# rasd3/3D-Dual-Fusion

Hardware: AMD Instinct MI355X
Metric: nuScenes sweeps/sec (0.075 m voxel, ~60k pts) (higher is better)
Workload: dtype f32 (fp32-grade throughout: every matrix-core GEMM -- C>=32 sparse convs, neck / head convs, FFN, query linears, image projection, value GEMM -- takes its fp32 operands as fp16 hi+lo pairs, 22 significand bits, 3 MFMA products, fp32 accumulate: <= 4e-6 of scale against float64, the grade of the exac

## Files before the change

### 3d-dual-fusion_amd/csrc/common.h

```cpp
#pragma once
#include <hip/hip_runtime.h>
#include <stdint.h>
#include <stdio.h>

#include "../../include/df3d_hip.h"

namespace df3d {

void set_error(const char *fmt, ...);

#define DF3D_CHECK_ARG(cond, ...)            \
  do {                                       \
    if (!(cond)) {                           \
      df3d::set_error(__VA_ARGS__);          \
      return DF3D_EINVAL;                    \
    }                                        \
  } while (0)

#define DF3D_HIP(call)                                                                   \
  do {                                                                                   \
    hipError_t e__ = (call);                                                             \
    if (e__ != hipSuccess) {                                                             \
      df3d::set_error("%s failed: %s (%s:%d)", #call, hipGetErrorString(e__), __FILE__, \
                      __LINE__);                                                         \
      return DF3D_EHIP;                                                                  \
    }                                                                                    \
  } while (0)

#define DF3D_LAUNCH_CHECK()                                                                  \
  do {                                                                                       \
    hipError_t e__ = hipGetLastError();                                                      \
    if (e__ != hipSuccess) {                                                                 \
      df3d::set_error("kernel launch failed: %s (%s:%d)", hipGetErrorString(e__), __FILE__, \
                      __LINE__);                                                             \
      return DF3D_EHIP;                                                                      \
    }                                                                                        \
  } while (0)

static inline size_t align_up(size_t v, size_t a) { return (v + a - 1) / a * a; }
#ifdef __HIPCC__
#define DF3D_SA_EXP 5
#define DF3D_SW_EXP 7
#define DF3D_SA_SCALE 32.0f
#define DF3D_SW_SCALE 128.0f
#define DF3D_SA_INV 0.03125f
#define DF3D_ACC_UNSCALE 0.000244140625f
#define DF3D_AA_UNSCALE 0.0009765625f
typedef __bf16 df3d_bf16x2 __attribute__((ext_vector_type(2)));
typedef _Float16 df3d_f16x2 __attribute__((ext_vector_type(2)));
typedef float df3d_f32x2 __attribute__((ext_vector_type(2)));
typedef _Float16 df3d_f16x8 __attribute__((ext_vector_type(8)));

static __device__ unsigned g_split_overflow_tu;

__device__ __forceinline__ unsigned rd_mix(unsigned x) {
  x ^= x >> 16, x *= 0x7feb352du, x ^= x >> 15, x *= 0x846ca68bu, x ^= x >> 16;
  return x;
}
__device__ __forceinline__ bool rd_keep(unsigned long long i, unsigned s0, unsigned s1, unsigned thr) {
  const unsigned h = rd_mix(rd_mix((unsigned)i ^ s0) + (unsigned)(i >> 32) * 0x9E3779B9u + s1);
  return (h >> 8) >= thr;
}

__device__ __forceinline__ unsigned bf16_pair(float x0, float x1) {
  df3d_f32x2 v = {x0, x1};
  return __builtin_bit_cast(unsigned, __builtin_convertvector(v, df3d_bf16x2));
}
__device__ __forceinline__ void split_pair_bf16_ref(float x0, float x1, unsigned &hi, unsigned &lo) {
  df3d_f32x2 v = {x0, x1};
  df3d_bf16x2 h = __builtin_convertvector(v, df3d_bf16x2);
  df3d_f32x2 r = v - __builtin_convertvector(h, df3d_f32x2);
  df3d_bf16x2 l = __builtin_convertvector(r, df3d_bf16x2);
  hi = __builtin_bit_cast(unsigned, h);
  lo = __builtin_bit_cast(unsigned, l);
}
template <bool CHECK>
__device__ __forceinline__ void split_pair_f16_ref(float x0, float x1, float s, unsigned &hi, unsigned &lo) {
  df3d_f32x2 v = {x0 * s, x1 * s};
  if (CHECK) {
    if (__builtin_expect(!(__builtin_fabsf(v[0]) <= 65504.f) || !(__builtin_fabsf(v[1]) <= 65504.f), 0))
      atomicOr(&g_split_overflow_tu, 1u);
  }
  df3d_f16x2 h = __builtin_convertvector(v, df3d_f16x2);
  df3d_f32x2 r = v - __builtin_convertvector(h, df3d_f32x2);
  df3d_f16x2 l = __builtin_convertvector(r, df3d_f16x2);
  hi = __builtin_bit_cast(unsigned, h);
  lo = __builtin_bit_cast(unsigned, l);
}
#define DF3D_SPLIT_PAIR_(x0, x1, S, CHECK, HI, LO)                          \
  do {                                                                      \
    unsigned sp_h__, sp_l__;                                                \
    df3d::split_pair_f16_ref<CHECK>(x0, x1, S, sp_h__, sp_l__);             \
    (HI) = sp_h__;                                                          \
    (LO) = sp_l__;                                                          \
  } while (0)
#define split_pair(x0, x1, HI, LO) DF3D_SPLIT_PAIR_(x0, x1, DF3D_SA_SCALE, true, HI, LO)
#define split_pair_nc(x0, x1, HI, LO) DF3D_SPLIT_PAIR_(x0, x1, DF3D_SA_SCALE, false, HI, LO)
#define split_pair_acc(x0, x1, HI, LO, AMAX)                                                  \
  do {                                                                                        \
    (AMAX) = fmaxf((AMAX), fmaxf(__builtin_fabsf(x0), __builtin_fabsf(x1)));                  \
    DF3D_SPLIT_PAIR_(x0, x1, DF3D_SA_SCALE, false, HI, LO);                                   \
  } while (0)
#define split_range_flag(AMAX)                                                                \
  do {                                                                                        \
    if (__builtin_expect(!((AMAX) * DF3D_SA_SCALE <= 65504.f), 0)) atomicOr(&df3d::g_split_overflow_tu, 1u); \
  } while (0)
#define split_range_flag_scaled(AMAX)                                                         \
  do {                                                                                        \
    if (__builtin_expect(!((AMAX) <= 65504.f), 0)) atomicOr(&df3d::g_split_overflow_tu, 1u);  \
  } while (0)
#define split_pair_w(x0, x1, HI, LO) DF3D_SPLIT_PAIR_(x0, x1, DF3D_SW_SCALE, true, HI, LO)
#define split_pair_bf16(x0, x1, HI, LO)                  \
  do {                                                   \
    unsigned sp_h__, sp_l__;                             \
    df3d::split_pair_bf16_ref(x0, x1, sp_h__, sp_l__);   \
    (HI) = sp_h__;                                       \
    (LO) = sp_l__;                                       \
  } while (0)
__device__ __forceinline__ void split_one(float x, unsigned &hi, unsigned &lo) {
  unsigned h, l;
  split_pair_f16_ref<true>(x, 0.f, DF3D_SA_SCALE, h, l);
  hi = h & 0xffffu;
  lo = l & 0xffffu;
}
__device__ __forceinline__ df3d_f32x2 split_part_to_f32(unsigned packed) {
  df3d_f32x2 v = __builtin_convertvector(__builtin_bit_cast(df3d_f16x2, packed), df3d_f32x2);
  return v * DF3D_SA_INV;
}
__device__ __forceinline__ df3d_f32x2 split_to_f32(unsigned hi, unsigned lo) {
  df3d_f32x2 h = __builtin_convertvector(__builtin_bit_cast(df3d_f16x2, hi), df3d_f32x2);
  df3d_f32x2 l = __builtin_convertvector(__builtin_bit_cast(df3d_f16x2, lo), df3d_f32x2);
  return (h + l) * DF3D_SA_INV;
}
#define DF3D_MFMA_F16(A, B, C) \
  __builtin_amdgcn_mfma_f32_16x16x32_f16(__builtin_bit_cast(df3d_f16x8, A), __builtin_bit_cast(df3d_f16x8, B), C, 0, 0, 0)
#endif

void split_overflow_register(const void *symbol, const char *tu);
#ifdef __HIPCC__
#define DF3D_SPLIT_OVERFLOW_TU(name)                                                                       \
  namespace {                                                                                              \
  struct SplitOverflowReg_##name {                                                                         \
    SplitOverflowReg_##name() { df3d::split_overflow_register((const void *)&df3d::g_split_overflow_tu, #name); } \
  } g_split_overflow_reg_##name;                                                                           \
  }
#endif

static inline int cdiv(long long a, long long b) { return (int)((a + b - 1) / b); }

struct Arena {
  char *base;
  size_t size, off;
  Arena(void *p, size_t n) : base((char *)p), size(n), off(0) {}
  template <typename T>
  T *take(size_t count) {
    size_t o = align_up(off, 256);
    size_t end = o + count * sizeof(T);
    if (end > size) return nullptr;
    off = end;
    return (T *)(base + o);
  }
};
static inline size_t arena_need(size_t cur, size_t bytes) { return align_up(cur, 256) + bytes; }

size_t scan_scratch_bytes(size_t n);
int exclusive_scan_u32(const uint32_t *in, uint32_t *out, size_t n, uint32_t *total,
                       void *scratch, size_t scratch_bytes, hipStream_t stream);
int exclusive_scan_popc64(const unsigned long long *words, uint32_t *out, size_t n,
                          uint32_t *total, void *scratch, size_t scratch_bytes,
                          hipStream_t stream);

struct GridHeader {
  int batch, shape[3];
  unsigned long long ncells;
  unsigned long long nwords;
  size_t off_bits, off_prefix, off_total, off_scratch, scratch_bytes;
};
struct GridView {
  const unsigned long long *bits;
  const uint32_t *prefix;
  int shape[3];
  long long vol;
};
GridHeader grid_layout(int batch, const int *shape);
static inline GridView grid_view(const void *blob, const GridHeader &h) {
  GridView v;
  v.bits = (const unsigned long long *)((const char *)blob + h.off_bits);
  v.prefix = (const uint32_t *)((const char *)blob + h.off_prefix);
  v.shape[0] = h.shape[0];
  v.shape[1] = h.shape[1];
  v.shape[2] = h.shape[2];
  v.vol = (long long)h.shape[0] * h.shape[1] * h.shape[2];
  return v;
}

__device__ __forceinline__ int grid_rank(const GridView &g, long long flat) {
  unsigned long long w = g.bits[flat >> 6];
  int b = (int)(flat & 63);
  if (!((w >> b) & 1ull)) return -1;
  return (int)(g.prefix[flat >> 6] + __popcll(w & ((1ull << b) - 1ull)));
}

size_t conv_operand_packed_bytes(int parts, int kvol, int cin, int cout);
int conv_operand_rows(int parts, const float *x, long long n, int c, void *rows, hipStream_t stream);
int conv_operand_run(int parts, const void *in, int n_in, int cin, const void *packed, int kvol, int cout, const int32_t *nbr,
                     int n_out, const float *bias, const float *scale, const float *shift, const void *residual, int relu,
                     float *out, void *out_rows, hipStream_t stream);

size_t topk_keys_workspace(int S, long long n, int K);
int topk_keys(const unsigned long long *keys, int S, long long n, int K, unsigned long long *out, int32_t *out_count,
              void *ws, size_t ws_bytes, hipStream_t stream);

}
```

### 3d-dual-fusion_amd/csrc/common.hip

```cpp
#include <stdarg.h>
#include <string.h>

#include "common.h"

namespace df3d {

static thread_local char g_err[512] = "";

void set_error(const char *fmt, ...) {
  va_list ap;
  va_start(ap, fmt);
  vsnprintf(g_err, sizeof(g_err), fmt, ap);
  va_end(ap);
}

static const void *g_ovf_sym[64];
static const char *g_ovf_tu[64];
static constexpr int OVF_MAXDEV = 16;
static unsigned *g_ovf_dev[OVF_MAXDEV][64];
static unsigned **g_ovf_table[OVF_MAXDEV];
static int g_ovf_table_n[OVF_MAXDEV];
static int g_ovf_n = 0;

static int ovf_resolve() {
  int dev = 0;
  if (hipGetDevice(&dev) != hipSuccess || dev < 0 || dev >= OVF_MAXDEV) return -1;
  for (int i = 0; i < g_ovf_n; ++i) {
    if (g_ovf_dev[dev][i]) continue;
    void *p = nullptr;
    if (hipGetSymbolAddress(&p, g_ovf_sym[i]) != hipSuccess || !p) {
      (void)hipGetLastError();
      continue;
    }
    g_ovf_dev[dev][i] = (unsigned *)p;
  }
  return dev;
}

__global__ void ovf_collect_kernel(unsigned *const *flags, int n, unsigned *out, int reset) {
  unsigned m = 0;
  for (int i = threadIdx.x; i < n; i += 64) {
    unsigned *f = flags[i];
    if (f && *f) {
      m |= 1u << (i & 31);
      if (reset) *f = 0u;
    }
  }
  for (int d = 32; d >= 1; d >>= 1) m |= __shfl_xor(m, d, 64);
  if (threadIdx.x == 0) *out = m;
}
void split_overflow_register(const void *symbol, const char *tu) {
  if (g_ovf_n < 64) g_ovf_sym[g_ovf_n] = symbol, g_ovf_tu[g_ovf_n] = tu, ++g_ovf_n;
}

constexpr int SCAN_THREADS = 256;
constexpr int SCAN_ITEMS = 4;
constexpr int SCAN_TILE = SCAN_THREADS * SCAN_ITEMS;

struct LoadU32 {
  const uint32_t *p;
  __device__ uint32_t operator()(size_t i) const { return p[i]; }
};
struct LoadPopc {
  const unsigned long long *p;
  __device__ uint32_t operator()(size_t i) const { return (uint32_t)__popcll(p[i]); }
};

__device__ __forceinline__ uint32_t wave_incl_scan(uint32_t v, int lane) {
#pragma unroll
  for (int d = 1; d < 64; d <<= 1) {
    uint32_t t = __shfl_up(v, d, 64);
    if (lane >= d) v += t;
  }
  return v;
}

__device__ __forceinline__ void block_excl_scan(uint32_t (&x)[SCAN_ITEMS], uint32_t &total,
                                                uint32_t *lds ) {
  int tid = threadIdx.x, lane = tid & 63, wave = tid >> 6;
  uint32_t s = 0;
#pragma unroll
  for (int i = 0; i < SCAN_ITEMS; ++i) s += x[i];
  uint32_t inc = wave_incl_scan(s, lane);
  if (lane == 63) lds[wave] = inc;
  __syncthreads();
  uint32_t woff = 0, tot = 0;
#pragma unroll
  for (int w = 0; w < SCAN_THREADS / 64; ++w) {
    uint32_t v = lds[w];
    if (w < wave) woff += v;
    tot += v;
  }
  uint32_t run = woff + inc - s;
#pragma unroll
  for (int i = 0; i < SCAN_ITEMS; ++i) {
    uint32_t v = x[i];
    x[i] = run;
    run += v;
  }
  total = tot;
  __syncthreads();
}

template <typename Loader>
__global__ __launch_bounds__(SCAN_THREADS) void scan_tiles_kernel(Loader in, uint32_t *out, size_t n,
                                                                  uint32_t *sums, uint32_t *total_if_single) {
  __shared__ uint32_t lds[SCAN_THREADS / 64 + 1];
  size_t base = (size_t)blockIdx.x * SCAN_TILE + (size_t)threadIdx.x * SCAN_ITEMS;
  uint32_t x[SCAN_ITEMS];
#pragma unroll
  for (int i = 0; i < SCAN_ITEMS; ++i) x[i] = (base + i < n) ? in(base + i) : 0u;
  uint32_t tot;
  block_excl_scan(x, tot, lds);
#pragma unroll
  for (int i = 0; i < SCAN_ITEMS; ++i)
    if (base + i < n) out[base + i] = x[i];
  if (threadIdx.x == 0) {
    sums[blockIdx.x] = tot;
    if (total_if_single) *total_if_single = tot;
  }
}

__global__ __launch_bounds__(SCAN_THREADS) void scan_offset_kernel(uint32_t *out, size_t n, const uint32_t *sums, size_t nb,
                                                                   uint32_t *total) {
  __shared__ uint32_t lds[SCAN_THREADS / 64];
  __shared__ uint32_t s_off;
  const int tid = threadIdx.x, lane = tid & 63, wave = tid >> 6;
  const bool last = blockIdx.x + 1 == nb;
  const size_t upto = last ? nb : blockIdx.x;
  uint32_t s = 0, mine = 0;
  for (size_t i = tid; i < upto; i += SCAN_THREADS) {
    const uint32_t v = sums[i];
    if (i < blockIdx.x) mine += v;
    s += v;
  }
#pragma unroll
  for (int d = 32; d >= 1; d >>= 1) {
    mine += __shfl_xor(mine, d, 64);
    s += __shfl_xor(s, d, 64);
  }
  __shared__ uint32_t lds2[SCAN_THREADS / 64];
  if (lane == 0) {
    lds[wave] = mine;
    lds2[wave] = s;
  }
  __syncthreads();
  if (tid == 0) {
    uint32_t a = 0, b = 0;
    for (int w = 0; w < SCAN_THREADS / 64; ++w) {
      a += lds[w];
      b += lds2[w];
    }
    s_off = a;
    if (last && total) *total = b;
  }
  __syncthreads();
  const uint32_t add = s_off;
  size_t base = (size_t)blockIdx.x * SCAN_TILE + (size_t)threadIdx.x * SCAN_ITEMS;
#pragma unroll
  for (int i = 0; i < SCAN_ITEMS; ++i)
    if (base + i < n) out[base + i] += add;
}

size_t scan_scratch_bytes(size_t n) { return align_up((n / SCAN_TILE + 2) * sizeof(uint32_t), 256); }

template <typename Loader>
static int scan_impl(Loader in, uint32_t *out, size_t n, uint32_t *total, void *scratch, size_t scratch_bytes,
                     hipStream_t stream) {
  if (n == 0) {
    if (total) DF3D_HIP(hipMemsetAsync(total, 0, sizeof(uint32_t), stream));
    return DF3D_OK;
  }
  if (scratch_bytes < scan_scratch_bytes(n)) {
    set_error("scan scratch too small");
    return DF3D_ENOMEM;
  }
  uint32_t *sums = (uint32_t *)scratch;
  size_t nb = (n + SCAN_TILE - 1) / SCAN_TILE;
  hipLaunchKernelGGL(scan_tiles_kernel<Loader>, dim3((unsigned)nb), dim3(SCAN_THREADS), 0, stream, in, out, n, sums,
                     nb == 1 ? total : (uint32_t *)nullptr);
  if (nb > 1)
    hipLaunchKernelGGL(scan_offset_kernel, dim3((unsigned)nb), dim3(SCAN_THREADS), 0, stream, out, n, sums, nb, total);
  DF3D_LAUNCH_CHECK();
  return DF3D_OK;
}

int exclusive_scan_u32(const uint32_t *in, uint32_t *out, size_t n, uint32_t *total, void *scratch,
                       size_t scratch_bytes, hipStream_t stream) {
  return scan_impl(LoadU32{in}, out, n, total, scratch, scratch_bytes, stream);
}
int exclusive_scan_popc64(const unsigned long long *words, uint32_t *out, size_t n, uint32_t *total,
                          void *scratch, size_t scratch_bytes, hipStream_t stream) {
  return scan_impl(LoadPopc{words}, out, n, total, scratch, scratch_bytes, stream);
}

}

extern "C" {

int df3d_version(void) { return 100; }

int df3d_split_overflow(int reset, char *where, int where_len) {
  unsigned any = 0;
  if (where && where_len > 0) where[0] = 0;
  if (hipDeviceSynchronize() != hipSuccess) {
    df3d::set_error("df3d_split_overflow: hipDeviceSynchronize failed");
    return DF3D_EHIP;
  }
  const int dev = df3d::ovf_resolve();
  if (dev < 0) {
    df3d::set_error("df3d_split_overflow: no current device");
    return DF3D_EHIP;
  }
  for (int i = 0; i < df3d::g_ovf_n; ++i) {
    unsigned *f = df3d::g_ovf_dev[dev][i];
    if (!f) continue;
    unsigned v = 0;
    DF3D_HIP(hipMemcpy(&v, f, sizeof(v), hipMemcpyDeviceToHost));
    if (v) {
      any |= v;
      if (where && where_len > 0) {
        size_t used = strlen(where);
        snprintf(where + used, (size_t)where_len - used, "%s%s", used ? "," : "", df3d::g_ovf_tu[i]);
      }
      if (reset) DF3D_HIP(hipMemset(f, 0, sizeof(v)));
    }
  }
  return any ? 1 : 0;
}

int df3d_split_overflow_collect(uint32_t *out, int reset, void *stream_) {
  hipStream_t stream = (hipStream_t)stream_;
  DF3D_CHECK_ARG(out, "split_overflow_collect: null output");
  const int dev = df3d::ovf_resolve();
  if (dev < 0) {
    df3d::set_error("df3d_split_overflow_collect: no current device");
    return DF3D_EHIP;
  }
  int resolved = 0;
  for (int i = 0; i < df3d::g_ovf_n; ++i) resolved += df3d::g_ovf_dev[dev][i] != nullptr;
  if (!df3d::g_ovf_table[dev] || df3d::g_ovf_table_n[dev] != resolved) {
    if (!df3d::g_ovf_table[dev]) DF3D_HIP(hipMalloc((void **)&df3d::g_ovf_table[dev], sizeof(unsigned *) * 64));
    DF3D_HIP(hipMemcpyAsync(df3d::g_ovf_table[dev], df3d::g_ovf_dev[dev], sizeof(unsigned *) * 64, hipMemcpyHostToDevice, stream));
    DF3D_HIP(hipStreamSynchronize(stream));
    df3d::g_ovf_table_n[dev] = resolved;
  }
  hipLaunchKernelGGL(df3d::ovf_collect_kernel, dim3(1), dim3(64), 0, stream, df3d::g_ovf_table[dev], df3d::g_ovf_n, out, reset);
  DF3D_LAUNCH_CHECK();
  return DF3D_OK;
}

int df3d_split_overflow_units(char *buf, int buflen) {
  if (!buf || buflen <= 0) return df3d::g_ovf_n;
  buf[0] = 0;
  for (int i = 0; i < df3d::g_ovf_n; ++i) {
    size_t used = strlen(buf);
    snprintf(buf + used, (size_t)buflen - used, "%s%s", used ? "," : "", df3d::g_ovf_tu[i]);
  }
  return df3d::g_ovf_n;
}
const char *df3d_last_error(void) { return df3d::g_err; }

int df3d_device_count(void) {
  int n = 0;
  if (hipGetDeviceCount(&n) != hipSuccess) return 0;
  return n;
}

int df3d_device_arch(char *buf, int buflen) {
  hipDeviceProp_t p;
  if (hipGetDeviceProperties(&p, 0) != hipSuccess) {
    df3d::set_error("hipGetDeviceProperties failed");
    return DF3D_EHIP;
  }
  snprintf(buf, buflen, "%s", p.gcnArchName);
  return DF3D_OK;
}
}
```

### 3d-dual-fusion_amd/csrc/executor.hip

```cpp
#include <stdio.h>
#include <stdlib.h>
#include <string.h>

#include <condition_variable>
#include <deque>
#include <mutex>
#include <string>
#include <thread>
#include <vector>

#include "common.h"

using namespace df3d;

namespace {

struct IndexSet {
  const int32_t *indices = nullptr;
  int n = 0;
  int shape[3] = {0, 0, 0};
  void *grid = nullptr;
  size_t grid_bytes = 0;
  int32_t *perm = nullptr;
  bool sorted = false;
};

struct LayerOut {
  float *features = nullptr;
  void *split = nullptr;
  void *rows16 = nullptr;
  int set = -1;
  int channels = 0;
  bool ran = false;
};

struct Bump {
  char *base;
  size_t cap, used = 0;
  bool overflow = false;
  Bump(void *p, size_t bytes) : base((char *)p), cap(bytes) {}
  void *take(size_t bytes) {
    size_t off = align_up(used, 256);
    used = off + bytes;
    if (used > cap) {
      overflow = true;
      return nullptr;
    }
    return base + off;
  }
};

int kvol_of(const int *k) { return k[0] * k[1] * k[2]; }

thread_local hipStream_t g_geo_stream = nullptr;
thread_local std::vector<hipEvent_t> g_event_sets[16];
thread_local unsigned g_run_counter = 0;
#define g_events g_event_sets[g_run_counter & 15]
thread_local hipEvent_t g_inputs_ready = nullptr;
hipEvent_t order_event(size_t i) {
  while (g_events.size() <= i) {
    hipEvent_t e = nullptr;
    if (hipEventCreateWithFlags(&e, hipEventDisableTiming) != hipSuccess) return nullptr;
    g_events.push_back(e);
  }
  return g_events[i];
}

}

extern "C" int df3d_backbone_inputs_ready(void *event) {
  g_inputs_ready = (hipEvent_t)event;
  return DF3D_OK;
}

namespace {

struct RunState {
  const df3d_layer *layers = nullptr;
  int nlayers = 0;
  const int32_t *indices = nullptr;
  int n = 0, in_channels = 0, batch = 0;
  int shape[3] = {0, 0, 0};
  Bump *gmem = nullptr;
  Bump *fmem = nullptr;
  Bump own_g{nullptr, 0}, own_f{nullptr, 0};
  std::vector<IndexSet> sets;
  std::vector<LayerOut> outs;
  std::vector<std::pair<int, const int32_t *>> rulebooks;
  std::vector<int> rulebook_set;
  std::vector<const int32_t *> layer_nbr;
  std::vector<const void *> rulebook_lists;
  std::vector<const void *> layer_lists;
  std::vector<int> layer_in_set;
  std::vector<char> need_f32;
  std::vector<char> want_split;
  int32_t *count_dev = nullptr;
  void *split0 = nullptr;
  void *rows16_0 = nullptr;
  hipEvent_t done = nullptr;
  hipEvent_t img_done = nullptr;
  int geometry_layers = 0;
  const float *input_features = nullptr;
  int range_next = 0;
};

int fail_arena(RunState &S, Bump *m, size_t *arena_used, size_t arena_bytes) {
  if (arena_used) *arena_used = m->used;
  set_error("backbone_run: arena of %zu bytes is too small (needed more than %zu)", arena_bytes, m->used);
  (void)S;
  return DF3D_ENOMEM;
}


int layer_parts(const df3d_layer &L) {
  if (!L.packed) return 0;
  if (L.reserved & 2) return 1;
  if (L.reserved & 8) return 3;
  return conv_operand_packed_bytes(2, kvol_of(L.ksize), L.cin, L.cout) != 0 ? 2 : 0;
}

int state_init(RunState &S, const df3d_layer *layers, int nlayers, const int32_t *indices, int n, int in_channels, int batch,
               const int *shape) {
  S.layers = layers, S.nlayers = nlayers, S.indices = indices, S.n = n, S.in_channels = in_channels, S.batch = batch;
  memcpy(S.shape, shape, sizeof(S.shape));
  S.outs.assign(nlayers, LayerOut());
  S.layer_nbr.assign(nlayers, nullptr);
  S.layer_lists.assign(nlayers, nullptr);
  S.layer_in_set.assign(nlayers, 0);
  IndexSet s0;
  s0.indices = indices;
  s0.n = n;
  memcpy(s0.shape, shape, sizeof(s0.shape));
  S.sets.push_back(s0);
  S.need_f32.assign(nlayers, 0);
  S.want_split.assign(nlayers, 0);
  bool flagged = false;
  for (int li = 0; li < nlayers; ++li) flagged = flagged || (layers[li].reserved & 4);
  static const bool write_all = getenv("DF3D_EXEC_F32_ALL") && atoi(getenv("DF3D_EXEC_F32_ALL"));
  if (write_all) flagged = false;
  for (int li = 0; li < nlayers; ++li) {
    const df3d_layer &L = layers[li];
    if (!flagged || (L.reserved & 4) || li == nlayers - 1) S.need_f32[li] = 1;
    if (L.residual >= 0 && L.residual < nlayers) S.need_f32[L.residual] = 1;
    const int parts = layer_parts(L);
    const bool split_consumer = parts >= 2 && !(L.reserved & 1) &&
                                conv_operand_packed_bytes(parts, kvol_of(L.ksize), L.cin, L.cout) != 0;
    if (L.input >= 0 && L.input < nlayers && !split_consumer) S.need_f32[L.input] = 1;
    if (L.input >= 0 && L.input < nlayers && split_consumer && !(L.reserved & 8)) S.want_split[L.input] = 1;
  }
  return DF3D_OK;
}

int geo_layer(RunState &S, int li, hipStream_t gstream, bool *new_table) {
  void *gs_ = (void *)gstream;
  Bump &mem = *S.gmem;
  const df3d_layer &L = S.layers[li];
  const int batch = S.batch;
  *new_table = false;
  DF3D_CHECK_ARG(L.input >= -1 && L.input < li && L.residual >= -1 && L.residual < li,
                 "backbone_run: layer %d reads a later layer", li);
  const int in_set = L.input < 0 ? 0 : S.outs[L.input].set;
  const int cin = L.input < 0 ? S.in_channels : S.outs[L.input].channels;
  DF3D_CHECK_ARG(cin == L.cin, "backbone_run: layer %d expects %d input channels, gets %d", li, L.cin, cin);
  const int K = kvol_of(L.ksize);
  DF3D_CHECK_ARG(K > 0 && K <= DF3D_MAX_KVOL, "backbone_run: layer %d kernel volume %d unsupported", li, K);
  if (!S.count_dev) {
    S.count_dev = (int32_t *)mem.take(256);
    if (!S.count_dev) return DF3D_ENOMEM;
  }
  const int32_t *nbr = nullptr;
  const void *lists = nullptr;
  int out_set = -1;
  if (L.rulebook >= 0)
    for (size_t r = 0; r < S.rulebooks.size(); ++r)
      if (S.rulebooks[r].first == L.rulebook) {
        nbr = S.rulebooks[r].second;
        lists = S.rulebook_lists[r];
        out_set = S.rulebook_set[r];
        DF3D_CHECK_ARG(L.kind != 0 || out_set == in_set,
                       "backbone_run: layer %d shares rulebook %d but reads another index set", li, L.rulebook);
      }
  if (!nbr) {
    auto ensure_grid = [&](int si) -> int {
      IndexSet &T = S.sets[si];
      if (T.grid) return DF3D_OK;
      T.grid_bytes = df3d_grid_bytes(batch, T.shape);
      T.grid = mem.take(T.grid_bytes);
      if (!T.sorted) T.perm = (int32_t *)mem.take((size_t)T.n * 4);
      if (!T.grid || (!T.sorted && !T.perm)) return DF3D_ENOMEM;
      return df3d_grid_build(T.indices, T.n, batch, T.shape, T.grid, T.grid_bytes, T.perm, gs_);
    };
    if (L.kind == 0) {
      int rc = ensure_grid(in_set);
      if (rc) return rc;
      const IndexSet &T = S.sets[in_set];
      int32_t *t = (int32_t *)mem.take((size_t)K * T.n * 4);
      if (!t) return DF3D_ENOMEM;
      rc = df3d_subm_neighbors(T.grid, T.perm, T.indices, T.n, batch, T.shape, L.ksize, L.dilation, t, gs_);
      if (rc) return rc;
      nbr = t;
      out_set = in_set;
    } else {
      const IndexSet T = S.sets[in_set];
      IndexSet O;
      for (int d = 0; d < 3; ++d)
        O.shape[d] = (T.shape[d] + 2 * L.padding[d] - L.dilation[d] * (L.ksize[d] - 1) - 1) / L.stride[d] + 1;
      long long fan = 1;
      for (int d = 0; d < 3; ++d) fan *= (L.ksize[d] + L.stride[d] - 1) / L.stride[d];
      long long vol = (long long)batch * O.shape[0] * O.shape[1] * O.shape[2];
      long long cap = (long long)T.n * (fan < K ? fan : K);
      if (cap > vol) cap = vol;
      if (cap < 1) cap = 1;
      O.grid_bytes = df3d_grid_bytes(batch, O.shape);
      O.grid = mem.take(O.grid_bytes);
      int32_t *oi = (int32_t *)mem.take((size_t)cap * 16);
      if (!O.grid || !oi) return DF3D_ENOMEM;
      int rc = df3d_conv_out_indices(T.indices, T.n, batch, T.shape, O.shape, L.ksize, L.stride, L.padding,
                                     L.dilation, O.grid, O.grid_bytes, oi, (int)cap, S.count_dev, gs_);
      if (rc) return rc;
      int32_t cnt = 0;
      DF3D_HIP(hipMemcpyAsync(&cnt, S.count_dev, sizeof(cnt), hipMemcpyDeviceToHost, gstream));
      DF3D_HIP(hipStreamSynchronize(gstream));
      if (cnt > cap) {
        set_error("backbone_run: layer %d produced %d outputs, capacity bound %lld", li, cnt, cap);
        return DF3D_EINVAL;
      }
      if (cnt <= 0) {
        set_error("backbone_run: layer %d has no active outputs", li);
        return DF3D_EINVAL;
      }
      O.indices = oi;
      O.n = cnt;
      O.sorted = true;
      S.sets.push_back(O);
      out_set = (int)S.sets.size() - 1;
      rc = ensure_grid(in_set);
      if (rc) return rc;
      const IndexSet &Tg = S.sets[in_set];
      int32_t *t = (int32_t *)mem.take((size_t)K * cnt * 4);
      if (!t) return DF3D_ENOMEM;
      rc = df3d_conv_neighbors(Tg.grid, Tg.perm, oi, cnt, batch, Tg.shape, L.ksize, L.stride, L.padding, L.dilation,
                               t, gs_);
      if (rc) return rc;
      nbr = t;
    }
    *new_table = true;
    static const bool lists_on = !(getenv("DF3D_ROW_LISTS") && getenv("DF3D_ROW_LISTS")[0] == '0');
    const bool fp32_small = !(L.reserved & 1) && layer_parts(L) == 0;
    const int n_rows = S.sets[out_set].n;
    if (lists_on && fp32_small && L.cin <= 16 && (L.cout == 16 || L.cout == 32) && n_rows >= 2048 &&
        S.sets[in_set].n < (1 << 26)) {
      const size_t lb = df3d_nbr_row_lists_bytes(K, n_rows);
      void *blob = lb ? mem.take(lb) : nullptr;
      if (lb && !blob) return DF3D_ENOMEM;
      if (blob) {
        int rc = df3d_nbr_row_lists(nbr, K, n_rows, S.sets[in_set].n, blob, lb, gs_);
        if (rc) return rc;
        lists = blob;
      }
    }
    S.rulebooks.push_back(std::make_pair(L.rulebook, nbr));
    S.rulebook_lists.push_back(lists);
    S.rulebook_set.push_back(out_set);
  }
  S.layer_nbr[li] = nbr;
  S.layer_lists[li] = lists;
  S.layer_in_set[li] = in_set;
  S.outs[li].set = out_set;
  S.outs[li].channels = L.cout;
  S.geometry_layers = li + 1;
  return DF3D_OK;
}

void view_geometry(const RunState &S, int li, df3d_layer_view &v) {
  const IndexSet &OS = S.sets[S.outs[li].set];
  v.nbr = S.layer_nbr[li];
  v.kvol = kvol_of(S.layers[li].ksize);
  v.indices = OS.indices;
  v.grid = OS.grid;
  v.grid_bytes = OS.grid_bytes;
  v.n = OS.n;
  v.channels = S.layers[li].cout;
  v.rows_sorted = OS.sorted ? 1 : 0;
  memcpy(v.shape, OS.shape, sizeof(v.shape));
}

int conv_layer(RunState &S, int li, const float *features, df3d_layer_view *views, hipStream_t stream) {
  void *stream_ = (void *)stream;
  Bump &mem = *S.fmem;
  const df3d_layer &L = S.layers[li];
  const int K = kvol_of(L.ksize);
  const int32_t *nbr = S.layer_nbr[li];
  const int in_set = S.layer_in_set[li], out_set = S.outs[li].set;
  const float *in_feat = L.input < 0 ? features : S.outs[L.input].features;
  const int n_out = S.sets[out_set].n;
  const int n_in = S.sets[in_set].n;
  LayerOut &o = S.outs[li];
  df3d_layer_view &v = views[li];
  view_geometry(S, li, v);
  if (L.reserved & 1) {
    v.features = nullptr;
    v.split = nullptr;
    return DF3D_OK;
  }
  DF3D_CHECK_ARG(L.input < 0 || S.outs[L.input].ran, "backbone_run: layer %d reads a geometry-only layer", li);
  o.ran = true;
  const int parts = layer_parts(L);
  if (parts)
    DF3D_CHECK_ARG(conv_operand_packed_bytes(parts, K, L.cin, L.cout) != 0,
                   "backbone_run: layer %d has no kernel on %d-part operands (K=%d cin=%d cout=%d)", li, parts, K, L.cin, L.cout);
  if (S.need_f32[li] || parts < 2) {
    o.features = (float *)mem.take((size_t)n_out * L.cout * 4);
    if (!o.features) return DF3D_ENOMEM;
  }
  const float *res = L.residual < 0 ? nullptr : S.outs[L.residual].features;
  if (L.residual >= 0)
    DF3D_CHECK_ARG(S.outs[L.residual].set == out_set && S.outs[L.residual].channels == L.cout,
                   "backbone_run: residual of layer %d lives on another index set", li);
  if (parts) {
    const size_t bpc = 2 * (size_t)parts;
    auto slot = [&](int layer) -> void *& {
      if (parts == 1) return layer < 0 ? S.rows16_0 : S.outs[layer].rows16;
      return layer < 0 ? S.split0 : S.outs[layer].split;
    };
    auto operand = [&](int layer, const float *rows, int n, int c, const void **out) {
      void *&r = slot(layer);
      if (!r) {
        r = mem.take((size_t)n * c * bpc);
        if (!r) return (int)DF3D_ENOMEM;
        int rc = conv_operand_rows(parts, rows, n, c, r, stream);
        if (rc) return rc;
      }
      *out = r;
      return (int)DF3D_OK;
    };
    const void *in_rows = nullptr, *res_rows = res;
    int rc = operand(L.input, in_feat, n_in, L.cin, &in_rows);
    if (rc) return rc;
    if (parts == 1 && L.residual >= 0) {
      rc = operand(L.residual, res, n_out, L.cout, &res_rows);
      if (rc) return rc;
    }
    void *&out_rows = slot(li);
    out_rows = mem.take((size_t)n_out * L.cout * bpc);
    if (!out_rows) return DF3D_ENOMEM;
    rc = conv_operand_run(parts, in_rows, n_in, L.cin, L.packed, K, L.cout, nbr, n_out, L.bias, L.scale, L.shift, res_rows,
                          L.relu, o.features, out_rows, stream);
    if (rc) return rc;
  } else {
    if (S.want_split[li] && S.layer_lists[li] && L.cout % 8 == 0) {
      o.split = mem.take((size_t)n_out * L.cout * 4);
      if (!o.split) return DF3D_ENOMEM;
    }
    int rc = df3d_sparse_conv_fused_lists(in_feat, n_in, L.cin, L.weight, K, L.cout, nbr, S.layer_lists[li], n_out, L.bias,
                                          L.scale, L.shift, res, L.relu, o.features, o.split, stream_);
    if (rc) return rc;
  }
  v.features = o.features;
  v.split = o.split ? o.split : o.rows16;
  v.reserved = o.rows16 && !o.split ? 2 : ((L.reserved & 8) && o.split ? 4 : 0);
  return DF3D_OK;
}

}

extern "C" int df3d_backbone_run(const df3d_layer *layers, int nlayers, const float *features, const int32_t *indices,
                                 int n, int in_channels, int batch, const int *shape, void *arena,
                                 size_t arena_bytes, df3d_layer_view *views, size_t *arena_used, void *stream_) {
  hipStream_t stream = (hipStream_t)stream_;
  hipEvent_t inputs_ready = g_inputs_ready;
  g_inputs_ready = nullptr;
  ++g_run_counter;
  DF3D_CHECK_ARG(layers && nlayers > 0 && features && indices && shape && arena && views,
                 "backbone_run: null argument");
  DF3D_CHECK_ARG(n > 0 && batch > 0, "backbone_run: empty input (n=%d, batch=%d)", n, batch);
  static const bool two_streams = !(getenv("DF3D_EXEC_STREAMS") && getenv("DF3D_EXEC_STREAMS")[0] == '0');
  hipStream_t gstream = stream;
  size_t next_event = 0;
  if (two_streams) {
    if (!g_geo_stream) DF3D_HIP(hipStreamCreateWithFlags(&g_geo_stream, hipStreamNonBlocking));
    gstream = g_geo_stream;
    if (inputs_ready) {
      DF3D_HIP(hipStreamWaitEvent(gstream, inputs_ready, 0));
    } else {
      hipEvent_t e = order_event(next_event++);
      DF3D_CHECK_ARG(e != nullptr, "backbone_run: cannot create an event");
      DF3D_HIP(hipEventRecord(e, stream));
      DF3D_HIP(hipStreamWaitEvent(gstream, e, 0));
    }
  }
  RunState S;
  S.own_g = Bump(arena, arena_bytes);
  S.gmem = S.fmem = &S.own_g;
  int rc = state_init(S, layers, nlayers, indices, n, in_channels, batch, shape);
  if (rc) return rc;
  for (int li = 0; li < nlayers; ++li) {
    bool new_table = false;
    rc = geo_layer(S, li, gstream, &new_table);
    if (rc == DF3D_ENOMEM) return fail_arena(S, S.gmem, arena_used, arena_bytes);
    if (rc) return rc;
    if (new_table && two_streams) {
      hipEvent_t e = order_event(next_event++);
      DF3D_CHECK_ARG(e != nullptr, "backbone_run: cannot create an event");
      DF3D_HIP(hipEventRecord(e, gstream));
      DF3D_HIP(hipStreamWaitEvent(stream, e, 0));
    }
    rc = conv_layer(S, li, features, views, stream);
    if (rc == DF3D_ENOMEM) return fail_arena(S, S.fmem, arena_used, arena_bytes);
    if (rc) return rc;
  }
  if (two_streams) {
    hipEvent_t e = order_event(next_event++);
    DF3D_CHECK_ARG(e != nullptr, "backbone_run: cannot create an event");
    DF3D_HIP(hipEventRecord(e, gstream));
    DF3D_HIP(hipStreamWaitEvent(stream, e, 0));
  }
  for (int li = 0; li < nlayers; ++li) {
    const IndexSet &OS = S.sets[S.outs[li].set];
    views[li].grid = OS.grid;
    views[li].grid_bytes = OS.grid_bytes;
  }
  if (arena_used) *arena_used = S.gmem->used;
  return DF3D_OK;
}

extern "C" int df3d_backbone_geometry(const df3d_layer *layers, int nlayers, const int32_t *indices, int n, int in_channels,
                                      int batch, const int *shape, void *arena, size_t arena_bytes, void *inputs_ready,
                                      df3d_layer_view *views, size_t *arena_used, void **handle) {
  DF3D_CHECK_ARG(layers && nlayers > 0 && indices && shape && arena && views && handle, "backbone_geometry: null argument");
  DF3D_CHECK_ARG(n > 0 && batch > 0, "backbone_geometry: empty input (n=%d, batch=%d)", n, batch);
  *handle = nullptr;
  if (!g_geo_stream) DF3D_HIP(hipStreamCreateWithFlags(&g_geo_stream, hipStreamNonBlocking));
  hipStream_t gstream = g_geo_stream;
  if (inputs_ready) DF3D_HIP(hipStreamWaitEvent(gstream, (hipEvent_t)inputs_ready, 0));
  RunState *S = new RunState();
  S->own_g = Bump(arena, arena_bytes);
  S->gmem = &S->own_g;
  int rc = state_init(*S, layers, nlayers, indices, n, in_channels, batch, shape);
  for (int li = 0; li < nlayers && !rc; ++li) {
    bool new_table = false;
    rc = geo_layer(*S, li, gstream, &new_table);
  }
  if (arena_used) *arena_used = S->gmem->used;
  if (rc == DF3D_ENOMEM) set_error("backbone_geometry: arena of %zu bytes is too small (needed more than %zu)", arena_bytes, S->gmem->used);
  if (!rc && hipEventCreateWithFlags(&S->done, hipEventDisableTiming) != hipSuccess) {
    set_error("backbone_geometry: cannot create an event");
    rc = DF3D_EHIP;
  }
  if (!rc && hipEventRecord(S->done, gstream) != hipSuccess) {
    set_error("backbone_geometry: hipEventRecord failed");
    rc = DF3D_EHIP;
  }
  if (rc) {
    if (S->done) (void)hipEventDestroy(S->done);
    delete S;
    return rc;
  }
  for (int li = 0; li < nlayers; ++li) {
    view_geometry(*S, li, views[li]);
    views[li].features = nullptr;
    views[li].split = nullptr;
    views[li].reserved = 0;
  }
  *handle = S;
  return DF3D_OK;
}

extern "C" int df3d_backbone_convs(void *handle, const float *features, void *arena, size_t arena_bytes,
                                   df3d_layer_view *views, size_t *arena_used, void *stream_) {
  DF3D_CHECK_ARG(handle && features && arena && views, "backbone_convs: null argument");
  RunState &S = *(RunState *)handle;
  DF3D_CHECK_ARG(S.geometry_layers == S.nlayers, "backbone_convs: the geometry phase of this handle did not finish");
  hipStream_t stream = (hipStream_t)stream_;
  DF3D_HIP(hipStreamWaitEvent(stream, S.done, 0));
  S.own_f = Bump(arena, arena_bytes);
  S.fmem = &S.own_f;
  S.split0 = S.rows16_0 = nullptr;
  for (auto &o : S.outs) o.features = nullptr, o.split = nullptr, o.rows16 = nullptr, o.ran = false;
  for (int li = 0; li < S.nlayers; ++li) {
    int rc = conv_layer(S, li, features, views, stream);
    if (rc == DF3D_ENOMEM) {
      if (arena_used) *arena_used = S.fmem->used;
      set_error("backbone_convs: arena of %zu bytes is too small (needed more than %zu)", arena_bytes, S.fmem->used);
      return DF3D_ENOMEM;
    }
    if (rc) return rc;
  }
  if (arena_used) *arena_used = S.fmem->used;
  return DF3D_OK;
}

extern "C" int df3d_backbone_convs_range(void *handle, const float *features, int first, int last, void *arena,
                                         size_t arena_bytes, df3d_layer_view *views, size_t *arena_used, void *stream_) {
  DF3D_CHECK_ARG(handle && features && arena && views, "backbone_convs_range: null argument");
  RunState &S = *(RunState *)handle;
  DF3D_CHECK_ARG(S.geometry_layers == S.nlayers, "backbone_convs_range: the geometry phase of this handle did not finish");
  DF3D_CHECK_ARG(first >= 0 && first < last && last <= S.nlayers, "backbone_convs_range: bad layer range [%d, %d) of %d", first,
                 last, S.nlayers);
  hipStream_t stream = (hipStream_t)stream_;
  if (first == 0) {
    DF3D_HIP(hipStreamWaitEvent(stream, S.done, 0));
    S.own_f = Bump(arena, arena_bytes);
    S.fmem = &S.own_f;
    S.split0 = S.rows16_0 = nullptr;
    for (auto &o : S.outs) o.features = nullptr, o.split = nullptr, o.rows16 = nullptr, o.ran = false;
    S.input_features = features;
  } else {
    DF3D_CHECK_ARG(S.range_next == first && S.fmem == &S.own_f && S.own_f.base == (char *)arena,
                   "backbone_convs_range: range [%d, %d) does not continue the previous one (next layer %d)", first, last,
                   S.range_next);
    LayerOut &p = S.outs[first - 1];
    DF3D_CHECK_ARG(p.ran, "backbone_convs_range: layer %d has not run", first - 1);
    p.features = (float *)features;
    p.split = nullptr;
    p.rows16 = nullptr;
  }
  for (int li = first; li < last; ++li) {
    int rc = conv_layer(S, li, S.input_features, views, stream);
    if (rc == DF3D_ENOMEM) {
      if (arena_used) *arena_used = S.fmem->used;
      set_error("backbone_convs_range: arena of %zu bytes is too small (needed more than %zu)", arena_bytes, S.fmem->used);
      return DF3D_ENOMEM;
    }
    if (rc) return rc;
  }
  S.range_next = last;
  if (arena_used) *arena_used = S.fmem->used;
  return DF3D_OK;
}

extern "C" int df3d_backbone_geometry_wait(void *handle, void *stream_) {
  DF3D_CHECK_ARG(handle, "backbone_geometry_wait: null handle");
  DF3D_HIP(hipStreamWaitEvent((hipStream_t)stream_, ((RunState *)handle)->done, 0));
  return DF3D_OK;
}

extern "C" int df3d_frame_head_image_wait(void *handle, void *stream_) {
  DF3D_CHECK_ARG(handle && ((RunState *)handle)->img_done, "frame_head_image_wait: no image projection in this handle");
  DF3D_HIP(hipStreamWaitEvent((hipStream_t)stream_, ((RunState *)handle)->img_done, 0));
  return DF3D_OK;
}

extern "C" int df3d_backbone_release(void *handle) {
  if (!handle) return DF3D_OK;
  RunState *S = (RunState *)handle;
  if (S->done) (void)hipEventDestroy(S->done);
  if (S->img_done) (void)hipEventDestroy(S->img_done);
  delete S;
  return DF3D_OK;
}


namespace {

struct HeadTicket {
  df3d_frame_head_desc d;
  std::vector<const float *> points;
  std::vector<int> num_points;
  Bump mem{nullptr, 0};
  size_t arena_bytes = 0;
  std::vector<df3d_layer_view> views;
  df3d_frame_head_out out;
  RunState *state = nullptr;
  int rc = DF3D_OK;
  std::string err;
  bool done = false;
  std::mutex mu;
  std::condition_variable cv;
};

struct HeadWorker {
  std::thread th;
  std::mutex mu;
  std::condition_variable cv;
  std::deque<HeadTicket *> q;
  bool stop = false;
  int device = 0;
};

thread_local hipStream_t g_img_stream = nullptr;

#define HEAD_TAKE(ptr, type, bytes)              \
  do {                                           \
    ptr = (type)t.mem.take(bytes);               \
    if (!ptr) return DF3D_ENOMEM;                \
  } while (0)

int frame_head_run(HeadTicket &t) {
  const df3d_frame_head_desc &d = t.d;
  if (!g_geo_stream) {
    static const bool high = !(getenv("DF3D_HEAD_PRIORITY") && getenv("DF3D_HEAD_PRIORITY")[0] == '0');
    int least = 0, greatest = 0;
    if (high && hipDeviceGetStreamPriorityRange(&least, &greatest) == hipSuccess && greatest != least) {
      DF3D_HIP(hipStreamCreateWithPriority(&g_geo_stream, hipStreamNonBlocking, greatest));
    } else {
      DF3D_HIP(hipStreamCreateWithFlags(&g_geo_stream, hipStreamNonBlocking));
    }
  }
  hipStream_t gs = g_geo_stream;
  void *gs_ = (void *)gs;
  const int B = d.batch, C = d.point_channels;
  memset(&t.out, 0, sizeof(t.out));
  static const bool dbg = getenv("DF3D_HEAD_DEBUG") != nullptr;
#define HEAD_PHASE(msg)                                                   \
  do {                                                                    \
    if (dbg) {                                                            \
      hipError_t e__ = hipStreamSynchronize(gs);                          \
      fprintf(stderr, "df3d frame head: %s -> %d\n", msg, (int)e__);     \
      fflush(stderr);                                                     \
    }                                                                     \
  } while (0)
  if (d.inputs_ready) DF3D_HIP(hipStreamWaitEvent(gs, (hipEvent_t)d.inputs_ready, 0));
  std::vector<float *> mean(B);
  std::vector<int32_t *> coors(B);
  std::vector<int> cap(B);
  int32_t *counts_dev;
  HEAD_TAKE(counts_dev, int32_t *, (size_t)(B > 64 ? B : 64) * 4);
  for (int b = 0; b < B; ++b) {
    const int P = t.num_points[b];
    cap[b] = (d.max_voxels < 0 || d.max_voxels > P) ? P : d.max_voxels;
    if (cap[b] < 1) cap[b] = 1;
    int32_t *num;
    void *ws;
    const size_t wsb = df3d_hard_voxelize_workspace_bytes(P, d.max_points, cap[b]);
    HEAD_TAKE(mean[b], float *, (size_t)cap[b] * C * 4);
    HEAD_TAKE(coors[b], int32_t *, (size_t)cap[b] * 16);
    HEAD_TAKE(num, int32_t *, (size_t)cap[b] * 4);
    HEAD_TAKE(ws, void *, wsb ? wsb : 1);
    int rc = df3d_hard_voxelize_batched(t.points[b], P, C, d.voxel_size, d.coors_range, d.max_points, cap[b], d.break_at_cap, b,
                                        nullptr, coors[b], num, mean[b], counts_dev + b, ws, wsb, gs_);
    if (rc) return rc;
  }
  HEAD_PHASE("voxelize queued");
  std::vector<int32_t> cnt(B, 0);
  DF3D_HIP(hipMemcpyAsync(cnt.data(), counts_dev, (size_t)B * 4, hipMemcpyDeviceToHost, gs));
  DF3D_HIP(hipStreamSynchronize(gs));
  long long total = 0;
  for (int b = 0; b < B; ++b) total += cnt[b];
  float *feats = mean[0];
  int32_t *ind = coors[0];
  if (B > 1) {
    HEAD_TAKE(feats, float *, (size_t)(total ? total : 1) * C * 4);
    HEAD_TAKE(ind, int32_t *, (size_t)(total ? total : 1) * 16);
    size_t at = 0;
    for (int b = 0; b < B; ++b) {
      if (cnt[b] > 0) {
        DF3D_HIP(hipMemcpyAsync(feats + at * C, mean[b], (size_t)cnt[b] * C * 4, hipMemcpyDeviceToDevice, gs));
        DF3D_HIP(hipMemcpyAsync(ind + at * 4, coors[b], (size_t)cnt[b] * 16, hipMemcpyDeviceToDevice, gs));
      }
      at += cnt[b];
    }
  }
  t.out.features = feats;
  t.out.coors = ind;
  t.out.n = (int)total;
  RunState *S = new RunState();
  t.state = S;
  if (hipEventCreateWithFlags(&S->done, hipEventDisableTiming) != hipSuccess) {
    set_error("frame_head: cannot create an event");
    return DF3D_EHIP;
  }
  if (d.img_ptrs && d.img_count > 0) {
    if (!g_img_stream) DF3D_HIP(hipStreamCreateWithFlags(&g_img_stream, hipStreamNonBlocking));
    HEAD_TAKE(t.out.img_split, void *, (size_t)d.img_count * d.img_pixels * 512);
    HEAD_TAKE(t.out.img_gate, float *, (size_t)d.img_count * d.img_pixels * 4);
    if (hipEventCreateWithFlags(&S->img_done, hipEventDisableTiming) != hipSuccess) {
      set_error("frame_head: cannot create an event");
      return DF3D_EHIP;
    }
    if (d.inputs_ready) DF3D_HIP(hipStreamWaitEvent(g_img_stream, (hipEvent_t)d.inputs_ready, 0));
    int rc = df3d_imgproj_split(d.img_ptrs, d.img_count, d.img_cin, d.img_pixels, d.img_packed, t.out.img_split, t.out.img_gate,
                                (void *)g_img_stream);
    if (rc) return rc;
    DF3D_HIP(hipEventRecord(S->img_done, g_img_stream));
    t.out.img_done = S->img_done;
  }
  if (total > 0 && d.nlayers > 0) {
    S->gmem = &t.mem;
    int rc = state_init(*S, d.layers, d.nlayers, ind, (int)total, C, B, d.shape);
    HEAD_PHASE("voxel counts read");
    if (dbg) fprintf(stderr, "df3d frame head: n = %lld, arena used %zu of %zu\n", total, t.mem.used, t.arena_bytes);
    for (int li = 0; li < d.nlayers && !rc; ++li) {
      bool new_table = false;
      rc = geo_layer(*S, li, gs, &new_table);
      if (dbg) {
        char b[64];
        snprintf(b, sizeof(b), "geometry layer %d rc %d", li, rc);
        HEAD_PHASE(b);
      }
    }
    if (rc) return rc;
    t.views.assign(d.nlayers, df3d_layer_view());
    for (int li = 0; li < d.nlayers; ++li) {
      memset(&t.views[li], 0, sizeof(df3d_layer_view));
      view_geometry(*S, li, t.views[li]);
    }
    if (d.ncam > 0) {
      DF3D_CHECK_ARG(d.nproj >= 0 && d.nproj <= DF3D_HEAD_MAX_PROJ && d.slots_proj < d.nproj, "frame_head: bad projection list");
      for (int p = 0; p < d.nproj; ++p) {
        const int li = d.proj[p].layer;
        DF3D_CHECK_ARG(li >= 0 && li < d.nlayers, "frame_head: projection %d reads layer %d", p, li);
        const IndexSet &T = S->sets[S->outs[li].set];
        HEAD_TAKE(t.out.grid_xy[p], int32_t *, (size_t)d.ncam * T.n * 8);
        HEAD_TAKE(t.out.mask[p], uint8_t *, (size_t)d.ncam * T.n);
        HEAD_TAKE(t.out.point_inv[p], float *, (size_t)T.n * 12);
        t.out.proj_n[p] = T.n;
        rc = df3d_project_voxels(T.indices, T.n, B, d.ncam, d.proj[p].scale_xyz, d.pc_min, d.lidar2cam, d.intrinsic, d.raw_hw,
                                 d.depth_thres, d.image_scale, d.feat_scale, t.out.grid_xy[p], t.out.mask[p],
                                 t.out.point_inv[p], nullptr, d.aug_inv, gs_);
        if (rc) return rc;
        if (d.proj[p].want_winner && d.feat_h > 0 && d.feat_w > 0) {
          HEAD_TAKE(t.out.winner[p], int32_t *, (size_t)B * d.ncam * d.feat_h * d.feat_w * 4);
          rc = df3d_scatter_winner(T.indices, t.out.grid_xy[p], t.out.mask[p], T.n, B, d.ncam, d.feat_h, d.feat_w,
                                   t.out.winner[p], gs_);
          if (rc) return rc;
        }
      }
      if (d.slots_proj >= 0) {
        const int p = d.slots_proj;
        const IndexSet &T = S->sets[S->outs[d.proj[p].layer].set];
        HEAD_TAKE(t.out.pos, int32_t *, (size_t)d.ncam * T.n * 4);
        HEAD_TAKE(t.out.counts, int32_t *, (size_t)B * d.ncam * 4);
        rc = df3d_query_slots(t.out.mask[p], T.indices, T.n, B, d.ncam, t.out.pos, t.out.counts, gs_);
        if (rc) return rc;
        int32_t *ptot = nullptr;
        if (d.want_pixrow && d.feat_h > 0 && d.feat_w > 0) {
          const size_t wsb = df3d_query_pixel_rows_workspace_bytes(B, d.ncam, d.feat_h, d.feat_w);
          void *ws;
          HEAD_TAKE(t.out.pixrow, int32_t *, (size_t)B * d.ncam * d.feat_h * d.feat_w * 4);
          HEAD_TAKE(ptot, int32_t *, 256);
          HEAD_TAKE(ws, void *, wsb);
          rc = df3d_query_pixel_rows(T.indices, t.out.grid_xy[p], t.out.mask[p], T.n, B, d.ncam, d.feat_h, d.feat_w, t.out.pixrow,
                                     ptot, ws, wsb, gs_);
          if (rc) return rc;
        }
        std::vector<int32_t> qc((size_t)B * d.ncam, 0);
        DF3D_HIP(hipMemcpyAsync(qc.data(), t.out.counts, qc.size() * 4, hipMemcpyDeviceToHost, gs));
        int32_t tot = 0;
        if (ptot) DF3D_HIP(hipMemcpyAsync(&tot, ptot, 4, hipMemcpyDeviceToHost, gs));
        DF3D_HIP(hipStreamSynchronize(gs));
        t.out.pixrow_total = tot;
        int mx = 0;
        for (int v : qc) mx = v > mx ? v : mx;
        t.out.max_ne = mx;
      }
    }
  }
  HEAD_PHASE("projection / slots");
  DF3D_HIP(hipEventRecord(S->done, gs));
  return DF3D_OK;
}

void head_worker_main(HeadWorker *w) {
  (void)hipSetDevice(w->device);
  for (;;) {
    HeadTicket *t = nullptr;
    {
      std::unique_lock<std::mutex> lk(w->mu);
      w->cv.wait(lk, [&] { return w->stop || !w->q.empty(); });
      if (w->q.empty()) return;
      t = w->q.front();
      w->q.pop_front();
    }
    int rc = frame_head_run(*t);
    {
      std::lock_guard<std::mutex> lk(t->mu);
      t->rc = rc;
      if (rc) t->err = df3d_last_error();
      t->done = true;
      t->cv.notify_all();
    }
  }
}

}

extern "C" void *df3d_head_worker_create(int device) {
  HeadWorker *w = new HeadWorker();
  w->device = device;
  w->th = std::thread(head_worker_main, w);
  return w;
}

extern "C" int df3d_head_worker_destroy(void *worker) {
  if (!worker) return DF3D_OK;
  HeadWorker *w = (HeadWorker *)worker;
  {
    std::lock_guard<std::mutex> lk(w->mu);
    w->stop = true;
  }
  w->cv.notify_all();
  if (w->th.joinable()) w->th.join();
  for (HeadTicket *t : w->q) delete t;
  delete w;
  return DF3D_OK;
}

extern "C" int df3d_frame_head_submit(void *worker, const df3d_frame_head_desc *desc, void *arena, size_t arena_bytes,
                                      void **ticket) {
  DF3D_CHECK_ARG(worker && desc && arena && ticket, "frame_head_submit: null argument");
  DF3D_CHECK_ARG(desc->batch > 0 && desc->points && desc->num_points && desc->point_channels > 0,
                 "frame_head_submit: no point clouds");
  DF3D_CHECK_ARG(desc->nlayers == 0 || desc->layers, "frame_head_submit: layer table missing");
  HeadTicket *t = new HeadTicket();
  t->d = *desc;
  t->points.assign(desc->points, desc->points + desc->batch);
  t->num_points.assign(desc->num_points, desc->num_points + desc->batch);
  t->d.points = nullptr, t->d.num_points = nullptr;
  t->mem = Bump(arena, arena_bytes);
  t->arena_bytes = arena_bytes;
  HeadWorker *w = (HeadWorker *)worker;
  {
    std::lock_guard<std::mutex> lk(w->mu);
    w->q.push_back(t);
  }
  w->cv.notify_one();
  *ticket = t;
  return DF3D_OK;
}

extern "C" int df3d_frame_head_wait(void *ticket, df3d_layer_view *views, df3d_frame_head_out *out, size_t *arena_used,
                                    void **handle) {
  DF3D_CHECK_ARG(ticket && out && handle, "frame_head_wait: null argument");
  HeadTicket *t = (HeadTicket *)ticket;
  {
    std::unique_lock<std::mutex> lk(t->mu);
    t->cv.wait(lk, [&] { return t->done; });
  }
  *handle = nullptr;
  if (arena_used) *arena_used = t->mem.used;
  int rc = t->rc;
  if (rc) {
    if (rc == DF3D_ENOMEM) set_error("frame_head: arena of %zu bytes is too small (needed more than %zu)", t->arena_bytes, t->mem.used);
    else set_error("%s", t->err.c_str());
    if (t->state) {
      if (t->state->done) (void)hipEventDestroy(t->state->done);
      if (t->state->img_done) (void)hipEventDestroy(t->state->img_done);
      delete t->state;
    }
    delete t;
    return rc;
  }
  *out = t->out;
  if (views && !t->views.empty()) memcpy(views, t->views.data(), t->views.size() * sizeof(df3d_layer_view));
  RunState *S = t->state;
  S->gmem = nullptr;
  *handle = S;
  delete t;
  return DF3D_OK;
}
```

### 3d-dual-fusion_amd/csrc/fusion.hip

```cpp
#include "common.h"

typedef float f32x4 __attribute__((ext_vector_type(4)));
typedef unsigned int u32x4 __attribute__((ext_vector_type(4)));

namespace df3d {

DF3D_SPLIT_OVERFLOW_TU(fusion)

struct ProjArgs {
  const int32_t *ind;
  int n, batch, ncam;
  float sx, sy, sz, minx, miny, minz;
  const float *l2c;
  const float *intr;
  const int32_t *raw_hw;
  const float *thres;
  float image_scale;
  const float *feat_scale;
  int32_t *grid;
  uint8_t *mask;
  float *pinv;
  float *depth;
  const float *aug;
};

__device__ __forceinline__ float dot4(float a0, float a1, float a2, float a3, const float *m) {
#pragma clang fp contract(off)
  float acc = a0 * m[0];
  acc = fmaf(a1, m[1], acc);
  acc = fmaf(a2, m[2], acc);
  acc = fmaf(a3, m[3], acc);
  return acc;
}

__global__ __launch_bounds__(256) void project_voxels_kernel(ProjArgs a) {
#pragma clang fp contract(off)
  long long t = (long long)blockIdx.x * blockDim.x + threadIdx.x;
  if (t >= (long long)a.n * a.ncam) return;
  int cam = (int)(t / a.n);
  int i = (int)(t - (long long)cam * a.n);
  const int32_t *p = a.ind + (size_t)i * 4;
  int b = p[0];
  float px = (float)p[3] * a.sx;
  px = px + a.minx;
  float py = (float)p[2] * a.sy;
  py = py + a.miny;
  float pz = (float)p[1] * a.sz;
  pz = pz + a.minz;
  if (a.aug) {
    const float *g = a.aug + (size_t)b * 30;
    px = px + g[0];
    py = py + g[1];
    pz = pz + g[2];
#pragma unroll
    for (int f = 0; f < 3; ++f) {
      const float *m = g + 3 + 9 * f;
      const float qx = fmaf(pz, m[6], fmaf(py, m[3], px * m[0]));
      const float qy = fmaf(pz, m[7], fmaf(py, m[4], px * m[1]));
      const float qz = fmaf(pz, m[8], fmaf(py, m[5], px * m[2]));
      px = qx, py = qy, pz = qz;
    }
  }
  if (cam == 0) {
    a.pinv[(size_t)i * 3 + 0] = px;
    a.pinv[(size_t)i * 3 + 1] = py;
    a.pinv[(size_t)i * 3 + 2] = pz;
  }
  const float *M = a.l2c + ((size_t)b * a.ncam + cam) * 16;
  float cx = dot4(px, py, pz, 1.f, M + 0);
  float cy = dot4(px, py, pz, 1.f, M + 4);
  float cz = dot4(px, py, pz, 1.f, M + 8);
  const float *K = a.intr + ((size_t)b * a.ncam + cam) * 9;
  float uh = fmaf(cz, K[2], fmaf(cy, K[1], (cx * K[0])));
  float vh = fmaf(cz, K[5], fmaf(cy, K[4], (cx * K[3])));
  float wh = fmaf(cz, K[8], fmaf(cy, K[7], (cx * K[6])));
  float u = uh / wh, v = vh / wh;
  bool ok = isfinite(u) && isfinite(v) && fabsf(u) < 1e9f && fabsf(v) < 1e9f;
  long long gx = 0, gy = 0;
  if (ok) {
    gx = (long long)u;
    gy = (long long)v;
    gx = (long long)(a.image_scale * (float)gx);
    gy = (long long)(a.image_scale * (float)gy);
    const int32_t *hw = a.raw_hw + ((size_t)b * a.ncam + cam) * 2;
    ok = gx > 0 && gx < hw[1] && gy > 0 && gy < hw[0] && cz > a.thres[cam];
  }
  int fx = 0, fy = 0;
  if (ok) {
    const float *fs = a.feat_scale + ((size_t)b * a.ncam + cam) * 2;
    fx = (int)((float)gx * fs[0]);
    fy = (int)((float)gy * fs[1]);
  }
  a.grid[((size_t)cam * a.n + i) * 2 + 0] = fx;
  a.grid[((size_t)cam * a.n + i) * 2 + 1] = fy;
  a.mask[(size_t)cam * a.n + i] = ok ? 1 : 0;
  if (a.depth) a.depth[(size_t)cam * a.n + i] = ok ? cz : 0.f;
}

struct ScatArgs {
  const float *feat;
  const float *pinv;
  const int32_t *ind;
  const int32_t *grid;
  const uint8_t *mask;
  int n, C, ncam, H, W;
  int32_t *winner;
  float *canvas;
};

__global__ __launch_bounds__(256) void scatter_winner_kernel(ScatArgs a) {
  long long t = (long long)blockIdx.x * blockDim.x + threadIdx.x;
  if (t >= (long long)a.n * a.ncam) return;
  int cam = (int)(t / a.n), i = (int)(t - (long long)cam * a.n);
  if (!a.mask[(size_t)cam * a.n + i]) return;
  int gx = a.grid[((size_t)cam * a.n + i) * 2], gy = a.grid[((size_t)cam * a.n + i) * 2 + 1];
  if (gx < 0 || gx >= a.W || gy < 0 || gy >= a.H) return;
  int img = a.ind[(size_t)i * 4] * a.ncam + cam;
  atomicMax(&a.winner[((size_t)img * a.H + gy) * a.W + gx], i);
}

__global__ __launch_bounds__(256) void scatter_write_kernel(ScatArgs a) {
  long long t = (long long)blockIdx.x * blockDim.x + threadIdx.x;
  if (t >= (long long)a.n * a.ncam) return;
  int cam = (int)(t / a.n), i = (int)(t - (long long)cam * a.n);
  if (!a.mask[(size_t)cam * a.n + i]) return;
  int gx = a.grid[((size_t)cam * a.n + i) * 2], gy = a.grid[((size_t)cam * a.n + i) * 2 + 1];
  if (gx < 0 || gx >= a.W || gy < 0 || gy >= a.H) return;
  int img = a.ind[(size_t)i * 4] * a.ncam + cam;
  size_t pix = (size_t)gy * a.W + gx;
  if (a.winner[(size_t)img * a.H * a.W + pix] != i) return;
  size_t hw = (size_t)a.H * a.W;
  float *dst = a.canvas + (size_t)img * (a.C + 3) * hw + pix;
  for (int c = 0; c < a.C; ++c) dst[(size_t)c * hw] = a.feat[(size_t)i * a.C + c];
  for (int c = 0; c < 3; ++c) dst[(size_t)(a.C + c) * hw] = a.pinv[(size_t)i * 3 + c];
}

struct AsmArgs {
  const float *feat;
  const float *pinv;
  const int32_t *ind;
  const int32_t *grid;
  const uint8_t *mask;
  const int32_t *pos;
  const float *img;
  int n, C, Ci, ncam, H, W, max_ne;
  float *v_feat;
  float *v_i_feat;
  float *qgrid;
  float *qpts;
};

__global__ __launch_bounds__(256) void assemble_queries_kernel(AsmArgs a) {
  long long w = ((long long)blockIdx.x * blockDim.x + threadIdx.x) >> 6;
  int lane = threadIdx.x & 63;
  if (w >= (long long)a.n * a.ncam) return;
  int cam = (int)(w / a.n), i = (int)(w - (long long)cam * a.n);
  if (!a.mask[(size_t)cam * a.n + i]) return;
  int slot = a.pos[(size_t)cam * a.n + i];
  if (slot >= a.max_ne) return;
  int img = a.ind[(size_t)i * 4] * a.ncam + cam;
  size_t q = (size_t)img * a.max_ne + slot;
  int gx = a.grid[((size_t)cam * a.n + i) * 2], gy = a.grid[((size_t)cam * a.n + i) * 2 + 1];
  for (int c = lane; c < a.C; c += 64) a.v_feat[q * a.C + c] = a.feat[(size_t)i * a.C + c];
  size_t hw = (size_t)a.H * a.W;
  const float *src = a.img + (size_t)img * a.Ci * hw + (size_t)gy * a.W + gx;
  for (int c = lane; c < a.Ci; c += 64) a.v_i_feat[q * a.Ci + c] = src[(size_t)c * hw];
  if (lane == 0) {
    a.qgrid[q * 2 + 0] = (float)gx / (float)a.W;
    a.qgrid[q * 2 + 1] = (float)gy / (float)a.H;
  }
  if (lane < 3) a.qpts[q * 3 + lane] = a.pinv[(size_t)i * 3 + lane];
}

__global__ __launch_bounds__(256) void writeback_kernel(const float *__restrict__ feat,
                                                        const float *__restrict__ enh,
                                                        const int32_t *__restrict__ ind,
                                                        const uint8_t *__restrict__ mask,
                                                        const int32_t *__restrict__ pos, int n, int C, int ncam,
                                                        int max_ne, float *__restrict__ out) {
  long long t = (long long)blockIdx.x * blockDim.x + threadIdx.x;
  if (t >= (long long)n * C) return;
  int i = (int)(t / C), c = (int)(t - (long long)i * C);
  float v = feat[t];
  int b = ind[(size_t)i * 4];
  for (int cam = 0; cam < ncam; ++cam) {
    if (mask[(size_t)cam * n + i]) {
      int slot = pos[(size_t)cam * n + i];
      if (slot < max_ne) v += enh[((size_t)(b * ncam + cam) * max_ne + slot) * C + c];
    }
  }
  out[t] = v;
}

__global__ __launch_bounds__(256) void writeback8_kernel(const float *__restrict__ feat, const float *__restrict__ enh,
                                                         const int32_t *__restrict__ ind, const uint8_t *__restrict__ mask,
                                                         const int32_t *__restrict__ pos, int n, int C, int ncam, int max_ne,
                                                         float *__restrict__ out, u32x4 *__restrict__ out_split) {
  const int C8 = C >> 3;
  long long t = (long long)blockIdx.x * blockDim.x + threadIdx.x;
  if (t >= (long long)n * C8) return;
  const int i = (int)(t / C8), c8 = (int)(t - (long long)i * C8);
  const float *f = feat + (size_t)i * C + c8 * 8;
  f32x4 v0 = *(const f32x4 *)f, v1 = *(const f32x4 *)(f + 4);
  const int b = ind[(size_t)i * 4];
  for (int cam = 0; cam < ncam; ++cam) {
    if (mask[(size_t)cam * n + i]) {
      const int slot = pos[(size_t)cam * n + i];
      if (slot < max_ne) {
        const float *e = enh + ((size_t)(b * ncam + cam) * max_ne + slot) * C + c8 * 8;
        v0 += *(const f32x4 *)e;
        v1 += *(const f32x4 *)(e + 4);
      }
    }
  }
  float *o = out + (size_t)i * C + c8 * 8;
  *(f32x4 *)o = v0;
  *(f32x4 *)(o + 4) = v1;
  if (out_split) {
    u32x4 h, l;
    split_pair(v0[0], v0[1], h[0], l[0]);
    split_pair(v0[2], v0[3], h[1], l[1]);
    split_pair(v1[0], v1[1], h[2], l[2]);
    split_pair(v1[2], v1[3], h[3], l[3]);
    out_split[((size_t)i * C8 + c8) * 2] = h;
    out_split[((size_t)i * C8 + c8) * 2 + 1] = l;
  }
}

}

using namespace df3d;

extern "C" int df3d_project_voxels(const int32_t *indices, int n, int batch, int ncam, const float *scale_xyz,
                                   const float *pc_min, const float *lidar2cam, const float *intrinsic,
                                   const int32_t *raw_hw, const float *depth_thres, float image_scale,
                                   const float *feat_scale, int32_t *grid_xy, uint8_t *mask, float *point_inv,
                                   float *depth, const float *aug_inv, void *stream_) {
  hipStream_t stream = (hipStream_t)stream_;
  DF3D_CHECK_ARG(indices && lidar2cam && intrinsic && raw_hw && depth_thres && feat_scale && grid_xy && mask &&
                     point_inv && scale_xyz && pc_min,
                 "project_voxels: null argument");
  if (n == 0) return DF3D_OK;
  ProjArgs a = {indices, n, batch, ncam, scale_xyz[0], scale_xyz[1], scale_xyz[2], pc_min[0], pc_min[1], pc_min[2],
                lidar2cam, intrinsic, raw_hw, depth_thres, image_scale, feat_scale, grid_xy, mask, point_inv, depth, aug_inv};
  hipLaunchKernelGGL(project_voxels_kernel, dim3(cdiv((long long)n * ncam, 256)), dim3(256), 0, stream, a);
  DF3D_LAUNCH_CHECK();
  return DF3D_OK;
}

extern "C" int df3d_scatter_to_image(const float *features, const float *point_inv, const int32_t *indices,
                                     const int32_t *grid_xy, const uint8_t *mask, int n, int channels, int batch,
                                     int ncam, int H, int W, int32_t *winner, float *canvas, void *stream_) {
  hipStream_t stream = (hipStream_t)stream_;
  DF3D_CHECK_ARG(winner && canvas, "scatter_to_image: null output");
  size_t nimg = (size_t)batch * ncam;
  DF3D_HIP(hipMemsetAsync(winner, 0xff, nimg * H * W * sizeof(int32_t), stream));
  DF3D_HIP(hipMemsetAsync(canvas, 0, nimg * (channels + 3) * (size_t)H * W * sizeof(float), stream));
  if (n == 0) return DF3D_OK;
  DF3D_CHECK_ARG(features && point_inv && indices && grid_xy && mask, "scatter_to_image: null input");
  ScatArgs a = {features, point_inv, indices, grid_xy, mask, n, channels, ncam, H, W, winner, canvas};
  dim3 g(cdiv((long long)n * ncam, 256));
  hipLaunchKernelGGL(scatter_winner_kernel, g, dim3(256), 0, stream, a);
  hipLaunchKernelGGL(scatter_write_kernel, g, dim3(256), 0, stream, a);
  DF3D_LAUNCH_CHECK();
  return DF3D_OK;
}

extern "C" int df3d_scatter_winner(const int32_t *indices, const int32_t *grid_xy, const uint8_t *mask, int n, int batch,
                                   int ncam, int H, int W, int32_t *winner, void *stream_) {
  hipStream_t stream = (hipStream_t)stream_;
  DF3D_CHECK_ARG(winner && batch > 0 && ncam > 0 && H > 0 && W > 0, "scatter_winner: bad arguments");
  DF3D_HIP(hipMemsetAsync(winner, 0xff, (size_t)batch * ncam * H * W * sizeof(int32_t), stream));
  if (n == 0) return DF3D_OK;
  DF3D_CHECK_ARG(indices && grid_xy && mask, "scatter_winner: null input");
  ScatArgs a = {nullptr, nullptr, indices, grid_xy, mask, n, 0, ncam, H, W, winner, nullptr};
  hipLaunchKernelGGL(scatter_winner_kernel, dim3(cdiv((long long)n * ncam, 256)), dim3(256), 0, stream, a);
  DF3D_LAUNCH_CHECK();
  return DF3D_OK;
}

extern "C" int df3d_assemble_queries(const float *features, const float *point_inv, const int32_t *indices,
                                     const int32_t *grid_xy, const uint8_t *mask, const int32_t *pos,
                                     const float *img_feats, int n, int channels, int img_channels, int batch,
                                     int ncam, int H, int W, int max_ne, float *v_feat, float *v_i_feat, float *qgrid,
                                     float *qpts, void *stream_) {
  hipStream_t stream = (hipStream_t)stream_;
  DF3D_CHECK_ARG(v_feat && v_i_feat && qgrid && qpts, "assemble_queries: null output");
  size_t nq = (size_t)batch * ncam * max_ne;
  DF3D_HIP(hipMemsetAsync(v_feat, 0, nq * channels * sizeof(float), stream));
  DF3D_HIP(hipMemsetAsync(v_i_feat, 0, nq * img_channels * sizeof(float), stream));
  DF3D_HIP(hipMemsetAsync(qgrid, 0, nq * 2 * sizeof(float), stream));
  DF3D_HIP(hipMemsetAsync(qpts, 0, nq * 3 * sizeof(float), stream));
  if (n == 0 || max_ne == 0) return DF3D_OK;
  DF3D_CHECK_ARG(features && point_inv && indices && grid_xy && mask && pos && img_feats,
                 "assemble_queries: null input");
  AsmArgs a = {features, point_inv, indices, grid_xy, mask, pos, img_feats, n, channels, img_channels, ncam, H, W,
               max_ne, v_feat, v_i_feat, qgrid, qpts};
  hipLaunchKernelGGL(assemble_queries_kernel, dim3(cdiv((long long)n * ncam * 64, 256)), dim3(256), 0, stream, a);
  DF3D_LAUNCH_CHECK();
  return DF3D_OK;
}

extern "C" int df3d_fusion_writeback(const float *features, const float *enh, const int32_t *indices,
                                     const uint8_t *mask, const int32_t *pos, int n, int channels, int ncam,
                                     int max_ne, float *out, void *stream_) {
  hipStream_t stream = (hipStream_t)stream_;
  if (n == 0) return DF3D_OK;
  DF3D_CHECK_ARG(features && enh && indices && mask && pos && out, "fusion_writeback: null argument");
  if (channels % 8 == 0 && (((uintptr_t)features | (uintptr_t)enh | (uintptr_t)out) & 15) == 0) {
    hipLaunchKernelGGL(writeback8_kernel, dim3(cdiv((long long)n * (channels / 8), 256)), dim3(256), 0, stream, features, enh,
                       indices, mask, pos, n, channels, ncam, max_ne, out, (u32x4 *)nullptr);
    DF3D_LAUNCH_CHECK();
    return DF3D_OK;
  }
  hipLaunchKernelGGL(writeback_kernel, dim3(cdiv((long long)n * channels, 256)), dim3(256), 0, stream, features, enh,
                     indices, mask, pos, n, channels, ncam, max_ne, out);
  DF3D_LAUNCH_CHECK();
  return DF3D_OK;
}

namespace df3d {

__global__ __launch_bounds__(256) void gate_scatter_kernel(const float *__restrict__ s9, const int32_t *__restrict__ ind,
                                                           const int32_t *__restrict__ grid,
                                                           const uint8_t *__restrict__ mask,
                                                           const int32_t *__restrict__ winner, int n, int ncam, int H,
                                                           int W, float *__restrict__ S) {
  long long t = (long long)blockIdx.x * blockDim.x + threadIdx.x;
  if (t >= (long long)n * ncam) return;
  int cam = (int)(t / n), i = (int)(t - (long long)cam * n);
  if (!mask[(size_t)cam * n + i]) return;
  int gx = grid[((size_t)cam * n + i) * 2], gy = grid[((size_t)cam * n + i) * 2 + 1];
  if (gx < 0 || gx >= W || gy < 0 || gy >= H) return;
  int img = ind[(size_t)i * 4] * ncam + cam;
  size_t pix = (size_t)gy * W + gx;
  if (winner[(size_t)img * H * W + pix] != i) return;
  size_t hw = (size_t)H * W;
  float *dst = S + (size_t)img * 9 * hw + pix;
#pragma unroll
  for (int k = 0; k < 9; ++k) dst[(size_t)k * hw] += s9[(size_t)i * 9 + k];
}

__global__ __launch_bounds__(256) void gate_scatter_rows_kernel(const float *__restrict__ feat, int C,
                                                                const float *__restrict__ pinv, const float *__restrict__ T,
                                                                const int32_t *__restrict__ winner, long long npix, int hw,
                                                                int clear, float *__restrict__ S) {
  extern __shared__ float Tl[];
  const int CE = C + 3;
  for (int e = threadIdx.x; e < 9 * CE; e += 256) {
    const int k = e / CE, c = e - k * CE;
    Tl[c * 9 + k] = T[e];
  }
  __syncthreads();
  const long long t = (long long)blockIdx.x * blockDim.x + threadIdx.x;
  if (t >= npix) return;
  const long long img = t / hw;
  const int pix = (int)(t - img * hw);
  float *dst = S + (size_t)img * 9 * hw + pix;
  const int i = winner[t];
  if (i < 0) {
    if (clear) {
#pragma unroll
      for (int k = 0; k < 9; ++k) dst[(size_t)k * hw] = 0.f;
    }
    return;
  }
  float acc[9];
#pragma unroll
  for (int k = 0; k < 9; ++k) acc[k] = 0.f;
  const float *f = feat + (size_t)i * C;
  for (int c0 = 0; c0 < C; c0 += 32) {
    float4 v[8];
#pragma unroll
    for (int u = 0; u < 8; ++u) v[u] = c0 + 4 * u < C ? *(const float4 *)(f + c0 + 4 * u) : make_float4(0.f, 0.f, 0.f, 0.f);
#pragma unroll
    for (int u = 0; u < 8; ++u) {
      const int c = c0 + 4 * u;
      if (c < C) {
        const float x[4] = {v[u].x, v[u].y, v[u].z, v[u].w};
#pragma unroll
        for (int j = 0; j < 4; ++j)
#pragma unroll
          for (int k = 0; k < 9; ++k) acc[k] = fmaf(x[j], Tl[(c + j) * 9 + k], acc[k]);
      }
    }
  }
#pragma unroll
  for (int j = 0; j < 3; ++j) {
    const float x = pinv[(size_t)i * 3 + j];
#pragma unroll
    for (int k = 0; k < 9; ++k) acc[k] = fmaf(x, Tl[(C + j) * 9 + k], acc[k]);
  }
#pragma unroll
  for (int k = 0; k < 9; ++k) dst[(size_t)k * hw] = clear ? acc[k] : dst[(size_t)k * hw] + acc[k];
}

template <bool BIAS>
__global__ __launch_bounds__(256) void gate_finish_kernel(const float *__restrict__ gate, const float *__restrict__ gate_bias,
                                                          const float *__restrict__ S,
                                                          const float *__restrict__ kg ,
                                                          int nimg, int H, int W, float *__restrict__ att) {
  long long t = (long long)blockIdx.x * blockDim.x + threadIdx.x;
  size_t hw = (size_t)H * W;
  if (t >= (long long)nimg * hw) return;
  int img = (int)(t / hw);
  int p = (int)(t - (long long)img * hw);
  int y = p / W, x = p - y * W;
  float acc = kg[18];
  const float gb = BIAS ? gate_bias[0] : 0.f;
#pragma unroll
  for (int ty = 0; ty < 3; ++ty)
#pragma unroll
    for (int tx = 0; tx < 3; ++tx) {
      int yy = y + ty - 1, xx = x + tx - 1;
      if (yy < 0 || yy >= H || xx < 0 || xx >= W) continue;
      int k = ty * 3 + tx;
      size_t q = (size_t)yy * W + xx;
      const float gq = BIAS ? gate[(size_t)img * hw + q] + gb : gate[(size_t)img * hw + q];
      acc += kg[k] + kg[9 + k] * gq + S[((size_t)img * 9 + k) * hw + q];
    }
  att[t] = 1.f / (1.f + __expf(-acc));
}

__global__ __launch_bounds__(256) void mark_query_pixels_kernel(const int32_t *__restrict__ ind, const int32_t *__restrict__ grid,
                                                                const uint8_t *__restrict__ mask, int n, int ncam, int H, int W,
                                                                uint32_t *__restrict__ flag) {
  long long t = (long long)blockIdx.x * blockDim.x + threadIdx.x;
  if (t >= (long long)n * ncam) return;
  const int cam = (int)(t / n), i = (int)(t - (long long)cam * n);
  if (!mask[t]) return;
  const int img = ind[(size_t)i * 4] * ncam + cam;
  const int gx = grid[t * 2], gy = grid[t * 2 + 1];
  flag[(size_t)img * H * W + (size_t)gy * W + gx] = 1u;
}

__global__ __launch_bounds__(256) void pixrow_kernel(const uint32_t *__restrict__ flag, const uint32_t *__restrict__ rank, size_t n,
                                                     int32_t *__restrict__ pixrow) {
  size_t i = (size_t)blockIdx.x * blockDim.x + threadIdx.x;
  if (i < n) pixrow[i] = flag[i] ? (int32_t)rank[i] : -1;
}

struct AsmArgs2 {
  const float *feat, *pinv;
  const int32_t *ind, *grid;
  const uint8_t *mask;
  const int32_t *pos;
  const float *img;
  const float *const *img_ptrs;
  const float *att;
  int n, C, Ci, ncam, H, W, max_ne;
  float *v_feat, *v_i_feat, *qgrid, *qpts, *qpos;
  const int32_t *pixrow;
  const float *compact;
};

__global__ __launch_bounds__(256) void assemble_queries2_kernel(AsmArgs2 a) {
  long long w = ((long long)blockIdx.x * blockDim.x + threadIdx.x) >> 6;
  int lane = threadIdx.x & 63;
  if (w >= (long long)a.n * a.ncam) return;
  int cam = (int)(w / a.n), i = (int)(w - (long long)cam * a.n);
  if (!a.mask[(size_t)cam * a.n + i]) return;
  int slot = a.pos[(size_t)cam * a.n + i];
  if (slot >= a.max_ne) return;
  int img = a.ind[(size_t)i * 4] * a.ncam + cam;
  size_t q = (size_t)img * a.max_ne + slot;
  int gx = a.grid[((size_t)cam * a.n + i) * 2], gy = a.grid[((size_t)cam * a.n + i) * 2 + 1];
  for (int c = lane; c < a.C; c += 64) a.v_feat[q * a.C + c] = a.feat[(size_t)i * a.C + c];
  size_t hw = (size_t)a.H * a.W;
  size_t pix = (size_t)gy * a.W + gx;
  float g = a.att ? a.att[(size_t)img * hw + pix] : 1.f;
  if (a.compact) {
    const float *src = a.compact + (size_t)a.pixrow[(size_t)img * hw + pix] * a.Ci;
    for (int c = lane; c < a.Ci; c += 64) a.v_i_feat[q * a.Ci + c] = src[c] * g;
  } else {
    const float *src = (a.img ? a.img + (size_t)img * a.Ci * hw : a.img_ptrs[img]) + pix;
    for (int c = lane; c < a.Ci; c += 64) a.v_i_feat[q * a.Ci + c] = src[(size_t)c * hw] * g;
  }
  if (lane == 0) {
    a.qgrid[q * 2 + 0] = (float)gx / (float)a.W;
    a.qgrid[q * 2 + 1] = (float)gy / (float)a.H;
  }
  if (lane < 3) a.qpts[q * 3 + lane] = a.pinv[(size_t)i * 3 + lane];
  if (a.qpos) {
    float d = a.pinv[(size_t)i * 3] / 60.f * 6.283185307179586f;
    for (int c = lane; c < a.C; c += 64) {
      float dim_t = powf(10000.f, (float)(2 * (c / 2)) / (float)a.C);
      float v = d / dim_t;
      a.qpos[q * a.C + c] = (c & 1) ? cosf(v) : sinf(v);
    }
  }
}

constexpr int ASM3_CH = 64;
__global__ __launch_bounds__(256) void assemble_queries3_kernel(AsmArgs2 a, const int32_t *__restrict__ counts) {
  __shared__ float tile[64][ASM3_CH + 1];
  __shared__ int rowL[64], pixL[64];
  __shared__ float gL[64];
  const int img = blockIdx.y, cam = img % a.ncam, b = img / a.ncam;
  const int cnt = counts[img] < a.max_ne ? counts[img] : a.max_ne;
  const int s0 = blockIdx.x * 64;
  if (s0 >= cnt) return;
  const int tid = threadIdx.x, lane = tid & 63, wave = tid >> 6;
  const size_t hw = (size_t)a.H * a.W;
  if (tid < 64) {
    int row = -1, pix = 0;
    float g = 0.f;
    const int s = s0 + tid;
    if (s < cnt) {
      int lo = 0, hi = a.n;
      while (lo < hi) {
        const int mid = (lo + hi) >> 1;
        if (a.ind[(size_t)mid * 4] < b) lo = mid + 1;
        else hi = mid;
      }
      int r0 = lo;
      hi = a.n;
      while (lo < hi) {
        const int mid = (lo + hi) >> 1;
        if (a.ind[(size_t)mid * 4] < b + 1) lo = mid + 1;
        else hi = mid;
      }
      int r1 = lo;
      const int32_t *pc = a.pos + (size_t)cam * a.n;
      const uint8_t *mc = a.mask + (size_t)cam * a.n;
      lo = r0, hi = r1;
      while (lo < hi) {
        const int mid = (lo + hi) >> 1;
        if (pc[mid] <= s) lo = mid + 1;
        else hi = mid;
      }
      row = lo - 1;
      if (!mc[row]) row = -1;
      if (row >= 0) {
        const int gx = a.grid[((size_t)cam * a.n + row) * 2], gy = a.grid[((size_t)cam * a.n + row) * 2 + 1];
        pix = gy * a.W + gx;
        g = a.att ? a.att[(size_t)img * hw + pix] : 1.f;
      }
      if (row >= 0 && blockIdx.z == 0) {
        const int gx = a.grid[((size_t)cam * a.n + row) * 2], gy = a.grid[((size_t)cam * a.n + row) * 2 + 1];
        const size_t q = (size_t)img * a.max_ne + s;
        a.qgrid[q * 2 + 0] = (float)gx / (float)a.W;
        a.qgrid[q * 2 + 1] = (float)gy / (float)a.H;
        a.qpts[q * 3 + 0] = a.pinv[(size_t)row * 3 + 0];
        a.qpts[q * 3 + 1] = a.pinv[(size_t)row * 3 + 1];
        a.qpts[q * 3 + 2] = a.pinv[(size_t)row * 3 + 2];
      }
    }
    rowL[tid] = row;
    pixL[tid] = pix;
    gL[tid] = g;
  }
  __syncthreads();
  const float *base = a.img ? a.img + (size_t)img * a.Ci * hw : a.img_ptrs[img];
  for (int c0 = blockIdx.z * ASM3_CH; c0 < a.Ci; c0 += gridDim.z * ASM3_CH) {
    const int myrow = rowL[lane];
    const float g = gL[lane];
    const float *src = base + pixL[lane];
#pragma unroll 4
    for (int c = wave; c < ASM3_CH; c += 4)
      tile[lane][c] = (myrow >= 0 && c0 + c < a.Ci) ? src[(size_t)(c0 + c) * hw] * g : 0.f;
    __syncthreads();
    for (int r = wave; r < 64; r += 4) {
      if (rowL[r] < 0 || c0 + lane >= a.Ci) continue;
      a.v_i_feat[((size_t)img * a.max_ne + s0 + r) * a.Ci + c0 + lane] = tile[r][lane];
    }
    __syncthreads();
  }
  if (blockIdx.z != 0) return;
  for (int r = wave; r < 64; r += 4) {
    const int row = rowL[r];
    if (row < 0) continue;
    const size_t q = (size_t)img * a.max_ne + s0 + r;
    for (int c = lane; c < a.C; c += 64) a.v_feat[q * a.C + c] = a.feat[(size_t)row * a.C + c];
    if (a.qpos) {
      const float d = a.pinv[(size_t)row * 3] / 60.f * 6.283185307179586f;
      for (int c = lane; c < a.C; c += 64) {
        const float dim_t = powf(10000.f, (float)(2 * (c / 2)) / (float)a.C);
        const float v = d / dim_t;
        a.qpos[q * a.C + c] = (c & 1) ? cosf(v) : sinf(v);
      }
    }
  }
}

__global__ __launch_bounds__(256) void qpos_pad_kernel(float *__restrict__ qpos, size_t n) {
  size_t i = (size_t)blockIdx.x * blockDim.x + threadIdx.x;
  if (i < n) qpos[i] = (i & 1) ? 1.f : 0.f;
}

__global__ __launch_bounds__(1024) void query_slots_kernel(const uint8_t *__restrict__ mask,
                                                           const int32_t *__restrict__ ind, int n, int ncam,
                                                           int32_t *__restrict__ pos, int32_t *__restrict__ counts) {
  const int cam = blockIdx.x, b = blockIdx.y;
  const int tid = threadIdx.x, lane = tid & 63, wave = tid >> 6;
  __shared__ int range[2];
  __shared__ int wsum[16];
  __shared__ int carry;
  if (tid < 2) {
    int key = b + tid, lo = 0, hi = n;
    while (lo < hi) {
      int mid = (lo + hi) >> 1;
      if (ind[(size_t)mid * 4] < key) lo = mid + 1;
      else hi = mid;
    }
    range[tid] = lo;
  }
  if (tid == 0) carry = 0;
  __syncthreads();
  const int r0 = range[0], r1 = range[1];
  const uint8_t *m = mask + (size_t)cam * n;
  for (int base = r0; base < r1; base += 1024) {
    int r = base + tid;
    bool v = r < r1 && m[r] != 0;
    unsigned long long bal = __ballot(v);
    int within = __popcll(bal & ((1ull << lane) - 1ull));
    if (lane == 0) wsum[wave] = __popcll(bal);
    __syncthreads();
    int off = carry;
    for (int w = 0; w < wave; ++w) off += wsum[w];
    if (r < r1) pos[(size_t)cam * n + r] = off + within;
    __syncthreads();
    if (tid == 0) {
      int t = 0;
      for (int w = 0; w < 16; ++w) t += wsum[w];
      carry += t;
    }
    __syncthreads();
  }
  if (tid == 0) counts[b * ncam + cam] = carry;
}

__global__ __launch_bounds__(256) void query_inverse_kernel(const int32_t *__restrict__ ind, const uint8_t *__restrict__ mask,
                                                            const int32_t *__restrict__ pos, const int32_t *__restrict__ grid,
                                                            const int32_t *__restrict__ pixrow, int n, int ncam, int max_ne,
                                                            int H, int W, int4 *__restrict__ inv) {
  long long t = (long long)blockIdx.x * blockDim.x + threadIdx.x;
  if (t >= (long long)n * ncam) return;
  const int cam = (int)(t / n), i = (int)(t - (long long)cam * n);
  if (!mask[t]) return;
  const int slot = pos[t];
  if (slot >= max_ne) return;
  const int img = ind[(size_t)i * 4] * ncam + cam;
  const int gx = grid[(size_t)t * 2], gy = grid[(size_t)t * 2 + 1];
  const int pr = pixrow ? pixrow[(size_t)img * H * W + (size_t)gy * W + gx] : -1;
  inv[(size_t)img * max_ne + slot] = make_int4(i, gx, gy, pr);
}

__global__ __launch_bounds__(256) void assemble_queries4_kernel(AsmArgs2 a, const int32_t *__restrict__ counts,
                                                                const int4 *__restrict__ inv, int nimg) {
  const long long w = ((long long)blockIdx.x * blockDim.x + threadIdx.x) >> 6;
  const int lane = threadIdx.x & 63;
  if (w >= (long long)nimg * a.max_ne) return;
  const int img = (int)(w / a.max_ne), slot = (int)(w - (long long)img * a.max_ne);
  const size_t q = (size_t)w;
  if (slot >= counts[img]) {
    for (int c = lane; c < a.C; c += 64) {
      a.v_feat[q * a.C + c] = 0.f;
      if (a.qpos) a.qpos[q * a.C + c] = (c & 1) ? 1.f : 0.f;
    }
    for (int c = lane; c < a.Ci; c += 64) a.v_i_feat[q * a.Ci + c] = 0.f;
    if (lane < 2) a.qgrid[q * 2 + lane] = 0.f;
    if (lane < 3) a.qpts[q * 3 + lane] = 0.f;
    return;
  }
  const int4 e = inv[q];
  const int i = e.x, gx = e.y, gy = e.z;
  const size_t hw = (size_t)a.H * a.W, pix = (size_t)gy * a.W + gx;
  float vf[4], vi[8];
#pragma unroll
  for (int j = 0; j < 4; ++j) vf[j] = (lane + 64 * j < a.C) ? a.feat[(size_t)i * a.C + lane + 64 * j] : 0.f;
  if (a.compact) {
    const float *src = a.compact + (size_t)e.w * a.Ci;
#pragma unroll
    for (int j = 0; j < 8; ++j) vi[j] = (lane + 64 * j < a.Ci) ? src[lane + 64 * j] : 0.f;
  } else {
    const float *src = (a.img ? a.img + (size_t)img * a.Ci * hw : a.img_ptrs[img]) + pix;
#pragma unroll
    for (int j = 0; j < 8; ++j) vi[j] = (lane + 64 * j < a.Ci) ? src[(size_t)(lane + 64 * j) * hw] : 0.f;
  }
  const float g = a.att ? a.att[(size_t)img * hw + pix] : 1.f;
  const float p0 = a.pinv[(size_t)i * 3], pl = lane < 3 ? a.pinv[(size_t)i * 3 + lane] : 0.f;
#pragma unroll
  for (int j = 0; j < 4; ++j)
    if (lane + 64 * j < a.C) a.v_feat[q * a.C + lane + 64 * j] = vf[j];
#pragma unroll
  for (int j = 0; j < 8; ++j)
    if (lane + 64 * j < a.Ci) a.v_i_feat[q * a.Ci + lane + 64 * j] = vi[j] * g;
  if (lane == 0) {
    a.qgrid[q * 2 + 0] = (float)gx / (float)a.W;
    a.qgrid[q * 2 + 1] = (float)gy / (float)a.H;
  }
  if (lane < 3) a.qpts[q * 3 + lane] = pl;
  if (a.qpos) {
    const float d = p0 / 60.f * 6.283185307179586f;
    for (int c = lane; c < a.C; c += 64) {
      float dim_t = powf(10000.f, (float)(2 * (c / 2)) / (float)a.C);
      float v = d / dim_t;
      a.qpos[q * a.C + c] = (c & 1) ? cosf(v) : sinf(v);
    }
  }
}

__global__ __launch_bounds__(256) void pad_queries_kernel(const int32_t *__restrict__ counts, int nimg, int max_ne, int C,
                                                          int Ci, float *__restrict__ v_feat,
                                                          float *__restrict__ v_i_feat, float *__restrict__ qgrid,
                                                          float *__restrict__ qpts, float *__restrict__ qpos) {
  long long w = ((long long)blockIdx.x * blockDim.x + threadIdx.x) >> 6;
  int lane = threadIdx.x & 63;
  if (w >= (long long)nimg * max_ne) return;
  int img = (int)(w / max_ne), slot = (int)(w - (long long)img * max_ne);
  if (slot < counts[img]) return;
  size_t q = (size_t)w;
  for (int c = lane; c < C; c += 64) {
    v_feat[q * C + c] = 0.f;
    if (qpos) qpos[q * C + c] = (c & 1) ? 1.f : 0.f;
  }
  for (int c = lane; c < Ci; c += 64) v_i_feat[q * Ci + c] = 0.f;
  if (lane < 2) qgrid[q * 2 + lane] = 0.f;
  if (lane < 3) qpts[q * 3 + lane] = 0.f;
}

}

extern "C" int df3d_gate_scatter(const float *s9, const int32_t *indices, const int32_t *grid_xy, const uint8_t *mask,
                                 int n, int batch, int ncam, int H, int W, int32_t *winner, float *S, int clear,
                                 void *stream_) {
  hipStream_t stream = (hipStream_t)stream_;
  DF3D_CHECK_ARG(winner && S, "gate_scatter: null output");
  size_t nimg = (size_t)batch * ncam;
  if (clear) DF3D_HIP(hipMemsetAsync(S, 0, nimg * 9 * (size_t)H * W * sizeof(float), stream));
  DF3D_HIP(hipMemsetAsync(winner, 0xff, nimg * H * W * sizeof(int32_t), stream));
  if (n == 0) return DF3D_OK;
  DF3D_CHECK_ARG(s9 && indices && grid_xy && mask, "gate_scatter: null input");
  ScatArgs a = {nullptr, nullptr, indices, grid_xy, mask, n, 0, ncam, H, W, winner, nullptr};
  dim3 g(cdiv((long long)n * ncam, 256));
  hipLaunchKernelGGL(scatter_winner_kernel, g, dim3(256), 0, stream, a);
  hipLaunchKernelGGL(gate_scatter_kernel, g, dim3(256), 0, stream, s9, indices, grid_xy, mask, winner, n, ncam, H, W, S);
  DF3D_LAUNCH_CHECK();
  return DF3D_OK;
}

extern "C" int df3d_gate_scatter_rows(const float *features, int channels, const float *point_inv, const float *T,
                                      const int32_t *indices, const int32_t *grid_xy, const uint8_t *mask, int n, int batch,
                                      int ncam, int H, int W, int32_t *winner, float *S, int clear, void *stream_) {
  hipStream_t stream = (hipStream_t)stream_;
  DF3D_CHECK_ARG(winner && S, "gate_scatter_rows: null output");
  DF3D_CHECK_ARG(channels > 0 && channels % 4 == 0 && channels <= 1024, "gate_scatter_rows: %d channels", channels);
  size_t nimg = (size_t)batch * ncam;
  DF3D_HIP(hipMemsetAsync(winner, 0xff, nimg * H * W * sizeof(int32_t), stream));
  if (n == 0) {
    if (clear) DF3D_HIP(hipMemsetAsync(S, 0, nimg * 9 * (size_t)H * W * sizeof(float), stream));
    return DF3D_OK;
  }
  DF3D_CHECK_ARG(features && point_inv && T && indices && grid_xy && mask, "gate_scatter_rows: null input");
  DF3D_CHECK_ARG((long long)H * W < 0x7fffffffLL, "gate_scatter_rows: map size");
  ScatArgs a = {nullptr, nullptr, indices, grid_xy, mask, n, 0, ncam, H, W, winner, nullptr};
  hipLaunchKernelGGL(scatter_winner_kernel, dim3(cdiv((long long)n * ncam, 256)), dim3(256), 0, stream, a);
  const long long npix = (long long)nimg * H * W;
  hipLaunchKernelGGL(gate_scatter_rows_kernel, dim3(cdiv(npix, 256)), dim3(256), (size_t)(channels + 3) * 9 * sizeof(float),
                     stream, features, channels, point_inv, T, winner, npix, H * W, clear, S);
  DF3D_LAUNCH_CHECK();
  return DF3D_OK;
}

extern "C" int df3d_gate_rows(const float *features, int channels, const float *point_inv, const float *T, const int32_t *winner,
                              int nimg, int H, int W, float *S, int clear, void *stream_) {
  hipStream_t stream = (hipStream_t)stream_;
  DF3D_CHECK_ARG(features && point_inv && T && winner && S, "gate_rows: null argument");
  DF3D_CHECK_ARG(channels > 0 && channels % 4 == 0 && channels <= 1024, "gate_rows: %d channels", channels);
  DF3D_CHECK_ARG((long long)H * W < 0x7fffffffLL, "gate_rows: map size");
  const long long npix = (long long)nimg * H * W;
  if (npix == 0) return DF3D_OK;
  hipLaunchKernelGGL(gate_scatter_rows_kernel, dim3(cdiv(npix, 256)), dim3(256), (size_t)(channels + 3) * 9 * sizeof(float),
                     stream, features, channels, point_inv, T, winner, npix, H * W, clear, S);
  DF3D_LAUNCH_CHECK();
  return DF3D_OK;
}

extern "C" int df3d_gate_finish_bias(const float *gate, const float *gate_bias, const float *S, const float *kg, int nimg, int H,
                                     int W, float *att, void *stream_) {
  hipStream_t stream = (hipStream_t)stream_;
  DF3D_CHECK_ARG(gate && gate_bias && S && kg && att, "gate_finish_bias: null argument");
  long long tot = (long long)nimg * H * W;
  if (tot == 0) return DF3D_OK;
  hipLaunchKernelGGL(gate_finish_kernel<true>, dim3(cdiv(tot, 256)), dim3(256), 0, stream, gate, gate_bias, S, kg, nimg, H, W, att);
  DF3D_LAUNCH_CHECK();
  return DF3D_OK;
}

extern "C" int df3d_fusion_writeback_split(const float *features, const float *enh, const int32_t *indices, const uint8_t *mask,
                                           const int32_t *pos, int n, int channels, int ncam, int max_ne, float *out,
                                           void *out_split, void *stream_) {
  hipStream_t stream = (hipStream_t)stream_;
  DF3D_CHECK_ARG(out && channels > 0 && channels % 8 == 0, "fusion_writeback_split: channels must be a multiple of 8");
  if (n == 0) return DF3D_OK;
  DF3D_CHECK_ARG(features && enh && indices && mask && pos, "fusion_writeback_split: null input");
  hipLaunchKernelGGL(writeback8_kernel, dim3(cdiv((long long)n * (channels / 8), 256)), dim3(256), 0, stream, features, enh,
                     indices, mask, pos, n, channels, ncam, max_ne, out, (u32x4 *)out_split);
  DF3D_LAUNCH_CHECK();
  return DF3D_OK;
}

extern "C" int df3d_gate_finish(const float *gate, const float *S, const float *kg, int nimg, int H, int W, float *att,
                                void *stream_) {
  hipStream_t stream = (hipStream_t)stream_;
  DF3D_CHECK_ARG(gate && S && kg && att, "gate_finish: null argument");
  long long tot = (long long)nimg * H * W;
  if (tot == 0) return DF3D_OK;
  hipLaunchKernelGGL(gate_finish_kernel<false>, dim3(cdiv(tot, 256)), dim3(256), 0, stream, gate, (const float *)nullptr, S, kg,
                     nimg, H, W, att);
  DF3D_LAUNCH_CHECK();
  return DF3D_OK;
}

static int assemble_queries2_impl(const float *features, const float *point_inv, const int32_t *indices,
                                  const int32_t *grid_xy, const uint8_t *mask, const int32_t *pos,
                                  const float *img_feats, const float *const *img_ptrs, const float *att, int n,
                                  int channels, int img_channels, int batch, int ncam, int H, int W, int max_ne,
                                  float *v_feat, float *v_i_feat, float *qgrid, float *qpts, float *qpos,
                                  const int32_t *counts, const int32_t *pixrow, const float *compact, int32_t *inv,
                                  void *stream_) {
  hipStream_t stream = (hipStream_t)stream_;
  DF3D_CHECK_ARG(v_feat && v_i_feat && qgrid && qpts, "assemble_queries2: null output");
  size_t nq = (size_t)batch * ncam * max_ne;
  if (qpos) DF3D_CHECK_ARG(channels % 2 == 0, "assemble_queries2: odd channel count");
  if (inv && counts && nq && n && channels <= 256 && img_channels <= 512) {
    DF3D_CHECK_ARG(features && point_inv && indices && grid_xy && mask && pos && (img_feats || img_ptrs || (compact && pixrow)),
                   "assemble_queries2: null input");
    AsmArgs2 a = {features, point_inv, indices, grid_xy, mask, pos, img_feats, img_ptrs, att, n, channels, img_channels, ncam, H, W,
                  max_ne, v_feat, v_i_feat, qgrid, qpts, qpos, pixrow, compact};
    hipLaunchKernelGGL(query_inverse_kernel, dim3(cdiv((long long)n * ncam, 256)), dim3(256), 0, stream, indices, mask, pos,
                       grid_xy, compact ? pixrow : nullptr, n, ncam, max_ne, H, W, (int4 *)inv);
    hipLaunchKernelGGL(assemble_queries4_kernel, dim3(cdiv((long long)nq * 64, 256)), dim3(256), 0, stream, a, counts,
                       (const int4 *)inv, batch * ncam);
    DF3D_LAUNCH_CHECK();
    return DF3D_OK;
  }
  if (counts && nq) {
    hipLaunchKernelGGL(pad_queries_kernel, dim3(cdiv((long long)nq * 64, 256)), dim3(256), 0, stream, counts,
                       batch * ncam, max_ne, channels, img_channels, v_feat, v_i_feat, qgrid, qpts, qpos);
  } else {
    DF3D_HIP(hipMemsetAsync(v_feat, 0, nq * channels * sizeof(float), stream));
    DF3D_HIP(hipMemsetAsync(v_i_feat, 0, nq * img_channels * sizeof(float), stream));
    DF3D_HIP(hipMemsetAsync(qgrid, 0, nq * 2 * sizeof(float), stream));
    DF3D_HIP(hipMemsetAsync(qpts, 0, nq * 3 * sizeof(float), stream));
    if (qpos && nq) {
      size_t tot = nq * channels;
      hipLaunchKernelGGL(qpos_pad_kernel, dim3(cdiv((long long)tot, 256)), dim3(256), 0, stream, qpos, tot);
    }
  }
  if (n == 0 || max_ne == 0) return DF3D_OK;
  DF3D_CHECK_ARG(features && point_inv && indices && grid_xy && mask && pos && (img_feats || img_ptrs || compact),
                 "assemble_queries2: null input");
  AsmArgs2 a = {features, point_inv, indices, grid_xy, mask, pos, img_feats, img_ptrs, att, n, channels, img_channels, ncam, H, W,
                max_ne, v_feat, v_i_feat, qgrid, qpts, qpos, pixrow, compact};
  if (compact) {
    hipLaunchKernelGGL(assemble_queries2_kernel, dim3(cdiv((long long)n * ncam * 64, 256)), dim3(256), 0, stream, a);
    DF3D_LAUNCH_CHECK();
    return DF3D_OK;
  }
  static const int forced = getenv("DF3D_ASSEMBLE") ? atoi(getenv("DF3D_ASSEMBLE")) : 0;
  const bool by_slot = forced == 1 || (forced != 2 && batch * ncam >= 12);
  if (counts && by_slot)
    hipLaunchKernelGGL(assemble_queries3_kernel, dim3(cdiv(max_ne, 64), batch * ncam, cdiv(img_channels, ASM3_CH)), dim3(256), 0, stream, a, counts);
  else
    hipLaunchKernelGGL(assemble_queries2_kernel, dim3(cdiv((long long)n * ncam * 64, 256)), dim3(256), 0, stream, a);
  DF3D_LAUNCH_CHECK();
  return DF3D_OK;
}

extern "C" int df3d_assemble_queries2(const float *features, const float *point_inv, const int32_t *indices,
                                      const int32_t *grid_xy, const uint8_t *mask, const int32_t *pos,
                                      const float *img_feats, const float *const *img_ptrs, const float *att, int n,
                                      int channels, int img_channels, int batch, int ncam, int H, int W, int max_ne,
                                      float *v_feat, float *v_i_feat, float *qgrid, float *qpts, float *qpos,
                                      const int32_t *counts, void *stream_) {
  return assemble_queries2_impl(features, point_inv, indices, grid_xy, mask, pos, img_feats, img_ptrs, att, n, channels,
                                img_channels, batch, ncam, H, W, max_ne, v_feat, v_i_feat, qgrid, qpts, qpos, counts, nullptr,
                                nullptr, nullptr, stream_);
}

extern "C" int df3d_assemble_queries2_slots(const float *features, const float *point_inv, const int32_t *indices,
                                            const int32_t *grid_xy, const uint8_t *mask, const int32_t *pos,
                                            const float *img_feats, const float *const *img_ptrs, const float *att, int n,
                                            int channels, int img_channels, int batch, int ncam, int H, int W, int max_ne,
                                            float *v_feat, float *v_i_feat, float *qgrid, float *qpts, float *qpos,
                                            const int32_t *counts, int32_t *slot_rows, const int32_t *pixrow,
                                            const float *compact, void *stream_) {
  DF3D_CHECK_ARG(counts && slot_rows, "assemble_queries2_slots: the list lengths and the table scratch are required");
  DF3D_CHECK_ARG((pixrow != nullptr) == (compact != nullptr), "assemble_queries2_slots: pixrow and compact come together");
  return assemble_queries2_impl(features, point_inv, indices, grid_xy, mask, pos, img_feats, img_ptrs, att, n, channels,
                                img_channels, batch, ncam, H, W, max_ne, v_feat, v_i_feat, qgrid, qpts, qpos, counts, pixrow,
                                compact, slot_rows, stream_);
}

extern "C" int df3d_assemble_queries2_compact(const float *features, const float *point_inv, const int32_t *indices,
                                              const int32_t *grid_xy, const uint8_t *mask, const int32_t *pos,
                                              const int32_t *pixrow, const float *compact, const float *att, int n, int channels,
                                              int img_channels, int batch, int ncam, int H, int W, int max_ne, float *v_feat,
                                              float *v_i_feat, float *qgrid, float *qpts, float *qpos, const int32_t *counts,
                                              void *stream_) {
  DF3D_CHECK_ARG(pixrow && compact, "assemble_queries2_compact: null pixel rows");
  return assemble_queries2_impl(features, point_inv, indices, grid_xy, mask, pos, nullptr, nullptr, att, n, channels,
                                img_channels, batch, ncam, H, W, max_ne, v_feat, v_i_feat, qgrid, qpts, qpos, counts, pixrow,
                                compact, nullptr, stream_);
}

static size_t df3d_query_pixel_rows_workspace_bytes_impl(long long npix) {
  return align_up((size_t)npix * 4, 256) * 2 + scan_scratch_bytes((size_t)npix) + 256;
}

extern "C" size_t df3d_query_pixel_rows_workspace_bytes(int batch, int ncam, int H, int W) {
  return df3d_query_pixel_rows_workspace_bytes_impl((long long)batch * ncam * H * W);
}

extern "C" int df3d_query_pixel_rows(const int32_t *indices, const int32_t *grid_xy, const uint8_t *mask, int n, int batch,
                                     int ncam, int H, int W, int32_t *pixrow, int32_t *total, void *workspace,
                                     size_t workspace_bytes, void *stream_) {
  hipStream_t stream = (hipStream_t)stream_;
  DF3D_CHECK_ARG(pixrow && total && workspace && batch > 0 && ncam > 0 && H > 0 && W > 0, "query_pixel_rows: bad arguments");
  const long long npix = (long long)batch * ncam * H * W;
  DF3D_CHECK_ARG(workspace_bytes >= df3d_query_pixel_rows_workspace_bytes_impl(npix), "query_pixel_rows: workspace too small");
  char *ws = (char *)workspace;
  uint32_t *flag = (uint32_t *)ws;
  uint32_t *rank = (uint32_t *)(ws + align_up((size_t)npix * 4, 256));
  void *scratch = ws + 2 * align_up((size_t)npix * 4, 256);
  DF3D_HIP(hipMemsetAsync(flag, 0, (size_t)npix * 4, stream));
  if (n > 0) {
    DF3D_CHECK_ARG(indices && grid_xy && mask, "query_pixel_rows: null input");
    hipLaunchKernelGGL(mark_query_pixels_kernel, dim3(cdiv((long long)n * ncam, 256)), dim3(256), 0, stream, indices, grid_xy, mask,
                       n, ncam, H, W, flag);
  }
  int rc = exclusive_scan_u32(flag, rank, (size_t)npix, (uint32_t *)total, scratch, scan_scratch_bytes((size_t)npix), stream);
  if (rc) return rc;
  hipLaunchKernelGGL(pixrow_kernel, dim3(cdiv(npix, 256)), dim3(256), 0, stream, flag, rank, (size_t)npix, pixrow);
  DF3D_LAUNCH_CHECK();
  return DF3D_OK;
}

extern "C" int df3d_query_slots(const uint8_t *mask, const int32_t *indices, int n, int batch, int ncam, int32_t *pos,
                                int32_t *counts, void *stream_) {
  hipStream_t stream = (hipStream_t)stream_;
  DF3D_CHECK_ARG(counts && batch > 0 && ncam > 0, "query_slots: bad arguments");
  if (n == 0) {
    DF3D_HIP(hipMemsetAsync(counts, 0, (size_t)batch * ncam * sizeof(int32_t), stream));
    return DF3D_OK;
  }
  DF3D_CHECK_ARG(mask && indices && pos, "query_slots: null argument");
  hipLaunchKernelGGL(query_slots_kernel, dim3(ncam, batch), dim3(1024), 0, stream, mask, indices, n, ncam, pos, counts);
  DF3D_LAUNCH_CHECK();
  return DF3D_OK;
}

namespace df3d {
__global__ __launch_bounds__(256) void chanfirst_dot_kernel(const float *__restrict__ x, const float *__restrict__ g, int C,
                                                            long long S, float *__restrict__ out) {
  typedef float f4 __attribute__((ext_vector_type(4)));
  const int row = blockIdx.x, n = row / C;
  const float *xr = x + (size_t)row * S, *gr = g + (size_t)n * S;
  float acc = 0.f;
  const bool vec = (S % 4 == 0) && (((size_t)xr | (size_t)gr) % 16 == 0);
  if (vec) {
    for (long long i = threadIdx.x; i < S / 4; i += 256) {
      const f4 a = ((const f4 *)xr)[i], b = ((const f4 *)gr)[i];
      acc += (a[0] * b[0] + a[1] * b[1]) + (a[2] * b[2] + a[3] * b[3]);
    }
  } else {
    for (long long i = threadIdx.x; i < S; i += 256) acc += xr[i] * gr[i];
  }
  __shared__ float red[256];
  red[threadIdx.x] = acc;
  __syncthreads();
  for (int w = 128; w > 0; w >>= 1) {
    if ((int)threadIdx.x < w) red[threadIdx.x] += red[threadIdx.x + w];
    __syncthreads();
  }
  if (threadIdx.x == 0) out[row] = red[0];
}
}

extern "C" int df3d_chanfirst_dot(const float *x, const float *g, int nmaps, int channels, long long S, float *out, void *stream_) {
  hipStream_t stream = (hipStream_t)stream_;
  DF3D_CHECK_ARG(nmaps >= 0 && channels > 0 && S >= 0, "chanfirst_dot: bad sizes");
  if (nmaps == 0) return DF3D_OK;
  DF3D_CHECK_ARG(x && g && out, "chanfirst_dot: null argument");
  hipLaunchKernelGGL(df3d::chanfirst_dot_kernel, dim3(nmaps * channels), dim3(256), 0, stream, x, g, channels, S, out);
  DF3D_LAUNCH_CHECK();
  return DF3D_OK;
}
```

### 3d-dual-fusion_amd/csrc/rulebook.hip

```cpp
#include "common.h"

namespace df3d {

GridHeader grid_layout(int batch, const int *shape) {
  GridHeader h;
  h.batch = batch;
  h.shape[0] = shape[0];
  h.shape[1] = shape[1];
  h.shape[2] = shape[2];
  h.ncells = (unsigned long long)batch * shape[0] * shape[1] * shape[2];
  h.nwords = (h.ncells + 63) / 64;
  size_t off = align_up(sizeof(GridHeader), 256);
  h.off_bits = off;
  off = align_up(off + h.nwords * 8, 256);
  h.off_prefix = off;
  off = align_up(off + h.nwords * 4, 256);
  h.off_total = off;
  off = align_up(off + 64, 256);
  h.off_scratch = off;
  h.scratch_bytes = scan_scratch_bytes(h.nwords);
  return h;
}

struct Shape3 {
  int v[3];
};

__global__ __launch_bounds__(256) void grid_setbits_kernel(const int32_t *__restrict__ ind, int n, Shape3 shp,
                                                           long long vol, unsigned long long *__restrict__ bits) {
  int i = blockIdx.x * blockDim.x + threadIdx.x;
  if (i >= n) return;
  const int32_t *p = ind + (size_t)i * 4;
  long long flat = (long long)p[0] * vol + ((long long)p[1] * shp.v[1] + p[2]) * shp.v[2] + p[3];
  atomicOr(&bits[flat >> 6], 1ull << (flat & 63));
}

__global__ __launch_bounds__(256) void grid_perm_kernel(const int32_t *__restrict__ ind, int n, GridView g,
                                                        int32_t *__restrict__ perm) {
  int i = blockIdx.x * blockDim.x + threadIdx.x;
  if (i >= n) return;
  const int32_t *p = ind + (size_t)i * 4;
  long long flat = (long long)p[0] * g.vol + ((long long)p[1] * g.shape[1] + p[2]) * g.shape[2] + p[3];
  perm[grid_rank(g, flat)] = i;
}

struct ConvGeom {
  int ks[3], st[3], pad[3], dil[3];
  int in_shape[3], out_shape[3];
  int K;
};

__global__ __launch_bounds__(256) void neighbors_kernel(GridView g, const int32_t *__restrict__ perm,
                                                        const int32_t *__restrict__ out_ind, int n, ConvGeom cg,
                                                        int32_t *__restrict__ nbr) {
  long long t = (long long)blockIdx.x * blockDim.x + threadIdx.x;
  if (t >= (long long)n * cg.K) return;
  int k = (int)(t / n);
  int o = (int)(t - (long long)k * n);
  const int32_t *p = out_ind + (size_t)o * 4;
  int kx = k % cg.ks[2];
  int kt = k / cg.ks[2];
  int ky = kt % cg.ks[1];
  int kz = kt / cg.ks[1];
  int z = p[1] * cg.st[0] - cg.pad[0] + kz * cg.dil[0];
  int y = p[2] * cg.st[1] - cg.pad[1] + ky * cg.dil[1];
  int x = p[3] * cg.st[2] - cg.pad[2] + kx * cg.dil[2];
  int r = -1;
  if (z >= 0 && z < g.shape[0] && y >= 0 && y < g.shape[1] && x >= 0 && x < g.shape[2]) {
    long long flat = (long long)p[0] * g.vol + ((long long)z * g.shape[1] + y) * g.shape[2] + x;
    r = grid_rank(g, flat);
    if (r >= 0 && perm) r = perm[r];
  }
  nbr[t] = r;
}

__global__ __launch_bounds__(256) void conv_mark_kernel(const int32_t *__restrict__ ind, int n, ConvGeom cg,
                                                        long long out_vol, unsigned long long *__restrict__ bits) {
  const int KZY = cg.ks[0] * cg.ks[1];
  long long t = (long long)blockIdx.x * blockDim.x + threadIdx.x;
  if (t >= (long long)n * KZY) return;
  int i = (int)(t / KZY);
  int kzy = (int)(t - (long long)i * KZY);
  const int32_t *p = ind + (size_t)i * 4;
  int kk[2] = {kzy / cg.ks[1], kzy % cg.ks[1]};
  int o[2];
#pragma unroll
  for (int d = 0; d < 2; ++d) {
    int num = p[1 + d] + cg.pad[d] - kk[d] * cg.dil[d];
    if (num < 0 || (num % cg.st[d]) != 0) return;
    o[d] = num / cg.st[d];
    if (o[d] >= cg.out_shape[d]) return;
  }
  const long long row = (long long)p[0] * out_vol + ((long long)o[0] * cg.out_shape[1] + o[1]) * cg.out_shape[2];
  long long cur = -1;
  unsigned long long mask = 0ull;
  for (int kx = 0; kx < cg.ks[2]; ++kx) {
    int num = p[3] + cg.pad[2] - kx * cg.dil[2];
    if (num < 0 || (num % cg.st[2]) != 0) continue;
    int ox = num / cg.st[2];
    if (ox >= cg.out_shape[2]) continue;
    long long flat = row + ox;
    if ((flat >> 6) != cur) {
      if (mask) atomicOr(&bits[cur], mask);
      cur = flat >> 6;
      mask = 0ull;
    }
    mask |= 1ull << (flat & 63);
  }
  if (mask) atomicOr(&bits[cur], mask);
}

__global__ __launch_bounds__(256) void conv_mark_transpose_kernel(const int32_t *__restrict__ ind, int n, ConvGeom cg,
                                                                  long long out_vol,
                                                                  unsigned long long *__restrict__ bits) {
  const int KZY = cg.ks[0] * cg.ks[1];
  long long t = (long long)blockIdx.x * blockDim.x + threadIdx.x;
  if (t >= (long long)n * KZY) return;
  int i = (int)(t / KZY);
  int kzy = (int)(t - (long long)i * KZY);
  const int32_t *p = ind + (size_t)i * 4;
  int kk[2] = {kzy / cg.ks[1], kzy % cg.ks[1]};
  int o[2];
#pragma unroll
  for (int d = 0; d < 2; ++d) {
    o[d] = p[1 + d] * cg.st[d] - cg.pad[d] + kk[d] * cg.dil[d];
    if (o[d] < 0 || o[d] >= cg.out_shape[d]) return;
  }
  const long long row = (long long)p[0] * out_vol + ((long long)o[0] * cg.out_shape[1] + o[1]) * cg.out_shape[2];
  long long cur = -1;
  unsigned long long mask = 0ull;
  for (int kx = 0; kx < cg.ks[2]; ++kx) {
    int ox = p[3] * cg.st[2] - cg.pad[2] + kx * cg.dil[2];
    if (ox < 0 || ox >= cg.out_shape[2]) continue;
    long long flat = row + ox;
    if ((flat >> 6) != cur) {
      if (mask) atomicOr(&bits[cur], mask);
      cur = flat >> 6;
      mask = 0ull;
    }
    mask |= 1ull << (flat & 63);
  }
  if (mask) atomicOr(&bits[cur], mask);
}

__global__ __launch_bounds__(256) void neighbors_transpose_kernel(GridView g, const int32_t *__restrict__ perm,
                                                                  const int32_t *__restrict__ out_ind, int n, ConvGeom cg,
                                                                  int32_t *__restrict__ nbr) {
  long long t = (long long)blockIdx.x * blockDim.x + threadIdx.x;
  if (t >= (long long)n * cg.K) return;
  int k = (int)(t / n);
  int o = (int)(t - (long long)k * n);
  const int32_t *p = out_ind + (size_t)o * 4;
  int c[3];
  c[2] = k % cg.ks[2];
  int kt = k / cg.ks[2];
  c[1] = kt % cg.ks[1];
  c[0] = kt / cg.ks[1];
  int in[3];
  bool ok = true;
#pragma unroll
  for (int d = 0; d < 3; ++d) {
    int num = p[1 + d] + cg.pad[d] - c[d] * cg.dil[d];
    if (num < 0 || (num % cg.st[d]) != 0) ok = false;
    in[d] = num / cg.st[d];
    if (in[d] >= g.shape[d]) ok = false;
  }
  int r = -1;
  if (ok) {
    long long flat = (long long)p[0] * g.vol + ((long long)in[0] * g.shape[1] + in[1]) * g.shape[2] + in[2];
    r = grid_rank(g, flat);
    if (r >= 0 && perm) r = perm[r];
  }
  nbr[t] = r;
}

__global__ __launch_bounds__(256) void grid_enumerate_kernel(GridView g, unsigned long long nwords,
                                                             int32_t *__restrict__ out_ind, int cap) {
  unsigned long long w = (unsigned long long)blockIdx.x * blockDim.x + threadIdx.x;
  if (w >= nwords) return;
  unsigned long long bits = g.bits[w];
  if (!bits) return;
  uint32_t r = g.prefix[w];
  const long long flat0 = (long long)(w << 6);
  const long long yx = (long long)g.shape[1] * g.shape[2];
  int bb = (int)(flat0 / g.vol);
  long long rem = flat0 - (long long)bb * g.vol;
  int z = (int)(rem / yx);
  rem -= (long long)z * yx;
  int y = (int)(rem / g.shape[2]);
  int x = (int)(rem - (long long)y * g.shape[2]);
  int prev = 0;
  while (bits) {
    int b = __ffsll((long long)bits) - 1;
    bits &= bits - 1;
    x += b - prev;
    prev = b;
    while (x >= g.shape[2]) {
      x -= g.shape[2];
      if (++y == g.shape[1]) {
        y = 0;
        if (++z == g.shape[0]) {
          z = 0;
          ++bb;
        }
      }
    }
    if ((int)r < cap) *(int4 *)(out_ind + (size_t)r * 4) = make_int4(bb, z, y, x);
    ++r;
  }
}

__global__ __launch_bounds__(256) void nbr_flag_kernel(const int32_t *__restrict__ nbr, size_t n,
                                                       uint32_t *__restrict__ flag) {
  size_t i = (size_t)blockIdx.x * blockDim.x + threadIdx.x;
  if (i < n) flag[i] = nbr[i] >= 0 ? 1u : 0u;
}

__global__ __launch_bounds__(256) void nbr_compact_kernel(const int32_t *__restrict__ nbr,
                                                          const uint32_t *__restrict__ excl, int K, int n_out,
                                                          int n_in, const uint32_t *__restrict__ total, int32_t *__restrict__ pairs,
                                                          int32_t *__restrict__ num) {
  size_t t = (size_t)blockIdx.x * blockDim.x + threadIdx.x;
  size_t n = (size_t)K * n_out;
  if (t >= n) return;
  int k = (int)(t / n_out);
  int o = (int)(t - (size_t)k * n_out);
  uint32_t seg0 = excl[(size_t)k * n_out];
  int v = nbr[t];
  if (v >= 0) {
    uint32_t j = excl[t] - seg0;
    if ((int)j < n_in) {
      pairs[((size_t)k * 2 + 0) * n_in + j] = v;
      pairs[((size_t)k * 2 + 1) * n_in + j] = o;
    }
  }
  if (o == 0) {
    uint32_t seg1 = (k + 1 < K) ? excl[(size_t)(k + 1) * n_out] : *total;
    num[k] = (int32_t)(seg1 - seg0);
  }
}

struct NumArr {
  int v[DF3D_MAX_KVOL];
};
__global__ __launch_bounds__(256) void pairs_to_nbr_kernel(const int32_t *__restrict__ pairs, NumArr num, int K,
                                                           int n_in, int n_out, int32_t *__restrict__ nbr) {
  size_t t = (size_t)blockIdx.x * blockDim.x + threadIdx.x;
  if (t >= (size_t)K * n_in) return;
  int k = (int)(t / n_in);
  int j = (int)(t - (size_t)k * n_in);
  if (j >= num.v[k]) return;
  int i = pairs[((size_t)k * 2 + 0) * n_in + j];
  int o = pairs[((size_t)k * 2 + 1) * n_in + j];
  if (o >= 0 && o < n_out) nbr[(size_t)k * n_out + o] = i;
}

static int fill_geom(ConvGeom &cg, const int *ks, const int *st, const int *pad, const int *dil, const int *in_shape,
                     const int *out_shape) {
  cg.K = 1;
  for (int d = 0; d < 3; ++d) {
    cg.ks[d] = ks[d];
    cg.st[d] = st ? st[d] : 1;
    cg.pad[d] = pad ? pad[d] : ks[d] / 2;
    cg.dil[d] = dil ? dil[d] : 1;
    cg.in_shape[d] = in_shape ? in_shape[d] : 0;
    cg.out_shape[d] = out_shape ? out_shape[d] : 0;
    cg.K *= ks[d];
  }
  return cg.K;
}

}

using namespace df3d;

extern "C" size_t df3d_grid_bytes(int batch, const int *shape) {
  if (batch <= 0 || !shape || shape[0] <= 0 || shape[1] <= 0 || shape[2] <= 0) return 0;
  GridHeader h = grid_layout(batch, shape);
  return h.off_scratch + h.scratch_bytes + 256;
}

static int grid_finish(void *grid, const GridHeader &h, hipStream_t stream) {
  unsigned long long *bits = (unsigned long long *)((char *)grid + h.off_bits);
  uint32_t *prefix = (uint32_t *)((char *)grid + h.off_prefix);
  uint32_t *total = (uint32_t *)((char *)grid + h.off_total);
  return exclusive_scan_popc64(bits, prefix, (size_t)h.nwords, total, (char *)grid + h.off_scratch, h.scratch_bytes,
                               stream);
}

extern "C" int df3d_grid_build(const int32_t *indices, int n, int batch, const int *shape, void *grid,
                               size_t grid_bytes, int32_t *perm, void *stream_) {
  hipStream_t stream = (hipStream_t)stream_;
  DF3D_CHECK_ARG(batch > 0 && shape && n >= 0, "grid_build: bad arguments");
  GridHeader h = grid_layout(batch, shape);
  if (grid_bytes < h.off_scratch + h.scratch_bytes) {
    set_error("grid_build: grid blob too small (%zu < %zu)", grid_bytes, h.off_scratch + h.scratch_bytes);
    return DF3D_ENOMEM;
  }
  unsigned long long *bits = (unsigned long long *)((char *)grid + h.off_bits);
  DF3D_HIP(hipMemsetAsync(bits, 0, (size_t)h.nwords * 8, stream));
  Shape3 s3 = {{shape[0], shape[1], shape[2]}};
  long long vol = (long long)shape[0] * shape[1] * shape[2];
  if (n > 0)
    hipLaunchKernelGGL(grid_setbits_kernel, dim3(cdiv(n, 256)), dim3(256), 0, stream, indices, n, s3, vol, bits);
  int rc = grid_finish(grid, h, stream);
  if (rc) return rc;
  if (perm && n > 0) {
    GridView g = grid_view(grid, h);
    hipLaunchKernelGGL(grid_perm_kernel, dim3(cdiv(n, 256)), dim3(256), 0, stream, indices, n, g, perm);
  }
  DF3D_LAUNCH_CHECK();
  return DF3D_OK;
}

extern "C" int df3d_subm_neighbors(const void *grid, const int32_t *perm, const int32_t *indices, int n, int batch,
                                   const int *shape, const int *ksize, const int *dilation, int32_t *nbr,
                                   void *stream_) {
  hipStream_t stream = (hipStream_t)stream_;
  DF3D_CHECK_ARG(grid && indices && nbr && shape && ksize, "subm_neighbors: null argument");
  ConvGeom cg;
  int K = fill_geom(cg, ksize, nullptr, nullptr, dilation, shape, shape);
  DF3D_CHECK_ARG(K <= DF3D_MAX_KVOL, "subm_neighbors: kernel volume %d > %d", K, DF3D_MAX_KVOL);
  for (int d = 0; d < 3; ++d) {
    DF3D_CHECK_ARG(ksize[d] % 2 == 1, "subm_neighbors: even kernel size");
    cg.pad[d] = (ksize[d] / 2) * cg.dil[d];
    DF3D_CHECK_ARG(cg.dil[d] == 1, "subm_neighbors: dilation != 1 is not supported");
  }
  if (n == 0) return DF3D_OK;
  GridHeader h = grid_layout(batch, shape);
  GridView g = grid_view(grid, h);
  long long total = (long long)n * K;
  hipLaunchKernelGGL(neighbors_kernel, dim3(cdiv(total, 256)), dim3(256), 0, stream, g, perm, indices, n, cg, nbr);
  DF3D_LAUNCH_CHECK();
  return DF3D_OK;
}

extern "C" int df3d_conv_out_indices(const int32_t *indices, int n, int batch, const int *in_shape,
                                     const int *out_shape, const int *ksize, const int *stride, const int *padding,
                                     const int *dilation, void *out_grid, size_t out_grid_bytes,
                                     int32_t *out_indices, int out_cap, int32_t *num_out, void *stream_) {
  hipStream_t stream = (hipStream_t)stream_;
  DF3D_CHECK_ARG(indices && out_grid && out_indices && num_out, "conv_out_indices: null argument");
  ConvGeom cg;
  int K = fill_geom(cg, ksize, stride, padding, dilation, in_shape, out_shape);
  DF3D_CHECK_ARG(K <= DF3D_MAX_KVOL, "conv_out_indices: kernel volume %d > %d", K, DF3D_MAX_KVOL);
  for (int d = 0; d < 3; ++d) DF3D_CHECK_ARG(cg.dil[d] == 1 && cg.st[d] >= 1, "conv_out_indices: dilation != 1");
  GridHeader h = grid_layout(batch, out_shape);
  if (out_grid_bytes < h.off_scratch + h.scratch_bytes) {
    set_error("conv_out_indices: grid blob too small");
    return DF3D_ENOMEM;
  }
  unsigned long long *bits = (unsigned long long *)((char *)out_grid + h.off_bits);
  DF3D_HIP(hipMemsetAsync(bits, 0, (size_t)h.nwords * 8, stream));
  long long out_vol = (long long)out_shape[0] * out_shape[1] * out_shape[2];
  if (n > 0) {
    long long total = (long long)n * cg.ks[0] * cg.ks[1];
    hipLaunchKernelGGL(conv_mark_kernel, dim3(cdiv(total, 256)), dim3(256), 0, stream, indices, n, cg, out_vol, bits);
  }
  int rc = grid_finish(out_grid, h, stream);
  if (rc) return rc;
  GridView g = grid_view(out_grid, h);
  hipLaunchKernelGGL(grid_enumerate_kernel, dim3(cdiv((long long)h.nwords, 256)), dim3(256), 0, stream, g, h.nwords,
                     out_indices, out_cap);
  DF3D_HIP(hipMemcpyAsync(num_out, (char *)out_grid + h.off_total, sizeof(int32_t), hipMemcpyDeviceToDevice, stream));
  DF3D_LAUNCH_CHECK();
  return DF3D_OK;
}

extern "C" int df3d_conv_transpose_out_indices(const int32_t *indices, int n, int batch, const int *in_shape,
                                               const int *out_shape, const int *ksize, const int *stride,
                                               const int *padding, const int *dilation, void *out_grid,
                                               size_t out_grid_bytes, int32_t *out_indices, int out_cap,
                                               int32_t *num_out, void *stream_) {
  hipStream_t stream = (hipStream_t)stream_;
  DF3D_CHECK_ARG(indices && out_grid && out_indices && num_out, "conv_transpose_out_indices: null argument");
  ConvGeom cg;
  int K = fill_geom(cg, ksize, stride, padding, dilation, in_shape, out_shape);
  DF3D_CHECK_ARG(K <= DF3D_MAX_KVOL, "conv_transpose_out_indices: kernel volume %d > %d", K, DF3D_MAX_KVOL);
  for (int d = 0; d < 3; ++d) DF3D_CHECK_ARG(cg.dil[d] >= 1 && cg.st[d] >= 1, "conv_transpose_out_indices: bad stride / dilation");
  GridHeader h = grid_layout(batch, out_shape);
  if (out_grid_bytes < h.off_scratch + h.scratch_bytes) {
    set_error("conv_transpose_out_indices: grid blob too small");
    return DF3D_ENOMEM;
  }
  unsigned long long *bits = (unsigned long long *)((char *)out_grid + h.off_bits);
  DF3D_HIP(hipMemsetAsync(bits, 0, (size_t)h.nwords * 8, stream));
  long long out_vol = (long long)out_shape[0] * out_shape[1] * out_shape[2];
  if (n > 0) {
    long long total = (long long)n * cg.ks[0] * cg.ks[1];
    hipLaunchKernelGGL(conv_mark_transpose_kernel, dim3(cdiv(total, 256)), dim3(256), 0, stream, indices, n, cg, out_vol,
                       bits);
  }
  int rc = grid_finish(out_grid, h, stream);
  if (rc) return rc;
  GridView g = grid_view(out_grid, h);
  hipLaunchKernelGGL(grid_enumerate_kernel, dim3(cdiv((long long)h.nwords, 256)), dim3(256), 0, stream, g, h.nwords,
                     out_indices, out_cap);
  DF3D_HIP(hipMemcpyAsync(num_out, (char *)out_grid + h.off_total, sizeof(int32_t), hipMemcpyDeviceToDevice, stream));
  DF3D_LAUNCH_CHECK();
  return DF3D_OK;
}

extern "C" int df3d_conv_transpose_neighbors(const void *in_grid, const int32_t *in_perm, const int32_t *out_indices,
                                             int n_out, int batch, const int *in_shape, const int *ksize,
                                             const int *stride, const int *padding, const int *dilation, int32_t *nbr,
                                             void *stream_) {
  hipStream_t stream = (hipStream_t)stream_;
  DF3D_CHECK_ARG(in_grid && out_indices && nbr, "conv_transpose_neighbors: null argument");
  ConvGeom cg;
  int K = fill_geom(cg, ksize, stride, padding, dilation, in_shape, nullptr);
  DF3D_CHECK_ARG(K <= DF3D_MAX_KVOL, "conv_transpose_neighbors: kernel volume %d > %d", K, DF3D_MAX_KVOL);
  if (n_out == 0) return DF3D_OK;
  GridHeader h = grid_layout(batch, in_shape);
  GridView g = grid_view(in_grid, h);
  long long total = (long long)n_out * K;
  hipLaunchKernelGGL(neighbors_transpose_kernel, dim3(cdiv(total, 256)), dim3(256), 0, stream, g, in_perm, out_indices,
                     n_out, cg, nbr);
  DF3D_LAUNCH_CHECK();
  return DF3D_OK;
}

extern "C" int df3d_conv_neighbors(const void *in_grid, const int32_t *in_perm, const int32_t *out_indices,
                                   int n_out, int batch, const int *in_shape, const int *ksize, const int *stride,
                                   const int *padding, const int *dilation, int32_t *nbr, void *stream_) {
  hipStream_t stream = (hipStream_t)stream_;
  DF3D_CHECK_ARG(in_grid && out_indices && nbr, "conv_neighbors: null argument");
  ConvGeom cg;
  int K = fill_geom(cg, ksize, stride, padding, dilation, in_shape, nullptr);
  DF3D_CHECK_ARG(K <= DF3D_MAX_KVOL, "conv_neighbors: kernel volume %d > %d", K, DF3D_MAX_KVOL);
  if (n_out == 0) return DF3D_OK;
  GridHeader h = grid_layout(batch, in_shape);
  GridView g = grid_view(in_grid, h);
  long long total = (long long)n_out * K;
  hipLaunchKernelGGL(neighbors_kernel, dim3(cdiv(total, 256)), dim3(256), 0, stream, g, in_perm, out_indices, n_out,
                     cg, nbr);
  DF3D_LAUNCH_CHECK();
  return DF3D_OK;
}

extern "C" size_t df3d_nbr_to_pairs_workspace_bytes(int kvol, int n_out) {
  size_t n = (size_t)kvol * (size_t)n_out;
  size_t b = 0;
  b = arena_need(b, n * 4);
  b = arena_need(b, 64);
  b = arena_need(b, scan_scratch_bytes(n));
  return b + 256;
}

extern "C" int df3d_nbr_to_pairs(const int32_t *nbr, int kvol, int n_out, int n_in, int32_t *indice_pairs,
                                 int32_t *indice_num, void *workspace, size_t workspace_bytes, void *stream_) {
  hipStream_t stream = (hipStream_t)stream_;
  DF3D_CHECK_ARG(nbr && indice_pairs && indice_num && kvol > 0 && kvol <= DF3D_MAX_KVOL, "nbr_to_pairs: bad args");
  DF3D_HIP(hipMemsetAsync(indice_pairs, 0xff, (size_t)kvol * 2 * (size_t)n_in * 4, stream));
  DF3D_HIP(hipMemsetAsync(indice_num, 0, (size_t)kvol * 4, stream));
  size_t n = (size_t)kvol * n_out;
  if (n == 0) return DF3D_OK;
  Arena ar(workspace, workspace_bytes);
  uint32_t *excl = ar.take<uint32_t>(n);
  uint32_t *total = ar.take<uint32_t>(16);
  size_t ssz = scan_scratch_bytes(n);
  void *sscr = ar.take<char>(ssz);
  if (!sscr) {
    set_error("nbr_to_pairs: workspace too small");
    return DF3D_ENOMEM;
  }
  hipLaunchKernelGGL(nbr_flag_kernel, dim3(cdiv((long long)n, 256)), dim3(256), 0, stream, nbr, n, excl);
  int rc = exclusive_scan_u32(excl, excl, n, total, sscr, ssz, stream);
  if (rc) return rc;
  hipLaunchKernelGGL(nbr_compact_kernel, dim3(cdiv((long long)n, 256)), dim3(256), 0, stream, nbr, excl, kvol, n_out,
                     n_in, total, indice_pairs, indice_num);
  DF3D_LAUNCH_CHECK();
  return DF3D_OK;
}

extern "C" int df3d_pairs_to_nbr(const int32_t *indice_pairs, const int32_t *indice_num_host, int kvol, int n_in,
                                 int n_out, int32_t *nbr, void *stream_) {
  hipStream_t stream = (hipStream_t)stream_;
  DF3D_CHECK_ARG(indice_pairs && indice_num_host && nbr && kvol > 0 && kvol <= DF3D_MAX_KVOL, "pairs_to_nbr: bad args");
  DF3D_HIP(hipMemsetAsync(nbr, 0xff, (size_t)kvol * (size_t)n_out * 4, stream));
  if (n_in == 0 || n_out == 0) return DF3D_OK;
  NumArr na;
  for (int k = 0; k < DF3D_MAX_KVOL; ++k) na.v[k] = k < kvol ? indice_num_host[k] : 0;
  size_t n = (size_t)kvol * n_in;
  hipLaunchKernelGGL(pairs_to_nbr_kernel, dim3(cdiv((long long)n, 256)), dim3(256), 0, stream, indice_pairs, na, kvol,
                     n_in, n_out, nbr);
  DF3D_LAUNCH_CHECK();
  return DF3D_OK;
}
```

### 3d-dual-fusion_amd/csrc/voxelize.hip

```cpp
#include "common.h"

namespace df3d {

struct VoxParams {
  float min[3], vs[3];
  int grid[3];
  int P, C, T, maxV, cap_mask;
  int batch_index;
};

__device__ __forceinline__ uint32_t hash_u32(uint32_t k) {
  k ^= k >> 16;
  k *= 0x85ebca6bu;
  k ^= k >> 13;
  k *= 0xc2b2ae35u;
  k ^= k >> 16;
  return k;
}

__global__ __launch_bounds__(256) void vox_insert_kernel(const float *__restrict__ pts, VoxParams p,
                                                         int *__restrict__ keys, int *__restrict__ first,
                                                         int *__restrict__ slot_of_point) {
  int i = blockIdx.x * blockDim.x + threadIdx.x;
  if (i >= p.P) return;
  const float *q = pts + (size_t)i * p.C;
  int c[3];
  bool ok = true;
#pragma unroll
  for (int j = 0; j < 3; ++j) {
    float f = floorf((q[j] - p.min[j]) / p.vs[j]);
    if (!(f >= 0.0f && f < (float)p.grid[j])) ok = false;
    c[j] = (int)f;
  }
  if (!ok) {
    slot_of_point[i] = -1;
    return;
  }
  int key = (c[2] * p.grid[1] + c[1]) * p.grid[0] + c[0];
  uint32_t s = hash_u32((uint32_t)key) & (uint32_t)p.cap_mask;
  while (true) {
    int prev = atomicCAS(&keys[s], -1, key);
    if (prev == -1 || prev == key) break;
    s = (s + 1) & (uint32_t)p.cap_mask;
  }
  atomicMin(&first[s], i);
  slot_of_point[i] = (int)s;
}

__global__ __launch_bounds__(256) void vox_flag_kernel(int P, const int *__restrict__ first,
                                                       const int *__restrict__ slot_of_point,
                                                       uint32_t *__restrict__ flag) {
  int i = blockIdx.x * blockDim.x + threadIdx.x;
  if (i >= P) return;
  int s = slot_of_point[i];
  flag[i] = (s >= 0 && first[s] == i) ? 1u : 0u;
}

__global__ __launch_bounds__(256) void vox_number_kernel(VoxParams p, const int *__restrict__ keys,
                                                         const int *__restrict__ first,
                                                         const int *__restrict__ slot_of_point,
                                                         const uint32_t *__restrict__ rank, int *__restrict__ vid,
                                                         int32_t *__restrict__ coors, int *__restrict__ misc,
                                                         int32_t *__restrict__ voxel_num) {
  int i = blockIdx.x * blockDim.x + threadIdx.x;
  if (i == 0) {
    int tot = misc[0];
    int n = tot < p.maxV ? tot : p.maxV;
    misc[2] = n;
    *voxel_num = n;
  }
  if (i >= p.P) return;
  int s = slot_of_point[i];
  if (s < 0 || first[s] != i) return;
  int r = (int)rank[i];
  vid[s] = r;
  if (r == p.maxV) misc[1] = i;
  if (r < p.maxV) {
    int key = keys[s];
    int x = key % p.grid[0];
    int t = key / p.grid[0];
    int y = t % p.grid[1];
    int z = t / p.grid[1];
    if (p.batch_index >= 0) {
      *(int4 *)(coors + (size_t)r * 4) = make_int4(p.batch_index, z, y, x);
    } else {
      coors[r * 3 + 0] = z;
      coors[r * 3 + 1] = y;
      coors[r * 3 + 2] = x;
    }
  }
}

__global__ __launch_bounds__(256) void vox_assign_kernel(VoxParams p, int break_at_cap,
                                                         const int *__restrict__ slot_of_point,
                                                         const int *__restrict__ vid, const int *__restrict__ misc,
                                                         int *__restrict__ count, int *__restrict__ ptlist) {
  int i = blockIdx.x * blockDim.x + threadIdx.x;
  if (i >= p.P) return;
  int s = slot_of_point[i];
  if (s < 0) return;
  int v = vid[s];
  if (v >= p.maxV) return;
  if (break_at_cap && i >= misc[1]) return;
  atomicAdd(&count[v], 1);
  int *lst = ptlist + (size_t)v * p.T;
  int x = i;
  for (int t = 0; t < p.T; ++t) {
    int old = atomicMin(&lst[t], x);
    if (old == 0x7f7f7f7f) break;
    x = old > x ? old : x;
  }
}

__global__ __launch_bounds__(256) void vox_gather_kernel(const float *__restrict__ pts, VoxParams p,
                                                         const int *__restrict__ misc, const int *__restrict__ count,
                                                         const int *__restrict__ ptlist, float *__restrict__ voxels,
                                                         int32_t *__restrict__ num, float *__restrict__ mean) {
  int v = blockIdx.x * blockDim.x + threadIdx.x;
  if (v >= misc[2]) return;
  int n = count[v];
  if (n > p.T) n = p.T;
  num[v] = n;
  const int *lst = ptlist + (size_t)v * p.T;
  for (int c = 0; c < p.C; ++c) {
    float acc = 0.f;
    for (int t = 0; t < p.T; ++t) {
      float x = 0.f;
      if (t < n) x = pts[(size_t)lst[t] * p.C + c];
      if (voxels) voxels[((size_t)v * p.T + t) * p.C + c] = x;
      acc += x;
    }
    if (mean) mean[(size_t)v * p.C + c] = acc / (float)n;
  }
}

static int table_capacity(int P) {
  int cap = 1024;
  while (cap < 2 * P) cap <<= 1;
  return cap;
}

__global__ __launch_bounds__(256) void vox_init_kernel(int *__restrict__ keys, size_t n_keys, int *__restrict__ first,
                                                       size_t n_first, int *__restrict__ count, size_t n_count,
                                                       int *__restrict__ ptlist, size_t n_pt, int *__restrict__ misc) {
  const size_t total = n_keys + n_first + n_count + n_pt + 16;
  const size_t i0 = ((size_t)blockIdx.x * 256 + threadIdx.x) * 4;
  for (int e = 0; e < 4; ++e) {
    size_t j = i0 + e;
    if (j >= total) return;
    if (j < n_keys) {
      keys[j] = -1;
      continue;
    }
    j -= n_keys;
    if (j < n_first) {
      first[j] = 0x7f7f7f7f;
      continue;
    }
    j -= n_first;
    if (j < n_count) {
      count[j] = 0;
      continue;
    }
    j -= n_count;
    if (j < n_pt) {
      ptlist[j] = 0x7f7f7f7f;
      continue;
    }
    misc[j - n_pt] = 0x7f7f7f7f;
  }
}

}

using namespace df3d;

extern "C" size_t df3d_hard_voxelize_workspace_bytes(int num_points, int max_points, int max_voxels) {
  if (num_points < 0) return 0;
  if (max_voxels < 0 || max_voxels > num_points) max_voxels = num_points;
  size_t cap = (size_t)table_capacity(num_points);
  size_t b = 0;
  b = arena_need(b, cap * 4);
  b = arena_need(b, cap * 4);
  b = arena_need(b, cap * 4);
  b = arena_need(b, (size_t)num_points * 4);
  b = arena_need(b, (size_t)num_points * 4);
  b = arena_need(b, (size_t)max_voxels * 4);
  b = arena_need(b, (size_t)max_voxels * (size_t)(max_points > 0 ? max_points : 1) * 4);
  b = arena_need(b, 64);
  b = arena_need(b, scan_scratch_bytes((size_t)num_points));
  return b + 256;
}

static int hard_voxelize_impl(const float *points, int num_points, int num_features, const float *voxel_size,
                              const float *coors_range, int max_points, int max_voxels, int break_at_cap,
                              float *voxels, int32_t *coors, int batch_index, int32_t *num_points_per_voxel,
                              float *mean, int32_t *voxel_num, void *workspace, size_t workspace_bytes,
                              void *stream_);

extern "C" int df3d_hard_voxelize(const float *points, int num_points, int num_features,
                                  const float *voxel_size, const float *coors_range, int max_points,
                                  int max_voxels, int break_at_cap, float *voxels, int32_t *coors,
                                  int32_t *num_points_per_voxel, float *mean, int32_t *voxel_num,
                                  void *workspace, size_t workspace_bytes, void *stream_) {
  return hard_voxelize_impl(points, num_points, num_features, voxel_size, coors_range, max_points, max_voxels,
                            break_at_cap, voxels, coors, -1, num_points_per_voxel, mean, voxel_num, workspace,
                            workspace_bytes, stream_);
}

extern "C" int df3d_hard_voxelize_batched(const float *points, int num_points, int num_features,
                                          const float *voxel_size, const float *coors_range, int max_points,
                                          int max_voxels, int break_at_cap, int batch_index, float *voxels,
                                          int32_t *coors4, int32_t *num_points_per_voxel, float *mean,
                                          int32_t *voxel_num, void *workspace, size_t workspace_bytes, void *stream_) {
  DF3D_CHECK_ARG(batch_index >= 0, "hard_voxelize_batched: negative batch index");
  return hard_voxelize_impl(points, num_points, num_features, voxel_size, coors_range, max_points, max_voxels,
                            break_at_cap, voxels, coors4, batch_index, num_points_per_voxel, mean, voxel_num, workspace,
                            workspace_bytes, stream_);
}

static int hard_voxelize_impl(const float *points, int num_points, int num_features, const float *voxel_size,
                              const float *coors_range, int max_points, int max_voxels, int break_at_cap,
                              float *voxels, int32_t *coors, int batch_index, int32_t *num_points_per_voxel,
                              float *mean, int32_t *voxel_num, void *workspace, size_t workspace_bytes,
                              void *stream_) {
  hipStream_t stream = (hipStream_t)stream_;
  DF3D_CHECK_ARG(num_points >= 0 && num_features >= 3, "hard_voxelize: need points [P,C>=3]");
  DF3D_CHECK_ARG(max_points > 0, "hard_voxelize: max_points must be > 0 (got %d)", max_points);
  DF3D_CHECK_ARG(coors && num_points_per_voxel && voxel_num, "hard_voxelize: null output");
  if (max_voxels < 0 || max_voxels > num_points) max_voxels = num_points;
  VoxParams p;
  long long vol = 1;
  for (int i = 0; i < 3; ++i) {
    p.min[i] = coors_range[i];
    p.vs[i] = voxel_size[i];
    p.grid[i] = (int)roundf((coors_range[3 + i] - coors_range[i]) / voxel_size[i]);
    DF3D_CHECK_ARG(p.grid[i] > 0, "hard_voxelize: empty grid on axis %d", i);
    vol *= p.grid[i];
  }
  DF3D_CHECK_ARG(vol < 2147483647LL, "hard_voxelize: grid volume %lld overflows int32 keys", vol);
  p.P = num_points;
  p.C = num_features;
  p.T = max_points;
  p.maxV = max_voxels;
  p.batch_index = batch_index;
  if (num_points == 0) {
    DF3D_HIP(hipMemsetAsync(voxel_num, 0, sizeof(int32_t), stream));
    return DF3D_OK;
  }
  int cap = table_capacity(num_points);
  p.cap_mask = cap - 1;
  if (workspace_bytes < df3d_hard_voxelize_workspace_bytes(num_points, max_points, max_voxels)) {
    set_error("hard_voxelize: workspace too small");
    return DF3D_ENOMEM;
  }
  Arena ar(workspace, workspace_bytes);
  int *keys = ar.take<int>(cap);
  int *first = ar.take<int>(cap);
  int *vid = ar.take<int>(cap);
  int *slot = ar.take<int>(num_points);
  uint32_t *rank = ar.take<uint32_t>(num_points);
  int *count = ar.take<int>(max_voxels);
  int *ptlist = ar.take<int>((size_t)max_voxels * max_points);
  int *misc = ar.take<int>(16);
  size_t ssz = scan_scratch_bytes((size_t)num_points);
  void *sscr = ar.take<char>(ssz);
  if (!sscr) {
    set_error("hard_voxelize: workspace too small");
    return DF3D_ENOMEM;
  }
  {
    const size_t n_keys = (size_t)cap, n_first = (size_t)cap, n_count = (size_t)max_voxels,
                 n_pt = (size_t)max_voxels * max_points, total = n_keys + n_first + n_count + n_pt + 16;
    hipLaunchKernelGGL(vox_init_kernel, dim3(cdiv((long long)((total + 3) / 4), 256)), dim3(256), 0, stream, keys, n_keys,
                       first, n_first, count, n_count, ptlist, n_pt, misc);
  }
  int nb = cdiv(num_points, 256);
  hipLaunchKernelGGL(vox_insert_kernel, dim3(nb), dim3(256), 0, stream, points, p, keys, first, slot);
  hipLaunchKernelGGL(vox_flag_kernel, dim3(nb), dim3(256), 0, stream, num_points, first, slot, rank);
  int rc = exclusive_scan_u32(rank, rank, (size_t)num_points, (uint32_t *)misc, sscr, ssz, stream);
  if (rc) return rc;
  hipLaunchKernelGGL(vox_number_kernel, dim3(nb), dim3(256), 0, stream, p, keys, first, slot, rank, vid, coors, misc,
                     voxel_num);
  hipLaunchKernelGGL(vox_assign_kernel, dim3(nb), dim3(256), 0, stream, p, break_at_cap, slot, vid, misc, count,
                     ptlist);
  hipLaunchKernelGGL(vox_gather_kernel, dim3(cdiv(max_voxels, 256)), dim3(256), 0, stream, points, p, misc, count,
                     ptlist, voxels, num_points_per_voxel, mean);
  DF3D_LAUNCH_CHECK();
  return DF3D_OK;
}
```

Measured before the change: 362.2.

## Cut launch count: batched grid zeroing, single-block scans, fused voxel flag scan

Adds a multi-range fill kernel that clears every grid bitmap the backbone will need in one launch ahead of time, so per-layer grid builds skip their own memsets. Scans of up to 32K elements now run as one 1024-thread block instead of tile plus offset kernels, with 16 items per thread and vectorised loads and stores. The voxelizer's flag kernel is folded into the scan loader. Neighbour kernels take a centre index and launch over only the first two kernel dimensions. The aim is fewer small launches and memsets on a latency-bound pipeline, at the cost of a single-block scan with limited parallelism and more complex code.

```diff
diff --git a/3d-dual-fusion_amd/csrc/common.h b/3d-dual-fusion_amd/csrc/common.h
--- a/3d-dual-fusion_amd/csrc/common.h
+++ b/3d-dual-fusion_amd/csrc/common.h
@@ -163,12 +163,21 @@
 };
 static inline size_t arena_need(size_t cur, size_t bytes) { return align_up(cur, 256) + bytes; }
 
+struct FillRange {
+  void *p;
+  size_t words;
+  uint32_t value;
+};
+int fill_ranges(const FillRange *ranges, int count, hipStream_t stream);
+
 size_t scan_scratch_bytes(size_t n);
 int exclusive_scan_u32(const uint32_t *in, uint32_t *out, size_t n, uint32_t *total,
                        void *scratch, size_t scratch_bytes, hipStream_t stream);
 int exclusive_scan_popc64(const unsigned long long *words, uint32_t *out, size_t n,
                           uint32_t *total, void *scratch, size_t scratch_bytes,
                           hipStream_t stream);
+int exclusive_scan_first_flag(const int *first, const int *slot_of_point, uint32_t *out, size_t n,
+                              uint32_t *total, void *scratch, size_t scratch_bytes, hipStream_t stream);
 
 struct GridHeader {
   int batch, shape[3];
@@ -201,6 +210,21 @@
   return (int)(g.prefix[flat >> 6] + __popcll(w & ((1ull << b) - 1ull)));
 }
 
+int zero_directories(int batch, const int (*shapes)[3], void *const *grids, int count, hipStream_t stream);
+int grid_build_on(const int32_t *indices, int n, int batch, const int *shape, void *grid, size_t grid_bytes, int32_t *perm,
+                  bool zero_bits, hipStream_t stream);
+int conv_out_indices_on(const int32_t *indices, int n, int batch, const int *in_shape, const int *out_shape,
+                        const int *ksize, const int *stride, const int *padding, const int *dilation, void *out_grid,
+                        size_t out_grid_bytes, int32_t *out_indices, int out_cap, int32_t *num_out, bool zero_bits,
+                        hipStream_t stream);
+const int32_t *grid_total_word(const void *grid, int batch, const int *shape);
+
+int scatter_winner_on(const int32_t *indices, const int32_t *grid_xy, const uint8_t *mask, int n, int batch, int ncam, int H,
+                      int W, int32_t *winner, bool fill, hipStream_t stream);
+int query_pixel_rows_on(const int32_t *indices, const int32_t *grid_xy, const uint8_t *mask, int n, int batch, int ncam, int H,
+                        int W, int32_t *pixrow, int32_t *total, void *workspace, size_t workspace_bytes, bool zero_flags,
+                        hipStream_t stream);
+
 size_t conv_operand_packed_bytes(int parts, int kvol, int cin, int cout);
 int conv_operand_rows(int parts, const float *x, long long n, int c, void *rows, hipStream_t stream);
 int conv_operand_run(int parts, const void *in, int n_in, int cin, const void *packed, int kvol, int cout, const int32_t *nbr,
diff --git a/3d-dual-fusion_amd/csrc/common.hip b/3d-dual-fusion_amd/csrc/common.hip
--- a/3d-dual-fusion_amd/csrc/common.hip
+++ b/3d-dual-fusion_amd/csrc/common.hip
@@ -53,18 +53,123 @@
   if (g_ovf_n < 64) g_ovf_sym[g_ovf_n] = symbol, g_ovf_tu[g_ovf_n] = tu, ++g_ovf_n;
 }
 
+constexpr int FILL_MAX_RANGES = 8;
+struct FillArgs {
+  uint32_t *p[FILL_MAX_RANGES];
+  unsigned long long words[FILL_MAX_RANGES];
+  unsigned long long end[FILL_MAX_RANGES];
+  uint32_t value[FILL_MAX_RANGES];
+  int count;
+};
+__global__ __launch_bounds__(256) void fill_ranges_kernel(FillArgs a) {
+  const unsigned long long t = (unsigned long long)blockIdx.x * blockDim.x + threadIdx.x;
+  unsigned long long begin = 0;
+  for (int i = 0; i < a.count; ++i) {
+    if (t < a.end[i]) {
+      const unsigned long long w = (t - begin) * 4;
+      const uint32_t v = a.value[i];
+      uint32_t *q = a.p[i] + w;
+      if (w + 4 <= a.words[i] && ((uintptr_t)a.p[i] & 15) == 0) {
+        *(uint4 *)q = make_uint4(v, v, v, v);
+      } else {
+        for (int e = 0; e < 4 && w + e < a.words[i]; ++e) q[e] = v;
+      }
+      return;
+    }
+    begin = a.end[i];
+  }
+}
+
+int fill_ranges(const FillRange *ranges, int count, hipStream_t stream) {
+  for (int at = 0; at < count; at += FILL_MAX_RANGES) {
+    FillArgs a;
+    unsigned long long end = 0;
+    a.count = 0;
+    for (int i = at; i < count && a.count < FILL_MAX_RANGES; ++i) {
+      if (!ranges[i].words) continue;
+      a.p[a.count] = (uint32_t *)ranges[i].p;
+      a.words[a.count] = ranges[i].words;
+      a.value[a.count] = ranges[i].value;
+      end += (ranges[i].words + 3) / 4;
+      a.end[a.count++] = end;
+    }
+    if (end) hipLaunchKernelGGL(fill_ranges_kernel, dim3(cdiv((long long)end, 256)), dim3(256), 0, stream, a);
+  }
+  DF3D_LAUNCH_CHECK();
+  return DF3D_OK;
+}
+
+constexpr int SCAN_TILE = 1024;
+constexpr int SCAN_SINGLE_MAX_TILES = 32;
+constexpr int SCAN_ITEMS = 16;
 constexpr int SCAN_THREADS = 256;
-constexpr int SCAN_ITEMS = 4;
-constexpr int SCAN_TILE = SCAN_THREADS * SCAN_ITEMS;
+constexpr int SCAN_WIDE_TILE = SCAN_THREADS * SCAN_ITEMS;
+constexpr int SCAN_SINGLE_THREADS = 1024;
+constexpr int SCAN_SINGLE_ROUND = SCAN_SINGLE_THREADS * SCAN_ITEMS;
+constexpr int SCAN_SINGLE_ROUNDS = SCAN_SINGLE_MAX_TILES * SCAN_TILE / SCAN_SINGLE_ROUND;
+static_assert(SCAN_SINGLE_ROUNDS * SCAN_SINGLE_ROUND == SCAN_SINGLE_MAX_TILES * SCAN_TILE, "whole rounds");
 
 struct LoadU32 {
   const uint32_t *p;
-  __device__ uint32_t operator()(size_t i) const { return p[i]; }
+  __device__ void load4(size_t i, size_t n, uint32_t *v) const {
+    if (i + 4 <= n && ((uintptr_t)p & 15) == 0) {
+      const uint4 q = *(const uint4 *)(p + i);
+      v[0] = q.x, v[1] = q.y, v[2] = q.z, v[3] = q.w;
+    } else {
+#pragma unroll
+      for (int e = 0; e < 4; ++e) v[e] = (i + e < n) ? p[i + e] : 0u;
+    }
+  }
 };
 struct LoadPopc {
   const unsigned long long *p;
-  __device__ uint32_t operator()(size_t i) const { return (uint32_t)__popcll(p[i]); }
+  __device__ void load4(size_t i, size_t n, uint32_t *v) const {
+    if (i + 4 <= n && ((uintptr_t)p & 15) == 0) {
+      const uint4 a = *(const uint4 *)(p + i), b = *(const uint4 *)(p + i + 2);
+      v[0] = __popc(a.x) + __popc(a.y), v[1] = __popc(a.z) + __popc(a.w);
+      v[2] = __popc(b.x) + __popc(b.y), v[3] = __popc(b.z) + __popc(b.w);
+    } else {
+#pragma unroll
+      for (int e = 0; e < 4; ++e) v[e] = (i + e < n) ? (uint32_t)__popcll(p[i + e]) : 0u;
+    }
+  }
 };
+struct LoadFirst {
+  const int *first, *slot;
+  __device__ void load4(size_t i, size_t n, uint32_t *v) const {
+    int s[4];
+    if (i + 4 <= n && ((uintptr_t)slot & 15) == 0) {
+      const int4 q = *(const int4 *)(slot + i);
+      s[0] = q.x, s[1] = q.y, s[2] = q.z, s[3] = q.w;
+    } else {
+#pragma unroll
+      for (int e = 0; e < 4; ++e) s[e] = (i + e < n) ? slot[i + e] : -1;
+    }
+#pragma unroll
+    for (int e = 0; e < 4; ++e) v[e] = (s[e] >= 0 && first[s[e]] == (int)(i + e)) ? 1u : 0u;
+  }
+};
+
+template <typename Loader>
+__device__ __forceinline__ void scan_load(const Loader &in, size_t base, size_t n, uint32_t (&x)[SCAN_ITEMS]) {
+#pragma unroll
+  for (int q = 0; q < SCAN_ITEMS; q += 4) {
+    if (base + q < n) in.load4(base + q, n, &x[q]);
+    else x[q] = x[q + 1] = x[q + 2] = x[q + 3] = 0u;
+  }
+}
+__device__ __forceinline__ void scan_store(uint32_t *out, size_t base, size_t n, const uint32_t (&x)[SCAN_ITEMS], uint32_t add) {
+#pragma unroll
+  for (int q = 0; q < SCAN_ITEMS; q += 4) {
+    if (base + q + 4 <= n && ((uintptr_t)out & 15) == 0) {
+      *(uint4 *)(out + base + q) = make_uint4(x[q] + add, x[q + 1] + add, x[q + 2] + add, x[q + 3] + add);
+    } else {
+#pragma unroll
+      for (int e = 0; e < 4; ++e)
+        if (base + q + e < n) out[base + q + e] = x[q + e] + add;
+    }
+  }
+}
 
 __device__ __forceinline__ uint32_t wave_incl_scan(uint32_t v, int lane) {
 #pragma unroll
@@ -75,8 +180,8 @@
   return v;
 }
 
-__device__ __forceinline__ void block_excl_scan(uint32_t (&x)[SCAN_ITEMS], uint32_t &total,
-                                                uint32_t *lds ) {
+template <int THREADS>
+__device__ __forceinline__ void block_excl_scan(uint32_t (&x)[SCAN_ITEMS], uint32_t &total, uint32_t *lds ) {
   int tid = threadIdx.x, lane = tid & 63, wave = tid >> 6;
   uint32_t s = 0;
 #pragma unroll
@@ -86,7 +191,7 @@
   __syncthreads();
   uint32_t woff = 0, tot = 0;
 #pragma unroll
-  for (int w = 0; w < SCAN_THREADS / 64; ++w) {
+  for (int w = 0; w < THREADS / 64; ++w) {
     uint32_t v = lds[w];
     if (w < wave) woff += v;
     tot += v;
@@ -103,22 +208,36 @@
 }
 
 template <typename Loader>
-__global__ __launch_bounds__(SCAN_THREADS) void scan_tiles_kernel(Loader in, uint32_t *out, size_t n,
-                                                                  uint32_t *sums, uint32_t *total_if_single) {
-  __shared__ uint32_t lds[SCAN_THREADS / 64 + 1];
-  size_t base = (size_t)blockIdx.x * SCAN_TILE + (size_t)threadIdx.x * SCAN_ITEMS;
+__global__ __launch_bounds__(SCAN_SINGLE_THREADS) void scan_single_kernel(Loader in, uint32_t *out, size_t n, uint32_t *total) {
+  __shared__ uint32_t lds[SCAN_SINGLE_THREADS / 64];
+  uint32_t x[SCAN_SINGLE_ROUNDS][SCAN_ITEMS];
+  const size_t base = (size_t)threadIdx.x * SCAN_ITEMS;
+#pragma unroll
+  for (int r = 0; r < SCAN_SINGLE_ROUNDS; ++r)
+    if ((size_t)r * SCAN_SINGLE_ROUND < n) scan_load(in, base + (size_t)r * SCAN_SINGLE_ROUND, n, x[r]);
+  uint32_t carry = 0;
+#pragma unroll
+  for (int r = 0; r < SCAN_SINGLE_ROUNDS; ++r) {
+    if ((size_t)r * SCAN_SINGLE_ROUND < n) {
+      uint32_t tot;
+      block_excl_scan<SCAN_SINGLE_THREADS>(x[r], tot, lds);
+      scan_store(out, base + (size_t)r * SCAN_SINGLE_ROUND, n, x[r], carry);
+      carry += tot;
+    }
+  }
+  if (threadIdx.x == 0 && total) *total = carry;
+}
+
+template <typename Loader>
+__global__ __launch_bounds__(SCAN_THREADS) void scan_tiles_kernel(Loader in, uint32_t *out, size_t n, uint32_t *sums) {
+  __shared__ uint32_t lds[SCAN_THREADS / 64];
+  size_t base = (size_t)blockIdx.x * SCAN_WIDE_TILE + (size_t)threadIdx.x * SCAN_ITEMS;
   uint32_t x[SCAN_ITEMS];
-#pragma unroll
-  for (int i = 0; i < SCAN_ITEMS; ++i) x[i] = (base + i < n) ? in(base + i) : 0u;
+  scan_load(in, base, n, x);
   uint32_t tot;
-  block_excl_scan(x, tot, lds);
-#pragma unroll
-  for (int i = 0; i < SCAN_ITEMS; ++i)
-    if (base + i < n) out[base + i] = x[i];
-  if (threadIdx.x == 0) {
-    sums[blockIdx.x] = tot;
-    if (total_if_single) *total_if_single = tot;
-  }
+  block_excl_scan<SCAN_THREADS>(x, tot, lds);
+  scan_store(out, base, n, x, 0u);
+  if (threadIdx.x == 0) sums[blockIdx.x] = tot;
 }
 
 __global__ __launch_bounds__(SCAN_THREADS) void scan_offset_kernel(uint32_t *out, size_t n, const uint32_t *sums, size_t nb,
@@ -156,10 +275,20 @@
   }
   __syncthreads();
   const uint32_t add = s_off;
-  size_t base = (size_t)blockIdx.x * SCAN_TILE + (size_t)threadIdx.x * SCAN_ITEMS;
-#pragma unroll
-  for (int i = 0; i < SCAN_ITEMS; ++i)
-    if (base + i < n) out[base + i] += add;
+  if (add == 0u) return;
+  size_t base = (size_t)blockIdx.x * SCAN_WIDE_TILE + (size_t)threadIdx.x * SCAN_ITEMS;
+#pragma unroll
+  for (int q = 0; q < SCAN_ITEMS; q += 4) {
+    if (base + q + 4 <= n && ((uintptr_t)out & 15) == 0) {
+      uint4 v = *(uint4 *)(out + base + q);
+      v.x += add, v.y += add, v.z += add, v.w += add;
+      *(uint4 *)(out + base + q) = v;
+    } else {
+#pragma unroll
+      for (int e = 0; e < 4; ++e)
+        if (base + q + e < n) out[base + q + e] += add;
+    }
+  }
 }
 
 size_t scan_scratch_bytes(size_t n) { return align_up((n / SCAN_TILE + 2) * sizeof(uint32_t), 256); }
@@ -175,12 +304,14 @@
     set_error("scan scratch too small");
     return DF3D_ENOMEM;
   }
-  uint32_t *sums = (uint32_t *)scratch;
-  size_t nb = (n + SCAN_TILE - 1) / SCAN_TILE;
-  hipLaunchKernelGGL(scan_tiles_kernel<Loader>, dim3((unsigned)nb), dim3(SCAN_THREADS), 0, stream, in, out, n, sums,
-                     nb == 1 ? total : (uint32_t *)nullptr);
-  if (nb > 1)
+  if (n <= (size_t)SCAN_SINGLE_MAX_TILES * SCAN_TILE) {
+    hipLaunchKernelGGL(scan_single_kernel<Loader>, dim3(1), dim3(SCAN_SINGLE_THREADS), 0, stream, in, out, n, total);
+  } else {
+    uint32_t *sums = (uint32_t *)scratch;
+    size_t nb = (n + SCAN_WIDE_TILE - 1) / SCAN_WIDE_TILE;
+    hipLaunchKernelGGL(scan_tiles_kernel<Loader>, dim3((unsigned)nb), dim3(SCAN_THREADS), 0, stream, in, out, n, sums);
     hipLaunchKernelGGL(scan_offset_kernel, dim3((unsigned)nb), dim3(SCAN_THREADS), 0, stream, out, n, sums, nb, total);
+  }
   DF3D_LAUNCH_CHECK();
   return DF3D_OK;
 }
@@ -192,6 +323,10 @@
 int exclusive_scan_popc64(const unsigned long long *words, uint32_t *out, size_t n, uint32_t *total,
                           void *scratch, size_t scratch_bytes, hipStream_t stream) {
   return scan_impl(LoadPopc{words}, out, n, total, scratch, scratch_bytes, stream);
+}
+int exclusive_scan_first_flag(const int *first, const int *slot_of_point, uint32_t *out, size_t n, uint32_t *total,
+                              void *scratch, size_t scratch_bytes, hipStream_t stream) {
+  return scan_impl(LoadFirst{first, slot_of_point}, out, n, total, scratch, scratch_bytes, stream);
 }
 
 }
diff --git a/3d-dual-fusion_amd/csrc/executor.hip b/3d-dual-fusion_amd/csrc/executor.hip
--- a/3d-dual-fusion_amd/csrc/executor.hip
+++ b/3d-dual-fusion_amd/csrc/executor.hip
@@ -7,6 +7,7 @@
 #include <mutex>
 #include <string>
 #include <thread>
+#include <array>
 #include <vector>
 
 #include "common.h"
@@ -94,7 +95,8 @@
   std::vector<int> layer_in_set;
   std::vector<char> need_f32;
   std::vector<char> want_split;
-  int32_t *count_dev = nullptr;
+  std::vector<void *> set_grid;
+  bool prepared = false;
   void *split0 = nullptr;
   void *rows16_0 = nullptr;
   hipEvent_t done = nullptr;
@@ -151,6 +153,57 @@
   return DF3D_OK;
 }
 
+void strided_out_shape(const df3d_layer &L, const int *in, int *out) {
+  for (int d = 0; d < 3; ++d) out[d] = (in[d] + 2 * L.padding[d] - L.dilation[d] * (L.ksize[d] - 1) - 1) / L.stride[d] + 1;
+}
+
+thread_local int32_t *g_count_host = nullptr;
+
+int geo_prepare(RunState &S, hipStream_t gstream) {
+  if (!g_count_host) DF3D_HIP(hipHostMalloc((void **)&g_count_host, 64, hipHostMallocDefault));
+  std::vector<std::array<int, 3>> shapes(1);
+  std::vector<char> need(1, 0);
+  memcpy(shapes[0].data(), S.shape, sizeof(S.shape));
+  std::vector<int> out_set(S.nlayers, 0);
+  std::vector<std::pair<int, int>> books;
+  for (int li = 0; li < S.nlayers; ++li) {
+    const df3d_layer &L = S.layers[li];
+    if (L.input >= li) break;
+    const int in_set = L.input < 0 ? 0 : out_set[L.input];
+    int os = -1;
+    if (L.rulebook >= 0)
+      for (auto &b : books)
+        if (b.first == L.rulebook) os = b.second;
+    if (os < 0) {
+      need[in_set] = 1;
+      if (L.kind == 0) {
+        os = in_set;
+      } else {
+        std::array<int, 3> o;
+        strided_out_shape(L, shapes[in_set].data(), o.data());
+        shapes.push_back(o);
+        need.push_back(1);
+        os = (int)shapes.size() - 1;
+      }
+      books.push_back(std::make_pair(L.rulebook, os));
+    }
+    out_set[li] = os;
+  }
+  S.set_grid.assign(shapes.size(), nullptr);
+  std::vector<void *> grids;
+  std::vector<std::array<int, 3>> gshapes;
+  for (size_t i = 0; i < shapes.size(); ++i) {
+    if (!need[i] || shapes[i][0] <= 0 || shapes[i][1] <= 0 || shapes[i][2] <= 0) continue;
+    void *g = S.gmem->take(df3d_grid_bytes(S.batch, shapes[i].data()));
+    if (!g) return DF3D_ENOMEM;
+    S.set_grid[i] = g;
+    grids.push_back(g);
+    gshapes.push_back(shapes[i]);
+  }
+  S.prepared = true;
+  return zero_directories(S.batch, (const int(*)[3])gshapes.data(), grids.data(), (int)grids.size(), gstream);
+}
+
 int geo_layer(RunState &S, int li, hipStream_t gstream, bool *new_table) {
   void *gs_ = (void *)gstream;
   Bump &mem = *S.gmem;
@@ -164,9 +217,9 @@
   DF3D_CHECK_ARG(cin == L.cin, "backbone_run: layer %d expects %d input channels, gets %d", li, L.cin, cin);
   const int K = kvol_of(L.ksize);
   DF3D_CHECK_ARG(K > 0 && K <= DF3D_MAX_KVOL, "backbone_run: layer %d kernel volume %d unsupported", li, K);
-  if (!S.count_dev) {
-    S.count_dev = (int32_t *)mem.take(256);
-    if (!S.count_dev) return DF3D_ENOMEM;
+  if (!S.prepared) {
+    int rc = geo_prepare(S, gstream);
+    if (rc) return rc;
   }
   const int32_t *nbr = nullptr;
   const void *lists = nullptr;
@@ -185,10 +238,11 @@
       IndexSet &T = S.sets[si];
       if (T.grid) return DF3D_OK;
       T.grid_bytes = df3d_grid_bytes(batch, T.shape);
-      T.grid = mem.take(T.grid_bytes);
+      const bool cleared = (size_t)si < S.set_grid.size() && S.set_grid[si];
+      T.grid = cleared ? S.set_grid[si] : mem.take(T.grid_bytes);
       if (!T.sorted) T.perm = (int32_t *)mem.take((size_t)T.n * 4);
       if (!T.grid || (!T.sorted && !T.perm)) return DF3D_ENOMEM;
-      return df3d_grid_build(T.indices, T.n, batch, T.shape, T.grid, T.grid_bytes, T.perm, gs_);
+      return grid_build_on(T.indices, T.n, batch, T.shape, T.grid, T.grid_bytes, T.perm, !cleared, gstream);
     };
     if (L.kind == 0) {
       int rc = ensure_grid(in_set);
@@ -203,8 +257,7 @@
     } else {
       const IndexSet T = S.sets[in_set];
       IndexSet O;
-      for (int d = 0; d < 3; ++d)
-        O.shape[d] = (T.shape[d] + 2 * L.padding[d] - L.dilation[d] * (L.ksize[d] - 1) - 1) / L.stride[d] + 1;
+      strided_out_shape(L, T.shape, O.shape);
       long long fan = 1;
       for (int d = 0; d < 3; ++d) fan *= (L.ksize[d] + L.stride[d] - 1) / L.stride[d];
       long long vol = (long long)batch * O.shape[0] * O.shape[1] * O.shape[2];
@@ -212,15 +265,18 @@
       if (cap > vol) cap = vol;
       if (cap < 1) cap = 1;
       O.grid_bytes = df3d_grid_bytes(batch, O.shape);
-      O.grid = mem.take(O.grid_bytes);
+      const size_t si = S.sets.size();
+      const bool cleared = si < S.set_grid.size() && S.set_grid[si];
+      O.grid = cleared ? S.set_grid[si] : mem.take(O.grid_bytes);
       int32_t *oi = (int32_t *)mem.take((size_t)cap * 16);
       if (!O.grid || !oi) return DF3D_ENOMEM;
-      int rc = df3d_conv_out_indices(T.indices, T.n, batch, T.shape, O.shape, L.ksize, L.stride, L.padding,
-                                     L.dilation, O.grid, O.grid_bytes, oi, (int)cap, S.count_dev, gs_);
+      int rc = conv_out_indices_on(T.indices, T.n, batch, T.shape, O.shape, L.ksize, L.stride, L.padding, L.dilation, O.grid,
+                                   O.grid_bytes, oi, (int)cap, nullptr, !cleared, gstream);
       if (rc) return rc;
-      int32_t cnt = 0;
-      DF3D_HIP(hipMemcpyAsync(&cnt, S.count_dev, sizeof(cnt), hipMemcpyDeviceToHost, gstream));
+      DF3D_HIP(hipMemcpyAsync(g_count_host, grid_total_word(O.grid, batch, O.shape), sizeof(int32_t), hipMemcpyDeviceToHost,
+                              gstream));
       DF3D_HIP(hipStreamSynchronize(gstream));
+      const int32_t cnt = *g_count_host;
       if (cnt > cap) {
         set_error("backbone_run: layer %d produced %d outputs, capacity bound %lld", li, cnt, cap);
         return DF3D_EINVAL;
@@ -697,6 +753,25 @@
     }
     if (d.ncam > 0) {
       DF3D_CHECK_ARG(d.nproj >= 0 && d.nproj <= DF3D_HEAD_MAX_PROJ && d.slots_proj < d.nproj, "frame_head: bad projection list");
+      const bool maps = d.feat_h > 0 && d.feat_w > 0;
+      const size_t npix = maps ? (size_t)B * d.ncam * d.feat_h * d.feat_w : 0;
+      const bool want_pixrow = d.slots_proj >= 0 && d.want_pixrow && maps;
+      const size_t pix_wsb = want_pixrow ? df3d_query_pixel_rows_workspace_bytes(B, d.ncam, d.feat_h, d.feat_w) : 0;
+      void *pix_ws = nullptr;
+      {
+        std::vector<FillRange> fills;
+        for (int p = 0; p < d.nproj; ++p)
+          if (d.proj[p].want_winner && maps) {
+            HEAD_TAKE(t.out.winner[p], int32_t *, npix * 4);
+            fills.push_back(FillRange{t.out.winner[p], npix, 0xffffffffu});
+          }
+        if (want_pixrow) {
+          HEAD_TAKE(pix_ws, void *, pix_wsb);
+          fills.push_back(FillRange{pix_ws, npix, 0u});
+        }
+        rc = fill_ranges(fills.data(), (int)fills.size(), gs);
+        if (rc) return rc;
+      }
       for (int p = 0; p < d.nproj; ++p) {
         const int li = d.proj[p].layer;
         DF3D_CHECK_ARG(li >= 0 && li < d.nlayers, "frame_head: projection %d reads layer %d", p, li);
@@ -709,10 +784,9 @@
                                  d.depth_thres, d.image_scale, d.feat_scale, t.out.grid_xy[p], t.out.mask[p],
                                  t.out.point_inv[p], nullptr, d.aug_inv, gs_);
         if (rc) return rc;
-        if (d.proj[p].want_winner && d.feat_h > 0 && d.feat_w > 0) {
-          HEAD_TAKE(t.out.winner[p], int32_t *, (size_t)B * d.ncam * d.feat_h * d.feat_w * 4);
-          rc = df3d_scatter_winner(T.indices, t.out.grid_xy[p], t.out.mask[p], T.n, B, d.ncam, d.feat_h, d.feat_w,
-                                   t.out.winner[p], gs_);
+        if (d.proj[p].want_winner && maps) {
+          rc = scatter_winner_on(T.indices, t.out.grid_xy[p], t.out.mask[p], T.n, B, d.ncam, d.feat_h, d.feat_w,
+                                 t.out.winner[p], false, gs);
           if (rc) return rc;
         }
       }
@@ -724,14 +798,11 @@
         rc = df3d_query_slots(t.out.mask[p], T.indices, T.n, B, d.ncam, t.out.pos, t.out.counts, gs_);
         if (rc) return rc;
         int32_t *ptot = nullptr;
-        if (d.want_pixrow && d.feat_h > 0 && d.feat_w > 0) {
-          const size_t wsb = df3d_query_pixel_rows_workspace_bytes(B, d.ncam, d.feat_h, d.feat_w);
-          void *ws;
-          HEAD_TAKE(t.out.pixrow, int32_t *, (size_t)B * d.ncam * d.feat_h * d.feat_w * 4);
+        if (want_pixrow) {
+          HEAD_TAKE(t.out.pixrow, int32_t *, npix * 4);
           HEAD_TAKE(ptot, int32_t *, 256);
-          HEAD_TAKE(ws, void *, wsb);
-          rc = df3d_query_pixel_rows(T.indices, t.out.grid_xy[p], t.out.mask[p], T.n, B, d.ncam, d.feat_h, d.feat_w, t.out.pixrow,
-                                     ptot, ws, wsb, gs_);
+          rc = query_pixel_rows_on(T.indices, t.out.grid_xy[p], t.out.mask[p], T.n, B, d.ncam, d.feat_h, d.feat_w, t.out.pixrow,
+                                   ptot, pix_ws, pix_wsb, false, gs);
           if (rc) return rc;
         }
         std::vector<int32_t> qc((size_t)B * d.ncam, 0);
diff --git a/3d-dual-fusion_amd/csrc/fusion.hip b/3d-dual-fusion_amd/csrc/fusion.hip
--- a/3d-dual-fusion_amd/csrc/fusion.hip
+++ b/3d-dual-fusion_amd/csrc/fusion.hip
@@ -268,9 +268,13 @@
 
 extern "C" int df3d_scatter_winner(const int32_t *indices, const int32_t *grid_xy, const uint8_t *mask, int n, int batch,
                                    int ncam, int H, int W, int32_t *winner, void *stream_) {
-  hipStream_t stream = (hipStream_t)stream_;
+  return df3d::scatter_winner_on(indices, grid_xy, mask, n, batch, ncam, H, W, winner, true, (hipStream_t)stream_);
+}
+
+int df3d::scatter_winner_on(const int32_t *indices, const int32_t *grid_xy, const uint8_t *mask, int n, int batch, int ncam,
+                            int H, int W, int32_t *winner, bool fill, hipStream_t stream) {
   DF3D_CHECK_ARG(winner && batch > 0 && ncam > 0 && H > 0 && W > 0, "scatter_winner: bad arguments");
-  DF3D_HIP(hipMemsetAsync(winner, 0xff, (size_t)batch * ncam * H * W * sizeof(int32_t), stream));
+  if (fill) DF3D_HIP(hipMemsetAsync(winner, 0xff, (size_t)batch * ncam * H * W * sizeof(int32_t), stream));
   if (n == 0) return DF3D_OK;
   DF3D_CHECK_ARG(indices && grid_xy && mask, "scatter_winner: null input");
   ScatArgs a = {nullptr, nullptr, indices, grid_xy, mask, n, 0, ncam, H, W, winner, nullptr};
@@ -591,11 +595,10 @@
 __global__ __launch_bounds__(1024) void query_slots_kernel(const uint8_t *__restrict__ mask,
                                                            const int32_t *__restrict__ ind, int n, int ncam,
                                                            int32_t *__restrict__ pos, int32_t *__restrict__ counts) {
-  const int cam = blockIdx.x, b = blockIdx.y;
+  const int cam = blockIdx.x, b = blockIdx.y, chunk = blockIdx.z;
   const int tid = threadIdx.x, lane = tid & 63, wave = tid >> 6;
   __shared__ int range[2];
-  __shared__ int wsum[16];
-  __shared__ int carry;
+  __shared__ int wsum[16], wbefore[16];
   if (tid < 2) {
     int key = b + tid, lo = 0, hi = n;
     while (lo < hi) {
@@ -605,29 +608,38 @@
     }
     range[tid] = lo;
   }
-  if (tid == 0) carry = 0;
   __syncthreads();
   const int r0 = range[0], r1 = range[1];
+  const long long base_ll = (long long)r0 + (long long)chunk * 1024;
+  if (base_ll >= r1) {
+    if (chunk == 0 && tid == 0) counts[b * ncam + cam] = 0;
+    return;
+  }
+  const int base = (int)base_ll;
   const uint8_t *m = mask + (size_t)cam * n;
-  for (int base = r0; base < r1; base += 1024) {
-    int r = base + tid;
-    bool v = r < r1 && m[r] != 0;
-    unsigned long long bal = __ballot(v);
-    int within = __popcll(bal & ((1ull << lane) - 1ull));
-    if (lane == 0) wsum[wave] = __popcll(bal);
-    __syncthreads();
-    int off = carry;
-    for (int w = 0; w < wave; ++w) off += wsum[w];
-    if (r < r1) pos[(size_t)cam * n + r] = off + within;
-    __syncthreads();
-    if (tid == 0) {
-      int t = 0;
-      for (int w = 0; w < 16; ++w) t += wsum[w];
-      carry += t;
-    }
-    __syncthreads();
-  }
-  if (tid == 0) counts[b * ncam + cam] = carry;
+  int before = 0;
+  for (int r = r0 + tid; r < base; r += 1024) before += m[r] != 0;
+  const int r = base + tid;
+  const bool v = r < r1 && m[r] != 0;
+  const unsigned long long bal = __ballot(v);
+  const int within = __popcll(bal & ((1ull << lane) - 1ull));
+#pragma unroll
+  for (int d = 32; d >= 1; d >>= 1) before += __shfl_xor(before, d, 64);
+  if (lane == 0) {
+    wsum[wave] = __popcll(bal);
+    wbefore[wave] = before;
+  }
+  __syncthreads();
+  int off = 0, tot = 0;
+#pragma unroll
+  for (int w = 0; w < 16; ++w) {
+    off += wbefore[w];
+    const int c = wsum[w];
+    if (w < wave) off += c;
+    tot += c;
+  }
+  if (r < r1) pos[(size_t)cam * n + r] = off + within;
+  if (tid == 0 && base_ll + 1024 >= r1) counts[b * ncam + cam] = off + tot;
 }
 
 __global__ __launch_bounds__(256) void query_inverse_kernel(const int32_t *__restrict__ ind, const uint8_t *__restrict__ mask,
@@ -917,7 +929,13 @@
 extern "C" int df3d_query_pixel_rows(const int32_t *indices, const int32_t *grid_xy, const uint8_t *mask, int n, int batch,
                                      int ncam, int H, int W, int32_t *pixrow, int32_t *total, void *workspace,
                                      size_t workspace_bytes, void *stream_) {
-  hipStream_t stream = (hipStream_t)stream_;
+  return df3d::query_pixel_rows_on(indices, grid_xy, mask, n, batch, ncam, H, W, pixrow, total, workspace, workspace_bytes, true,
+                                   (hipStream_t)stream_);
+}
+
+int df3d::query_pixel_rows_on(const int32_t *indices, const int32_t *grid_xy, const uint8_t *mask, int n, int batch, int ncam,
+                              int H, int W, int32_t *pixrow, int32_t *total, void *workspace, size_t workspace_bytes,
+                              bool zero_flags, hipStream_t stream) {
   DF3D_CHECK_ARG(pixrow && total && workspace && batch > 0 && ncam > 0 && H > 0 && W > 0, "query_pixel_rows: bad arguments");
   const long long npix = (long long)batch * ncam * H * W;
   DF3D_CHECK_ARG(workspace_bytes >= df3d_query_pixel_rows_workspace_bytes_impl(npix), "query_pixel_rows: workspace too small");
@@ -925,7 +943,7 @@
   uint32_t *flag = (uint32_t *)ws;
   uint32_t *rank = (uint32_t *)(ws + align_up((size_t)npix * 4, 256));
   void *scratch = ws + 2 * align_up((size_t)npix * 4, 256);
-  DF3D_HIP(hipMemsetAsync(flag, 0, (size_t)npix * 4, stream));
+  if (zero_flags) DF3D_HIP(hipMemsetAsync(flag, 0, (size_t)npix * 4, stream));
   if (n > 0) {
     DF3D_CHECK_ARG(indices && grid_xy && mask, "query_pixel_rows: null input");
     hipLaunchKernelGGL(mark_query_pixels_kernel, dim3(cdiv((long long)n * ncam, 256)), dim3(256), 0, stream, indices, grid_xy, mask,
@@ -947,7 +965,8 @@
     return DF3D_OK;
   }
   DF3D_CHECK_ARG(mask && indices && pos, "query_slots: null argument");
-  hipLaunchKernelGGL(query_slots_kernel, dim3(ncam, batch), dim3(1024), 0, stream, mask, indices, n, ncam, pos, counts);
+  hipLaunchKernelGGL(query_slots_kernel, dim3(ncam, batch, cdiv(n, 1024)), dim3(1024), 0, stream, mask, indices, n, ncam, pos,
+                     counts);
   DF3D_LAUNCH_CHECK();
   return DF3D_OK;
 }
diff --git a/3d-dual-fusion_amd/csrc/rulebook.hip b/3d-dual-fusion_amd/csrc/rulebook.hip
--- a/3d-dual-fusion_amd/csrc/rulebook.hip
+++ b/3d-dual-fusion_amd/csrc/rulebook.hip
@@ -1,3 +1,5 @@
+#include <vector>
+
 #include "common.h"
 
 namespace df3d {
@@ -51,63 +53,111 @@
 };
 
 __global__ __launch_bounds__(256) void neighbors_kernel(GridView g, const int32_t *__restrict__ perm,
-                                                        const int32_t *__restrict__ out_ind, int n, ConvGeom cg,
+                                                        const int32_t *__restrict__ out_ind, int n, ConvGeom cg, int centre,
                                                         int32_t *__restrict__ nbr) {
+  const int KZY = cg.ks[0] * cg.ks[1];
   long long t = (long long)blockIdx.x * blockDim.x + threadIdx.x;
-  if (t >= (long long)n * cg.K) return;
-  int k = (int)(t / n);
-  int o = (int)(t - (long long)k * n);
-  const int32_t *p = out_ind + (size_t)o * 4;
-  int kx = k % cg.ks[2];
-  int kt = k / cg.ks[2];
-  int ky = kt % cg.ks[1];
-  int kz = kt / cg.ks[1];
-  int z = p[1] * cg.st[0] - cg.pad[0] + kz * cg.dil[0];
-  int y = p[2] * cg.st[1] - cg.pad[1] + ky * cg.dil[1];
-  int x = p[3] * cg.st[2] - cg.pad[2] + kx * cg.dil[2];
-  int r = -1;
-  if (z >= 0 && z < g.shape[0] && y >= 0 && y < g.shape[1] && x >= 0 && x < g.shape[2]) {
-    long long flat = (long long)p[0] * g.vol + ((long long)z * g.shape[1] + y) * g.shape[2] + x;
-    r = grid_rank(g, flat);
-    if (r >= 0 && perm) r = perm[r];
-  }
-  nbr[t] = r;
+  if (t >= (long long)n * KZY) return;
+  const int kzy = (int)(t / n);
+  const int o = (int)(t - (long long)kzy * n);
+  const int4 p = *(const int4 *)(out_ind + (size_t)o * 4);
+  const int kz = kzy / cg.ks[1], ky = kzy - kz * cg.ks[1];
+  const int z = p.y * cg.st[0] - cg.pad[0] + kz * cg.dil[0];
+  const int y = p.z * cg.st[1] - cg.pad[1] + ky * cg.dil[1];
+  const bool row_ok = z >= 0 && z < g.shape[0] && y >= 0 && y < g.shape[1];
+  const long long row = (long long)p.x * g.vol + ((long long)z * g.shape[1] + y) * g.shape[2];
+  const int k0 = kzy * cg.ks[2];
+  int32_t *dst = nbr + (size_t)k0 * n + o;
+  const int x0 = p.w * cg.st[2] - cg.pad[2];
+  int k_lo = 0, k_hi = cg.ks[2] - 1;
+  while (k_lo <= k_hi && x0 + k_lo * cg.dil[2] < 0) ++k_lo;
+  while (k_hi >= k_lo && x0 + k_hi * cg.dil[2] >= g.shape[2]) --k_hi;
+  const bool any = row_ok && k_lo <= k_hi;
+  const long long wa = any ? (row + x0 + k_lo * cg.dil[2]) >> 6 : 0, wb = any ? (row + x0 + k_hi * cg.dil[2]) >> 6 : 0;
+  unsigned long long ba = 0ull, bb = 0ull;
+  uint32_t pa = 0, pb = 0;
+  if (any) {
+    ba = g.bits[wa], bb = g.bits[wb];
+    pa = g.prefix[wa], pb = g.prefix[wb];
+  }
+  for (int kx = 0; kx < cg.ks[2]; ++kx) {
+    int r = -1;
+    if (any && kx >= k_lo && kx <= k_hi) {
+      if (k0 + kx == centre) {
+        r = o;
+      } else {
+        const long long flat = row + x0 + kx * cg.dil[2], wi = flat >> 6;
+        unsigned long long w;
+        uint32_t pre;
+        if (wi == wa) w = ba, pre = pa;
+        else if (wi == wb) w = bb, pre = pb;
+        else w = g.bits[wi], pre = g.prefix[wi];
+        const int b = (int)(flat & 63);
+        if ((w >> b) & 1ull) {
+          r = (int)(pre + __popcll(w & ((1ull << b) - 1ull)));
+          if (perm) r = perm[r];
+        }
+      }
+    }
+    dst[(size_t)kx * n] = r;
+  }
+}
+
+__device__ __forceinline__ void wave_merged_or(unsigned long long *__restrict__ bits, long long w, unsigned long long m) {
+  if (!__any(w >= 0)) return;
+  const int lane = threadIdx.x & 63;
+#pragma unroll
+  for (int d = 1; d < 64; d <<= 1) {
+    const long long ow = __shfl_down(w, d, 64);
+    const unsigned long long om = __shfl_down(m, d, 64);
+    if (lane + d < 64 && ow == w) m |= om;
+  }
+  const long long pw = __shfl_up(w, 1, 64);
+  if (w >= 0 && (lane == 0 || pw != w)) atomicOr(&bits[w], m);
 }
 
 __global__ __launch_bounds__(256) void conv_mark_kernel(const int32_t *__restrict__ ind, int n, ConvGeom cg,
                                                         long long out_vol, unsigned long long *__restrict__ bits) {
   const int KZY = cg.ks[0] * cg.ks[1];
-  long long t = (long long)blockIdx.x * blockDim.x + threadIdx.x;
-  if (t >= (long long)n * KZY) return;
-  int i = (int)(t / KZY);
-  int kzy = (int)(t - (long long)i * KZY);
-  const int32_t *p = ind + (size_t)i * 4;
-  int kk[2] = {kzy / cg.ks[1], kzy % cg.ks[1]};
-  int o[2];
+  const long long t = (long long)blockIdx.x * blockDim.x + threadIdx.x;
+  bool ok = t < (long long)n * KZY;
+  const int kzy = ok ? (int)(t / n) : 0;
+  const int i = ok ? (int)(t - (long long)kzy * n) : 0;
+  const int4 p = ok ? *(const int4 *)(ind + (size_t)i * 4) : make_int4(0, 0, 0, 0);
+  const int kk[2] = {kzy / cg.ks[1], kzy % cg.ks[1]};
+  const int pin[2] = {p.y, p.z};
+  int o[2] = {0, 0};
 #pragma unroll
   for (int d = 0; d < 2; ++d) {
-    int num = p[1 + d] + cg.pad[d] - kk[d] * cg.dil[d];
-    if (num < 0 || (num % cg.st[d]) != 0) return;
+    int num = pin[d] + cg.pad[d] - kk[d] * cg.dil[d];
+    if (num < 0 || (num % cg.st[d]) != 0) ok = false;
     o[d] = num / cg.st[d];
-    if (o[d] >= cg.out_shape[d]) return;
-  }
-  const long long row = (long long)p[0] * out_vol + ((long long)o[0] * cg.out_shape[1] + o[1]) * cg.out_shape[2];
-  long long cur = -1;
-  unsigned long long mask = 0ull;
-  for (int kx = 0; kx < cg.ks[2]; ++kx) {
-    int num = p[3] + cg.pad[2] - kx * cg.dil[2];
-    if (num < 0 || (num % cg.st[2]) != 0) continue;
-    int ox = num / cg.st[2];
-    if (ox >= cg.out_shape[2]) continue;
-    long long flat = row + ox;
-    if ((flat >> 6) != cur) {
-      if (mask) atomicOr(&bits[cur], mask);
-      cur = flat >> 6;
-      mask = 0ull;
+    if (o[d] >= cg.out_shape[d]) ok = false;
+  }
+  const long long row = (long long)p.x * out_vol + ((long long)o[0] * cg.out_shape[1] + o[1]) * cg.out_shape[2];
+  long long w0 = -1, w1 = -1;
+  unsigned long long m0 = 0ull, m1 = 0ull;
+  if (ok) {
+    for (int kx = 0; kx < cg.ks[2]; ++kx) {
+      int num = p.w + cg.pad[2] - kx * cg.dil[2];
+      if (num < 0 || (num % cg.st[2]) != 0) continue;
+      int ox = num / cg.st[2];
+      if (ox >= cg.out_shape[2]) continue;
+      const long long flat = row + ox, wi = flat >> 6;
+      const unsigned long long bit = 1ull << (flat & 63);
+      if (w0 < 0 || wi == w0) {
+        w0 = wi;
+        m0 |= bit;
+      } else if (w1 < 0 || wi == w1) {
+        w1 = wi;
+        m1 |= bit;
+      } else {
+        atomicOr(&bits[wi], bit);
+      }
     }
-    mask |= 1ull << (flat & 63);
-  }
-  if (mask) atomicOr(&bits[cur], mask);
+  }
+  wave_merged_or(bits, w0, m0);
+  wave_merged_or(bits, w1, m1);
 }
 
 __global__ __launch_bounds__(256) void conv_mark_transpose_kernel(const int32_t *__restrict__ ind, int n, ConvGeom cg,
@@ -288,9 +338,21 @@
                                stream);
 }
 
-extern "C" int df3d_grid_build(const int32_t *indices, int n, int batch, const int *shape, void *grid,
-                               size_t grid_bytes, int32_t *perm, void *stream_) {
-  hipStream_t stream = (hipStream_t)stream_;
+namespace df3d {
+
+int zero_directories(int batch, const int (*shapes)[3], void *const *grids, int count, hipStream_t stream) {
+  std::vector<FillRange> r(count);
+  for (int i = 0; i < count; ++i) {
+    GridHeader h = grid_layout(batch, shapes[i]);
+    r[i].p = (char *)grids[i] + h.off_bits;
+    r[i].words = (size_t)h.nwords * 2;
+    r[i].value = 0u;
+  }
+  return fill_ranges(r.data(), count, stream);
+}
+
+int grid_build_on(const int32_t *indices, int n, int batch, const int *shape, void *grid, size_t grid_bytes, int32_t *perm,
+                  bool zero_bits, hipStream_t stream) {
   DF3D_CHECK_ARG(batch > 0 && shape && n >= 0, "grid_build: bad arguments");
   GridHeader h = grid_layout(batch, shape);
   if (grid_bytes < h.off_scratch + h.scratch_bytes) {
@@ -298,7 +360,7 @@
     return DF3D_ENOMEM;
   }
   unsigned long long *bits = (unsigned long long *)((char *)grid + h.off_bits);
-  DF3D_HIP(hipMemsetAsync(bits, 0, (size_t)h.nwords * 8, stream));
+  if (zero_bits) DF3D_HIP(hipMemsetAsync(bits, 0, (size_t)h.nwords * 8, stream));
   Shape3 s3 = {{shape[0], shape[1], shape[2]}};
   long long vol = (long long)shape[0] * shape[1] * shape[2];
   if (n > 0)
@@ -313,11 +375,18 @@
   return DF3D_OK;
 }
 
+}
+
+extern "C" int df3d_grid_build(const int32_t *indices, int n, int batch, const int *shape, void *grid,
+                               size_t grid_bytes, int32_t *perm, void *stream_) {
+  return grid_build_on(indices, n, batch, shape, grid, grid_bytes, perm, true, (hipStream_t)stream_);
+}
+
 extern "C" int df3d_subm_neighbors(const void *grid, const int32_t *perm, const int32_t *indices, int n, int batch,
                                    const int *shape, const int *ksize, const int *dilation, int32_t *nbr,
                                    void *stream_) {
   hipStream_t stream = (hipStream_t)stream_;
-  DF3D_CHECK_ARG(grid && indices && nbr && shape && ksize, "subm_neighbors: null argument");
+  DF3D_CHECK_ARG(grid && shape && ksize && (n == 0 || (indices && nbr)), "subm_neighbors: null argument");
   ConvGeom cg;
   int K = fill_geom(cg, ksize, nullptr, nullptr, dilation, shape, shape);
   DF3D_CHECK_ARG(K <= DF3D_MAX_KVOL, "subm_neighbors: kernel volume %d > %d", K, DF3D_MAX_KVOL);
@@ -329,18 +398,19 @@
   if (n == 0) return DF3D_OK;
   GridHeader h = grid_layout(batch, shape);
   GridView g = grid_view(grid, h);
-  long long total = (long long)n * K;
-  hipLaunchKernelGGL(neighbors_kernel, dim3(cdiv(total, 256)), dim3(256), 0, stream, g, perm, indices, n, cg, nbr);
-  DF3D_LAUNCH_CHECK();
-  return DF3D_OK;
-}
-
-extern "C" int df3d_conv_out_indices(const int32_t *indices, int n, int batch, const int *in_shape,
-                                     const int *out_shape, const int *ksize, const int *stride, const int *padding,
-                                     const int *dilation, void *out_grid, size_t out_grid_bytes,
-                                     int32_t *out_indices, int out_cap, int32_t *num_out, void *stream_) {
-  hipStream_t stream = (hipStream_t)stream_;
-  DF3D_CHECK_ARG(indices && out_grid && out_indices && num_out, "conv_out_indices: null argument");
+  const int centre = ((ksize[0] / 2) * ksize[1] + ksize[1] / 2) * ksize[2] + ksize[2] / 2;
+  long long total = (long long)n * ksize[0] * ksize[1];
+  hipLaunchKernelGGL(neighbors_kernel, dim3(cdiv(total, 256)), dim3(256), 0, stream, g, perm, indices, n, cg, centre, nbr);
+  DF3D_LAUNCH_CHECK();
+  return DF3D_OK;
+}
+
+namespace df3d {
+int conv_out_indices_on(const int32_t *indices, int n, int batch, const int *in_shape, const int *out_shape,
+                        const int *ksize, const int *stride, const int *padding, const int *dilation, void *out_grid,
+                        size_t out_grid_bytes, int32_t *out_indices, int out_cap, int32_t *num_out, bool zero_bits,
+                        hipStream_t stream) {
+  DF3D_CHECK_ARG((indices || n == 0) && out_grid && out_indices, "conv_out_indices: null argument");
   ConvGeom cg;
   int K = fill_geom(cg, ksize, stride, padding, dilation, in_shape, out_shape);
   DF3D_CHECK_ARG(K <= DF3D_MAX_KVOL, "conv_out_indices: kernel volume %d > %d", K, DF3D_MAX_KVOL);
@@ -351,7 +421,7 @@
     return DF3D_ENOMEM;
   }
   unsigned long long *bits = (unsigned long long *)((char *)out_grid + h.off_bits);
-  DF3D_HIP(hipMemsetAsync(bits, 0, (size_t)h.nwords * 8, stream));
+  if (zero_bits) DF3D_HIP(hipMemsetAsync(bits, 0, (size_t)h.nwords * 8, stream));
   long long out_vol = (long long)out_shape[0] * out_shape[1] * out_shape[2];
   if (n > 0) {
     long long total = (long long)n * cg.ks[0] * cg.ks[1];
@@ -362,9 +432,23 @@
   GridView g = grid_view(out_grid, h);
   hipLaunchKernelGGL(grid_enumerate_kernel, dim3(cdiv((long long)h.nwords, 256)), dim3(256), 0, stream, g, h.nwords,
                      out_indices, out_cap);
-  DF3D_HIP(hipMemcpyAsync(num_out, (char *)out_grid + h.off_total, sizeof(int32_t), hipMemcpyDeviceToDevice, stream));
-  DF3D_LAUNCH_CHECK();
-  return DF3D_OK;
+  if (num_out)
+    DF3D_HIP(hipMemcpyAsync(num_out, (char *)out_grid + h.off_total, sizeof(int32_t), hipMemcpyDeviceToDevice, stream));
+  DF3D_LAUNCH_CHECK();
+  return DF3D_OK;
+}
+const int32_t *grid_total_word(const void *grid, int batch, const int *shape) {
+  return (const int32_t *)((const char *)grid + grid_layout(batch, shape).off_total);
+}
+}
+
+extern "C" int df3d_conv_out_indices(const int32_t *indices, int n, int batch, const int *in_shape,
+                                     const int *out_shape, const int *ksize, const int *stride, const int *padding,
+                                     const int *dilation, void *out_grid, size_t out_grid_bytes,
+                                     int32_t *out_indices, int out_cap, int32_t *num_out, void *stream_) {
+  DF3D_CHECK_ARG(num_out, "conv_out_indices: null argument");
+  return conv_out_indices_on(indices, n, batch, in_shape, out_shape, ksize, stride, padding, dilation, out_grid,
+                             out_grid_bytes, out_indices, out_cap, num_out, true, (hipStream_t)stream_);
 }
 
 extern "C" int df3d_conv_transpose_out_indices(const int32_t *indices, int n, int batch, const int *in_shape,
@@ -424,16 +508,16 @@
                                    int n_out, int batch, const int *in_shape, const int *ksize, const int *stride,
                                    const int *padding, const int *dilation, int32_t *nbr, void *stream_) {
   hipStream_t stream = (hipStream_t)stream_;
-  DF3D_CHECK_ARG(in_grid && out_indices && nbr, "conv_neighbors: null argument");
+  DF3D_CHECK_ARG(in_grid && (n_out == 0 || (out_indices && nbr)), "conv_neighbors: null argument");
   ConvGeom cg;
   int K = fill_geom(cg, ksize, stride, padding, dilation, in_shape, nullptr);
   DF3D_CHECK_ARG(K <= DF3D_MAX_KVOL, "conv_neighbors: kernel volume %d > %d", K, DF3D_MAX_KVOL);
   if (n_out == 0) return DF3D_OK;
   GridHeader h = grid_layout(batch, in_shape);
   GridView g = grid_view(in_grid, h);
-  long long total = (long long)n_out * K;
+  long long total = (long long)n_out * ksize[0] * ksize[1];
   hipLaunchKernelGGL(neighbors_kernel, dim3(cdiv(total, 256)), dim3(256), 0, stream, g, in_perm, out_indices, n_out,
-                     cg, nbr);
+                     cg, -1, nbr);
   DF3D_LAUNCH_CHECK();
   return DF3D_OK;
 }
diff --git a/3d-dual-fusion_amd/csrc/voxelize.hip b/3d-dual-fusion_amd/csrc/voxelize.hip
--- a/3d-dual-fusion_amd/csrc/voxelize.hip
+++ b/3d-dual-fusion_amd/csrc/voxelize.hip
@@ -45,15 +45,6 @@
   }
   atomicMin(&first[s], i);
   slot_of_point[i] = (int)s;
-}
-
-__global__ __launch_bounds__(256) void vox_flag_kernel(int P, const int *__restrict__ first,
-                                                       const int *__restrict__ slot_of_point,
-                                                       uint32_t *__restrict__ flag) {
-  int i = blockIdx.x * blockDim.x + threadIdx.x;
-  if (i >= P) return;
-  int s = slot_of_point[i];
-  flag[i] = (s >= 0 && first[s] == i) ? 1u : 0u;
 }
 
 __global__ __launch_bounds__(256) void vox_number_kernel(VoxParams p, const int *__restrict__ keys,
@@ -277,8 +268,7 @@
   }
   int nb = cdiv(num_points, 256);
   hipLaunchKernelGGL(vox_insert_kernel, dim3(nb), dim3(256), 0, stream, points, p, keys, first, slot);
-  hipLaunchKernelGGL(vox_flag_kernel, dim3(nb), dim3(256), 0, stream, num_points, first, slot, rank);
-  int rc = exclusive_scan_u32(rank, rank, (size_t)num_points, (uint32_t *)misc, sscr, ssz, stream);
+  int rc = exclusive_scan_first_flag(first, slot, rank, (size_t)num_points, (uint32_t *)misc, sscr, ssz, stream);
   if (rc) return rc;
   hipLaunchKernelGGL(vox_number_kernel, dim3(nb), dim3(256), 0, stream, p, keys, first, slot, rank, vid, coors, misc,
                      voxel_num);
```

Result: faster. 368.0 (median of 6 runs) (+1.6%).
